# tsy935/eeg-gnn-ssl

Measured on AMD Instinct MI355X. Metric: EEG clips/sec (60s, 19ch, K=2, 2-layer x64) fwd+bwd, higher is better.
Workload: dtype f32

## Files before the change

eeg_gnn_ssl_amd/_lib.py:

```python
from __future__ import annotations

import ctypes
import os
from ctypes import POINTER, c_char_p, c_float, c_int, c_int32, c_int64, c_size_t, c_void_p

_HERE = os.path.dirname(os.path.abspath(__file__))
HIP_LIB_PATH = os.path.join(_HERE, "libeeg_dcrnn_hip.so")
DEV_LIB_PATH = os.path.join(_HERE, "libeeg_dcrnn_hip_dev.so")
ABI_VERSION = 5


class LayerDims(ctypes.Structure):
    _fields_ = [("T", c_int32), ("B", c_int32), ("N", c_int32), ("H", c_int32), ("Fin", c_int32),
                ("M", c_int32), ("act", c_int32), ("p_batched", c_int32), ("x_planes_ready", c_int32),
                ("x_batch_major", c_int32), ("x_plane_stride", c_int64), ("pack3", c_void_p), ("spectral", c_void_p),
                ("spack", c_void_p)]


class DecoderDims(ctypes.Structure):
    _fields_ = [("T", c_int32), ("B", c_int32), ("N", c_int32), ("H", c_int32), ("Dout", c_int32),
                ("M", c_int32), ("L", c_int32), ("act", c_int32), ("p_batched", c_int32), ("dropout_p", c_float),
                ("teacher_on_device", c_int32)]


_FP = c_void_p

_SIGNATURES = {
    "eeg_dcrnn_last_error": (c_char_p, []),
    "eeg_dcrnn_abi_version": (c_int, []),
    "eeg_dcrnn_is_device_build": (c_int, []),
    "eeg_dcrnn_supported": (c_int, [c_int, c_int, c_int, c_int]),
    "eeg_dcrnn_zero": (c_int, [_FP, c_size_t, c_void_p]),
    "eeg_dcrnn_prof_enable": (c_int, [c_int]),
    "eeg_dcrnn_prof_report": (c_int, [ctypes.c_char_p, c_size_t]),
    "eeg_dcrnn_prof_clock_probe": (c_int, [_FP, c_void_p]),
    "eeg_dcrnn_prof_clock_samples": (c_int, [_FP]),
    "eeg_dcrnn_hop_polys": (c_int, [POINTER(c_void_p), c_int, c_int, c_int, c_int, _FP, c_void_p]),
    "eeg_dcrnn_fft_features": (c_int, [_FP, c_int, c_int, c_int, c_int, _FP, _FP, c_float, c_float, _FP, _FP, c_void_p]),
    "eeg_dcrnn_corr_graph_ws_floats": (c_size_t, [c_int, c_int]),
    "eeg_dcrnn_corr_graph": (c_int, [_FP, c_int, c_int, c_int, c_int, c_int, _FP, _FP, _FP, _FP, c_void_p]),
    "eeg_dcrnn_pack_floats": (c_size_t, [c_int, c_int, c_int]),
    "eeg_dcrnn_pack_cell": (c_int, [_FP, _FP, _FP, _FP, c_int, c_int, c_int, _FP, c_void_p]),
    "eeg_dcrnn_pack3_halves": (c_size_t, [c_int, c_int, c_int]),
    "eeg_dcrnn_pack_cell_bf16x3": (c_int, [_FP, _FP, c_int, c_int, c_int, _FP, c_void_p]),
    "eeg_dcrnn_diffuse_fwd": (c_int, [_FP, _FP, c_int, c_int, c_int, c_int, c_int, c_int, _FP, c_void_p]),
    "eeg_dcrnn_diffuse_adj": (c_int, [_FP, _FP, c_int, c_int, c_int, c_int, c_int, c_int, _FP, c_void_p]),
    "eeg_dcrnn_dconv_fwd_ws_floats": (c_size_t, [c_int, c_int, c_int, c_int, c_int]),
    "eeg_dcrnn_dconv_fwd": (c_int, [_FP, _FP, c_int, c_int, c_int, c_int, c_int, _FP, _FP, c_int, _FP, _FP, c_void_p]),
    "eeg_dcrnn_dconv_bwd_ws_floats": (c_size_t, [c_int, c_int, c_int, c_int, c_int]),
    "eeg_dcrnn_dconv_bwd": (c_int, [_FP, _FP, c_int, c_int, c_int, c_int, c_int, _FP, c_int, _FP, _FP, _FP, _FP, _FP, c_void_p]),
    "eeg_dcrnn_spectral_basis_floats": (c_size_t, [c_int]),
    "eeg_dcrnn_spectral_basis": (c_int, [_FP, c_int, _FP, c_void_p]),
    "eeg_dcrnn_spectral_pack_floats": (c_size_t, [c_int, c_int, c_int, c_int]),
    "eeg_dcrnn_pack_cell_spectral": (c_int, [_FP, _FP, _FP, c_int, c_int, c_int, c_int, _FP, c_void_p]),
    "eeg_dcrnn_spectral_ok": (c_int, [POINTER(LayerDims), c_int]),
    "eeg_dcrnn_spectral_rows": (c_size_t, [c_size_t]),
    "eeg_dcrnn_layer_fwd_ws_floats": (c_size_t, [POINTER(LayerDims)]),
    "eeg_dcrnn_batch_major_ok": (c_int, [POINTER(LayerDims)]),
    "eeg_dcrnn_layer_fwd": (c_int, [POINTER(LayerDims)] + [_FP] * 14 + [c_void_p]),
    "eeg_dcrnn_layer_bwd_ws_floats": (c_size_t, [POINTER(LayerDims), c_int]),
    "eeg_dcrnn_layer_bwd": (c_int, [POINTER(LayerDims)] + [_FP] * 22 + [c_void_p]),
    "eeg_dcrnn_decoder_saved_floats": (c_size_t, [POINTER(DecoderDims)]),
    "eeg_dcrnn_decoder_fwd_ws_floats": (c_size_t, [POINTER(DecoderDims)]),
    "eeg_dcrnn_decoder_bwd_ws_floats": (c_size_t, [POINTER(DecoderDims)]),
    "eeg_dcrnn_decoder_is_persistent": (c_int, [POINTER(DecoderDims)]),
    "eeg_dcrnn_decoder_fwd": (c_int, [POINTER(DecoderDims), _FP, c_void_p, _FP, _FP, POINTER(c_void_p), _FP, _FP,
                                      _FP, _FP, _FP, _FP, c_void_p]),
    "eeg_dcrnn_decoder_bwd": (c_int, [POINTER(DecoderDims), c_void_p, _FP, POINTER(c_void_p), _FP, _FP, _FP, _FP, _FP,
                                      POINTER(c_void_p), POINTER(c_void_p), POINTER(c_void_p), POINTER(c_void_p),
                                      _FP, _FP, _FP, c_void_p]),
    "eeg_dcrnn_teacher_flags": (c_int, [_FP, _FP, c_int64, ctypes.c_double, c_int, _FP, c_void_p]),
    "eeg_dcrnn_fft_features_pair": (c_int, [_FP, _FP, c_int, c_int, c_int, c_int, c_int, _FP, _FP, c_float, c_float, _FP, _FP, _FP, c_void_p]),
    "eeg_dcrnn_augment_features": (c_int, [_FP, _FP, c_int, c_int, c_int, c_int, c_int, _FP, _FP, _FP, _FP, c_void_p]),
    "eeg_dcrnn_window_features": (c_int, [_FP, c_int, c_int, c_int, c_int, _FP, _FP, c_float, c_float, _FP, c_void_p]),
    "eeg_dcrnn_window_features_pair": (c_int, [_FP, _FP, c_int, c_int, c_int, c_int, c_int, _FP, _FP, c_float, c_float, _FP, _FP, c_void_p]),
    "eeg_dcrnn_augment_windows": (c_int, [_FP, _FP, c_int, c_int, c_int, c_int, c_int, _FP, _FP, _FP, _FP, _FP, c_void_p]),
    "eeg_dcrnn_corr_graph_rows_ws_floats": (c_size_t, [c_int, c_int, c_int]),
    "eeg_dcrnn_corr_graph_rows": (c_int, [_FP, c_int, c_int, c_int, c_int, ctypes.c_longlong, c_int, _FP, _FP, _FP, _FP, c_void_p]),
    "eeg_dcrnn_augment_draw": (c_int, [_FP, c_int, c_int, _FP, _FP, _FP, _FP, _FP, _FP, c_int, _FP, c_void_p]),
    "eeg_dcrnn_pack_cells": (c_int, [c_int, POINTER(c_void_p), POINTER(c_void_p), POINTER(c_void_p), POINTER(c_void_p), POINTER(ctypes.c_int32),
                             c_int, c_int, POINTER(c_void_p), _FP, c_int, POINTER(c_void_p), c_void_p]),
    "eeg_dcrnn_cls_head_loss_ws_floats": (c_size_t, [c_int, c_int, c_int]),
    "eeg_dcrnn_cls_head_loss": (c_int, [_FP, _FP, _FP, _FP, c_int, c_int, c_int, c_int, c_int, c_float, _FP, _FP, _FP, _FP, _FP, _FP, _FP, _FP, _FP,
                                c_void_p]),
    "eeg_dcrnn_gather_last": (c_int, [_FP, _FP, c_int, c_int, c_int, _FP, c_void_p]),
    "eeg_dcrnn_rng_take": (c_int, [_FP, ctypes.c_uint64, _FP, c_void_p]),
    "eeg_dcrnn_cls_head_fwd": (c_int, [_FP, _FP, _FP, c_int, c_int, c_int, c_int, c_float, _FP, _FP, _FP, c_void_p]),
    "eeg_dcrnn_cls_head_bwd": (c_int, [_FP, _FP, _FP, _FP, c_int, c_int, c_int, c_int, c_float, _FP, _FP, _FP, _FP, c_void_p]),
    "eeg_dcrnn_dropout_mask": (c_int, [_FP, c_size_t, c_float, _FP, c_void_p]),
    "eeg_dcrnn_bce_logits": (c_int, [_FP, _FP, c_int, _FP, _FP, c_void_p]),
    "eeg_dcrnn_ce_logits": (c_int, [_FP, _FP, c_int, c_int, _FP, _FP, c_void_p]),
    "eeg_dcrnn_masked_loss_ws_floats": (c_size_t, []),
    "eeg_dcrnn_masked_loss": (c_int, [_FP, _FP, c_size_t, c_int, c_float, c_float, c_float, c_int, _FP, _FP, _FP, c_void_p]),
    "eeg_dcrnn_clip_adam_ws_floats": (c_size_t, []),
    "eeg_dcrnn_clip_adam": (c_int, [_FP, _FP, _FP, _FP, c_size_t, c_float, c_float, c_float, c_float, c_float, c_float,
                                    c_int, c_float, _FP, _FP, c_void_p]),
    "eeg_dcrnn_clip_adam_dev": (c_int, [_FP, _FP, _FP, _FP, c_size_t, c_float, _FP, c_float, c_float, c_float, c_float,
                                        _FP, c_float, _FP, _FP, c_void_p]),
}


_SIGNATURES_DEV = {
    "eeg_dcrnn_set_seq_probe": (c_int, [_FP]),
    "eeg_dcrnn_set_tuning": (c_int, [c_int, c_int]),
}


class EegDcrnnError(RuntimeError):
    """Raised when a library call reports an error (shape/dtype/launch problems)."""


class EegDcrnnLib:
    def __init__(self, path: str = HIP_LIB_PATH, strict: bool = True):
        if not os.path.exists(path):
            raise ImportError(
                f"{path} not found: the MI355X HIP library is not built. Run `python -c 'import "
                f"__graft_entry__ as g; g.build()'` (or `make -C eeg_gnn_ssl_amd/csrc`). There is no CPU fallback.")
        self.path = path
        self._dll = ctypes.CDLL(path)
        for name, (res, args) in _SIGNATURES.items():
            try:
                fn = getattr(self._dll, name)
            except AttributeError as e:
                if not strict:
                    continue
                raise ImportError(f"{path} does not export {name} (declared in include/eeg_dcrnn.h)") from e
            fn.restype = res
            fn.argtypes = args
        self.is_dev_build = hasattr(self._dll, "eeg_dcrnn_set_tuning")
        if self.is_dev_build:
            for name, (res, args) in _SIGNATURES_DEV.items():
                fn = getattr(self._dll, name)
                fn.restype, fn.argtypes = res, args
        if self._dll.eeg_dcrnn_abi_version() != ABI_VERSION:
            raise ImportError(f"{path}: ABI version {self._dll.eeg_dcrnn_abi_version()} != {ABI_VERSION}; rebuild")
        self.is_device_build = bool(self._dll.eeg_dcrnn_is_device_build())

    def last_error(self) -> str:
        return self._dll.eeg_dcrnn_last_error().decode()

    def call(self, name: str, *args):
        rc = getattr(self._dll, name)(*args)
        if rc != 0:
            raise EegDcrnnError(f"{name}: {self.last_error()}")

    def query(self, name: str, *args):
        return getattr(self._dll, name)(*args)


_LIB = None


def get_lib() -> EegDcrnnLib:
    global _LIB
    if _LIB is None:
        lib = EegDcrnnLib(HIP_LIB_PATH)
        if not lib.is_device_build:
            raise ImportError(f"{HIP_LIB_PATH} is not a device build")
        _LIB = lib
    return _LIB
```

eeg_gnn_ssl_amd/csrc/api.cpp:

```cpp
#include <atomic>
#include <cmath>
#include <cstdarg>
#include <cstdio>
#include <cstring>

#include <string>
#include <vector>

#include "../../include/eeg_dcrnn.h"
#include "../../include/eeg_dcrnn_dev.h"
#include "../../include/eeg_dcrnn_prof.h"
#include "kernels_decoder.h"
#include "kernels_diffuse.h"
#include "kernels_feat.h"
#include "kernels_gemm.h"
#include "kernels_gemm_bf.h"
#include "kernels_graph.h"
#include "kernels_head.h"
#include "kernels_pack.h"
#include "spec_common.h"
#include "spec_launch.h"
#include "kernels_tail.h"
#include "prof.h"
#include "seq_launch.h"
// ... 515 lines not shown
    return 0;
}
namespace {
__global__ __launch_bounds__(256) void clock_probe_kernel(long long ticks, long long* __restrict__ out) {
    const float a = 0.001f * (threadIdx.x & 63), b = 1.f + (threadIdx.x & 63);
    f32x4 p = {0.f, 0.f, 0.f, 0.f}, q = p;
    const long long r0 = realtime_now();
    long long r1 = r0, rh = 0, ch = 0;
    for (int i = 0; i < (1 << 20) && r1 - r0 < ticks; ++i) {
#pragma unroll
        for (int k = 0; k < 16; ++k) { p = mfma16(a, b, p); q = mfma16(b, a, q); }
        r1 = realtime_now();
        if (rh == 0 && r1 - r0 >= ticks / 2) { rh = r1; ch = cycle_now(); }
    }
    const long long c1 = cycle_now();
    if (p[0] + q[0] == 12345.f) out[2] = 1;
    if (threadIdx.x == 0 && rh != 0) {
        atomic_add_u64(reinterpret_cast<unsigned long long*>(out), (unsigned long long)(c1 - ch));
        atomic_add_u64(reinterpret_cast<unsigned long long*>(out) + 1, (unsigned long long)(r1 - rh));
    }
}
}
int eeg_dcrnn_prof_clock_samples(int64_t* buf4) {
    g_clock_samples.store(reinterpret_cast<long long*>(buf4), std::memory_order_release);
    return 0;
}
int eeg_dcrnn_prof_clock_probe(int64_t* out2, void* stream) {
    if (out2 == nullptr) return fail("prof_clock_probe: null output");
    EEG_LAUNCH(clock_probe_kernel, dim3(platform_num_cus()), dim3(256), 0, S_(stream), (long long)20000, reinterpret_cast<long long*>(out2));
    return check_launch("clock_probe");
}
int eeg_dcrnn_supported(int N, int H, int Fin, int M) { return check_dims(N, H, Fin, M) == 0 ? 1 : 0; }
int eeg_dcrnn_zero(void* p, size_t bytes, void* stream) {
    if (bytes == 0) return 0;
    if (p == nullptr) return fail("zero: null pointer");
    if (reinterpret_cast<uintptr_t>(p) % 16 != 0)
        return hipMemsetAsync(p, 0, bytes, S_(stream)) == hipSuccess ? 0 : fail("zero: memset failed");
    const size_t n16 = bytes / 16;
    const int blocks = (int)(n16 / 256 < 1 ? 1 : (n16 / 256 > 1024 ? 1024 : n16 / 256));
    EEG_LAUNCH_P("zero", zero_kernel, dim3(blocks), dim3(256), 0, S_(stream), reinterpret_cast<float4*>(p), n16,
                 reinterpret_cast<unsigned char*>(p) + 16 * n16, (int)(bytes - 16 * n16));
    return check_launch("zero");
}

int eeg_dcrnn_hop_polys(const float* const* supports, int n_supports, int n_graphs, int N, int K, float* P_out,
                        void* stream) {
    if (n_supports < 1 || n_supports > 4) return fail("hop_polys: n_supports=%d unsupported (1..4)", n_supports);
    if (N < 1 || N > kMaxNodes) return fail("hop_polys: num_nodes=%d unsupported", N);
    if (K < 0) return fail("hop_polys: max_diffusion_step=%d unsupported (>= 0)", K);
    if (n_graphs < 1) return fail("hop_polys: no graphs (n_graphs=%d)", n_graphs);
    if (K == 0) return 0;
    if (n_supports * K + 1 > kMaxM) return fail("hop_polys: %d supports x K=%d exceeds %d hop matrices", n_supports, K, kMaxM);
    SupPtrs sp;
    for (int i = 0; i < 4; ++i) sp.p[i] = i < n_supports ? supports[i] : nullptr;
    const size_t lds = 4 * kMaxNodes * kMaxNodes * sizeof(float);
    EEG_LAUNCH_P("hop_polys", hop_polys_kernel, dim3(n_graphs), dim3(round_up(N * N, 64)), lds, S_(stream), sp, n_supports, N, K, P_out);
    return check_launch("hop_polys");
}

size_t eeg_dcrnn_pack_floats(int Fin, int H, int M) { return make_cell_pack(Fin, H, M).total; }

int eeg_dcrnn_pack_cell(const float* Wg, const float* bg, const float* Wc, const float* bc, int Fin, int H, int M,
                        float* pack, void* stream) {
    if (!seq_h_supported(H)) return fail("pack_cell: rnn_units=%d unsupported", H);
    if (Fin < 4 || Fin % 4 != 0) return fail("pack_cell: input dim %d must be a positive multiple of 4", Fin);
    if (!seq_m_supported(M)) return fail("pack_cell: num hop matrices M=%d unsupported (1,2,3,4,5,7)", M);
    CellPack p = make_cell_pack(Fin, H, M);
    EEG_LAUNCH_P("pack_cell", pack_cell_kernel, dim3(512), dim3(256), 0, S_(stream), Wg, bg, Wc, bc, pack, p);
    return check_launch("pack_cell");
}
size_t eeg_dcrnn_pack3_halves(int Fin, int H, int M) { return pack3_supported(Fin, H, M) ? make_pack3(Fin, H, M).total : 0; }
int eeg_dcrnn_pack_cell_bf16x3(const float* Wg, const float* Wc, int Fin, int H, int M, uint16_t* pack3, void* stream) {
    if (!pack3_supported(Fin, H, M)) return fail("pack_cell_bf16x3: rnn_units=%d, input_dim=%d, %d hop matrices: the bf16 split exists for 64 units", H, Fin, M);
    if (Wg == nullptr || Wc == nullptr || pack3 == nullptr) return fail("pack_cell_bf16x3: null pointer");
    EEG_LAUNCH_P("pack_cell", pack_cell_bf3_kernel, dim3(512), dim3(256), 0, S_(stream), Wg, Wc, Fin, H, M, pack3);
    return check_launch("pack_cell_bf3");
}

int eeg_dcrnn_diffuse_fwd(const float* X, const float* P, int p_batched, int S, int B, int N, int F, int M,
                          float* planes, void* stream) {
    if (N < 1 || N > kMaxNodes || F < 4 || F % 4 != 0 || M < 1 || M > kMaxM) return fail("diffuse_fwd: bad dims N=%d F=%d M=%d", N, F, M);
    if (S < 1 || B < 1) return fail("diffuse_fwd: empty input (S=%d, B=%d)", S, B);
    return diffuse_fwd(X, P, p_batched, S, B, N, F, M, planes, S_(stream));
}
int eeg_dcrnn_diffuse_adj(const float* Z, const float* P, int p_batched, int S, int B, int N, int F, int M,
                          float* dX, void* stream) {
    if (N < 1 || N > kMaxNodes || F < 4 || F % 4 != 0 || M < 1 || M > kMaxM) return fail("diffuse_adj: bad dims N=%d F=%d M=%d", N, F, M);
    if (S < 1 || B < 1) return fail("diffuse_adj: empty input (S=%d, B=%d)", S, B);
    return diffuse_adj(Z, P, p_batched, S, B, N, F, M, dX, S_(stream));
}

static bool layer_dims_positive(const eeg_layer_dims* d) {
    return d != nullptr && d->T >= 1 && d->B >= 1 && d->N >= 1 && d->H >= 1 && d->Fin >= 1 && d->M >= 1;
}
size_t eeg_dcrnn_layer_fwd_ws_floats(const eeg_layer_dims* d) {
    if (!layer_dims_positive(d)) return 0;
    const size_t xw = (size_t)d->T * d->B * d->N * 3 * d->H;
    return d->spectral != nullptr ? xw + (size_t)d->N * spec_rows(d->T * d->B) * 3 * d->H : xw;
}

size_t eeg_dcrnn_spectral_basis_floats(int N) { return (N >= 1 && N <= kMaxNodes) ? (size_t)spec_basis_floats(N) : 0; }
size_t eeg_dcrnn_spectral_rows(size_t S) { return (S + 15) / 16 * 16; }
int eeg_dcrnn_spectral_basis(const float* support, int N, float* basis, void* stream) {
    if (N < 2 || N > kMaxNodes) return fail("spectral_basis: num_nodes=%d unsupported (2..%d)", N, kMaxNodes);
    if (support == nullptr || basis == nullptr) return fail("spectral_basis: null pointer");
    if (launch_spec_basis(support, N, basis, S_(stream))) return fail("spectral_basis: launch failed");
    return check_launch("spectral_basis");
}
size_t eeg_dcrnn_spectral_pack_floats(int Fin, int H, int M, int N) {
    return (Fin >= 4 && Fin % 4 == 0 && H == 64 && M >= 1 && M <= kMaxM && N >= 1 && N <= kMaxNodes) ? spec_pack_floats(Fin, H, M, N) : 0;
}
int eeg_dcrnn_pack_cell_spectral(const float* Wg, const float* Wc, const float* basis, int Fin, int H, int M, int N, float* spack,
                                 void* stream) {
    if (eeg_dcrnn_spectral_pack_floats(Fin, H, M, N) == 0)
        return fail("pack_cell_spectral: input_dim=%d rnn_units=%d hop matrices=%d nodes=%d: the spectral form exists for 64 units", Fin, H, M, N);
    if (Wg == nullptr || Wc == nullptr || basis == nullptr || spack == nullptr) return fail("pack_cell_spectral: null pointer");
    if (launch_spec_pack(Wg, Wc, basis, Fin, H, M, N, spack, S_(stream))) return fail("pack_cell_spectral: launch failed");
    return check_launch("pack_cell_spectral");
}
int eeg_dcrnn_pack_cells(int n_cells, const float* const* Wg, const float* const* bg, const float* const* Wc, const float* const* bc,
                         const int32_t* Fin, int H, int M, float* const* packs, const float* basis, int N, float* const* spacks,
                         void* stream) {
    if (n_cells < 1 || n_cells > 4) return fail("pack_cells: %d cells (1..4 per launch)", n_cells);
    if (Wg == nullptr || bg == nullptr || Wc == nullptr || bc == nullptr || Fin == nullptr || packs == nullptr) return fail("pack_cells: null pointer table");
    if (!seq_h_supported(H)) return fail("pack_cells: rnn_units=%d unsupported", H);
    if (!seq_m_supported(M)) return fail("pack_cells: num hop matrices M=%d unsupported (1,2,3,4,5,7)", M);
    if ((basis == nullptr) != (spacks == nullptr)) return fail("pack_cells: the per-frequency packs need the basis block and their output table");
    int fin[4];
    for (int c = 0; c < n_cells; ++c) {
        fin[c] = Fin[c];
        if (fin[c] < 4 || fin[c] % 4 != 0) return fail("pack_cells: input dim %d of cell %d must be a positive multiple of 4", fin[c], c);
        if (Wg[c] == nullptr || bg[c] == nullptr || Wc[c] == nullptr || bc[c] == nullptr || packs[c] == nullptr || (spacks != nullptr && spacks[c] == nullptr))
            return fail("pack_cells: null pointer in the tables of cell %d", c);
        if (spacks != nullptr && eeg_dcrnn_spectral_pack_floats(fin[c], H, M, N) == 0)
            return fail("pack_cells: input_dim=%d rnn_units=%d hop matrices=%d nodes=%d: the spectral form exists for 64 units", fin[c], H, M, N);
    }
    if (launch_pack_cells(n_cells, Wg, bg, Wc, bc, fin, H, M, packs, basis, N, spacks, S_(stream))) return fail("pack_cells: launch failed");
    return check_launch("pack_cells");
}
int eeg_dcrnn_spectral_ok(const eeg_layer_dims* d, int need_dx) {
    if (!layer_dims_positive(d) || d->p_batched) return 0;
    if (d->x_planes_ready && d->Fin != d->H) return 0;
    if (check_dims(d->N, d->H, d->Fin, d->M)) return 0;
    return spec_supported(d->T, d->B, d->N, d->H, d->Fin, d->M, need_dx) ? 1 : 0;
}

int eeg_dcrnn_batch_major_ok(const eeg_layer_dims* d) {
    if (!diffuse_streams(d->p_batched, d->T * d->B, d->B, d->N, d->Fin)) return 0;
    const int R = d->T * d->B * d->N;
    const GemmKnobs k = gemm_knobs();
    return (nn_dma_applies(d->Fin, R, 3 * d->H, k) && tn_dma_applies(d->Fin, 3 * d->H, k)) ? 2 : 1;
}

int eeg_dcrnn_layer_fwd(const eeg_layer_dims* d, const float* X, float* Xtm, const float* h0, const float* P,
                        const float* pack, float* planes, float* Hext, float* Rs, float* Us, float* Cs, float* RHs,
                        float* Hplanes, float* RHplanes, float* ws, void* stream) {
    if (check_dims(d->N, d->H, d->Fin, d->M)) return 1;
    if (d->T < 1 || d->B < 1) return fail("layer_fwd: empty sequence/batch (T=%d, B=%d)", d->T, d->B);
    const bool save = Rs != nullptr;
    if (save != (Us != nullptr) || save != (Cs != nullptr) || save != (RHs != nullptr))
        return fail("layer_fwd: Rs/Us/Cs/RHs must be all NULL or all non-NULL");
    hipStream_t st = S_(stream);
    const int S = d->T * d->B, R = S * d->N, H = d->H, M = d->M, Fin = d->Fin;
    const size_t state = (size_t)d->B * d->N * H;
    CellPack p = make_cell_pack(Fin, H, M);
    if (h0 != nullptr && h0 != Hext && copy_floats(Hext, h0, state, st)) return 1;
    const size_t xs = d->x_plane_stride > 0 ? (size_t)d->x_plane_stride : (size_t)R * Fin;
    BtMap bt;
    if (d->x_batch_major) {
        if (Xtm != nullptr || d->x_planes_ready) return fail("layer_fwd: x_batch_major excludes Xtm and x_planes_ready");
        if (d->spectral == nullptr && eeg_dcrnn_batch_major_ok(d) != 2) return fail("layer_fwd: x_batch_major is not available for this shape (eeg_dcrnn_batch_major_ok)");
        bt.T = d->T; bt.B = d->B; bt.N = d->N;
    }
    float* XW = ws;
    if (d->spectral != nullptr) {
        if (!eeg_dcrnn_spectral_ok(d, 0)) return fail("layer_fwd: the spectral form does not cover this shape (eeg_dcrnn_spectral_ok)");
        if (Xtm != nullptr || d->spack == nullptr) return fail("layer_fwd: spectral excludes Xtm and needs spack");
        if ((Hplanes != nullptr) != (RHplanes != nullptr)) return fail("layer_fwd: Hplanes/RHplanes must be both NULL or both non-NULL");
        const SpecPack sp = make_spec_pack(Fin, H, M, d->N);
        const int N = d->N, Sp = spec_rows(S), SpE = d->B + Sp;
        const size_t xgs = d->x_plane_stride > 0 ? (size_t)d->x_plane_stride : (size_t)Sp * Fin;
        float* Yh = ws + (size_t)R * 3 * H;
        if (!d->x_planes_ready && launch_spec_mix(1, X, d->spectral, nullptr, N, d->T, d->B, Fin, d->x_batch_major ? 1 : 0, planes, st, "spec_mix_x"))
            return fail("spec_mix: launch failed");
        int nnf = g_tune[EEG_TUNE_SPEC_NN_GROUPED] == 0 ? launch_nnf(planes, xgs, Fin, Sp, N, d->spack + sp.sxr, sp.sxr_stride, Yh, num_cus(), st, "gemm_nn_xw", pack + p.bias,
                                               d->spectral + spec_csum_offset(N)) : -1;
        if (nnf > 0) return fail("gemm_nnf: launch failed");
        if (nnf < 0 && launch_nng(planes, Fin, Sp, N, d->spack + sp.sxq, sp.sxq_stride, sp.nct_x, Yh, num_cus(), st, "gemm_nn_xw", pack + p.bias,
                                  d->spectral + spec_csum_offset(N), xgs)) return fail("gemm_nng: launch failed");
        SeqFwdArgs a{XW, h0 != nullptr ? Hext : nullptr, P, d->p_batched, pack + p.bhg, pack + p.bhc, Hext + state, Rs, Us, Cs, RHs, nullptr, nullptr,
                     (size_t)0, d->T, d->B, N, d->act, seq_probe_arg(st)};
        SeqCall call = seq_fwd_call(H, M, N, d->T, d->B, 0, a.probe);
        call.spectral = true; call.Sp = Sp; call.SpE = SpE;
        const SeqPlan plan = seq_fwd_plan(call);
        if (plan.kind == SeqKind::TwoWaveSpec) {
            a.XW = Yh; a.Hpl = Hplanes; a.RHpl = RHplanes; a.spec_U = d->spectral; a.spec_Sp = Sp; a.spec_SpE = SpE;
            if (seq_fwd(H, M, plan, a, st)) return 1;
            if (Hplanes != nullptr) {
                if (launch_spec_zero_rows(Hplanes, N, (d->T + 1) * d->B, SpE, H, st)) return fail("spec_zero_rows: launch failed");
                if (launch_spec_zero_pad(RHplanes, N, S, H, st)) return fail("spec_zero_pad: launch failed");
            }
        } else {
            if (launch_spec_mix(0, Yh, d->spectral, nullptr, N, d->T, d->B, 3 * H, 0, XW, st, "spec_mix_y")) return fail("spec_mix: launch failed");
            if (seq_fwd(H, M, plan, a, st)) return 1;
            if (Hplanes != nullptr) {
                if (launch_spec_mix(1, Hext, d->spectral, nullptr, N, d->T + 1, d->B, H, 0, Hplanes, st, "spec_mix_h", SpE)) return fail("spec_mix: launch failed");
                if (launch_spec_mix(1, RHs, d->spectral, nullptr, N, d->T, d->B, H, 0, RHplanes, st, "spec_mix_h")) return fail("spec_mix: launch failed");
            }
        }
        return check_launch("layer_fwd (spectral)");
    } else if (d->x_planes_ready) {
        if (Xtm != nullptr) return fail("layer_fwd: x_planes_ready excludes a batch-major input");
    } else {
        if (diffuse_fwd(X, P, d->p_batched, S, d->B, d->N, Fin, M, planes, st, xs, d->x_batch_major ? 2 : (Xtm != nullptr ? 1 : 0), Xtm)) return 1;
        if (Xtm != nullptr) X = Xtm;
    }
    SegPtrs segs;
    for (int m = 0; m < kMaxM; ++m) segs.p[m] = m == 0 ? X : (m < M ? planes + (size_t)(m - 1) * xs : nullptr);
    const bool bf3 = d->pack3 != nullptr && pack3_supported(Fin, H, M);
    const Pack3 q = make_pack3(Fin, H, M);
    const NnCall cxw = nn_call(M, Fin, R, 3 * H / 16, 3 * H, 3 * H, bt, p.has_bxq, bf3 ? q.xw_nct : 0);
    if (gemm_nn(gemm_nn_plan(cxw), cxw, segs, NnRhs{pack + p.bx, pack + p.bxq, bf3 ? d->pack3 + q.xw : nullptr}, pack + p.bias, XW, st, "gemm_nn_xw", bt)) return 1;
    if ((Hplanes != nullptr) != (RHplanes != nullptr)) return fail("layer_fwd: Hplanes/RHplanes must be both NULL or both non-NULL");
    SeqFwdArgs a{XW, h0 != nullptr ? Hext : nullptr, P, d->p_batched, pack + p.bhg, pack + p.bhc, Hext + state, Rs, Us, Cs, RHs, Hplanes, RHplanes,
                 (size_t)(d->T + 1) * state, d->T, d->B, d->N, d->act, seq_probe_arg(st)};
    return seq_fwd(H, M, seq_fwd_plan(seq_fwd_call(H, M, d->N, d->T, d->B, a.plane_stride, a.probe)), a, st);
}

size_t eeg_dcrnn_layer_bwd_ws_floats(const eeg_layer_dims* d, int need_dx) { return layer_dims_positive(d) ? bwd_ws(d, need_dx).total : 0; }

int eeg_dcrnn_layer_bwd(const eeg_layer_dims* d, const float* X, const float* P, const float* pack,
                        const float* planes, const float* Hext, const float* Rs, const float* Us, const float* Cs,
                        const float* RHs, const float* Hplanes, const float* RHplanes, const float* dHseq,
                        const float* d_at_end, const float* d_at_len,
                        const int64_t* lengths, float* dX, float* dh0, float* dWg, float* dbg, float* dWc,
                        float* dbc, float* ws, void* stream) {
    if (check_dims(d->N, d->H, d->Fin, d->M)) return 1;
    if (d->T < 1 || d->B < 1) return fail("layer_bwd: empty sequence/batch (T=%d, B=%d)", d->T, d->B);
    hipStream_t st = S_(stream);
    const int S = d->T * d->B, R = S * d->N, H = d->H, M = d->M, Fin = d->Fin, N = d->N;
    const size_t state = (size_t)d->B * N * H;
    CellPack p = make_cell_pack(Fin, H, M);
    BwdWs w = bwd_ws(d, dX != nullptr);
    float* dXW = ws + w.dxw;
    float* dbias = ws + w.dbias;
    SeqBwdArgs a{Hext + state, Hext, Rs, Us, Cs, dHseq, d_at_end, d_at_len,
                 reinterpret_cast<const long long*>(lengths), P, d->p_batched, pack + p.b1, pack + p.b2,
                 dXW, dh0, dbias, d->T, d->B, N, d->act, seq_probe_arg(st)};
    SeqCall call = seq_bwd_call(H, M, N, d->T, d->B, a.probe);
    call.spectral = d->spectral != nullptr; call.Sp = spec_rows(S); call.SpE = d->B + spec_rows(S);
    const SeqPlan plan = seq_bwd_plan(call);
    const bool dyh_done = plan.kind == SeqKind::TwoWaveSpec;
    if (dyh_done) { a.spec_U = d->spectral; a.dYh = ws + w.dyh; a.spec_Sp = call.Sp; }
    if (seq_bwd(H, M, plan, a, st)) return 1;
    const size_t xs = d->x_plane_stride > 0 ? (size_t)d->x_plane_stride : (size_t)R * Fin;
    BtMap bt;
    if (d->x_batch_major) {
        if (d->spectral == nullptr && eeg_dcrnn_batch_major_ok(d) != 2) return fail("layer_bwd: x_batch_major is not available for this shape");
        bt.T = d->T; bt.B = d->B; bt.N = N;
    }
    if (d->spectral != nullptr) {
        if (!eeg_dcrnn_spectral_ok(d, dX != nullptr)) return fail("layer_bwd: the spectral form does not cover this shape (eeg_dcrnn_spectral_ok)");
        if (d->spack == nullptr) return fail("layer_bwd: spectral needs spack");
        if ((Hplanes != nullptr) != (RHplanes != nullptr)) return fail("layer_bwd: Hplanes/RHplanes must be both NULL or both non-NULL");
        const SpecPack sp = make_spec_pack(Fin, H, M, N);
        const int Sp = spec_rows(S), SpE = d->B + Sp;
        float* dYh = ws + w.dyh;
        if (dyh_done) {
            if (launch_spec_zero_pad(dYh, N, S, 3 * H, st)) return fail("spec_zero_pad: launch failed");
        } else if (launch_spec_mix(1, dXW, d->spectral, nullptr, N, d->T, d->B, 3 * H, 0, dYh, st, "spec_mix_dy")) return fail("spec_mix: launch failed");
        const float *hh = Hplanes, *rhh = RHplanes;
        size_t hh_gs = (size_t)SpE * H;
        if (hh == nullptr) {
            if (launch_spec_mix(1, Hext, d->spectral, nullptr, N, d->T, d->B, H, 0, ws + w.hplanes, st, "spec_mix_h")) return fail("spec_mix: launch failed");
            if (launch_spec_mix(1, RHs, d->spectral, nullptr, N, d->T, d->B, H, 0, ws + w.rhplanes, st, "spec_mix_h")) return fail("spec_mix: launch failed");
            hh = ws + w.hplanes; rhh = ws + w.rhplanes; hh_gs = 0;
        }
        if (cell_weight_grads_spectral(d, planes, xs_spec(d), hh, hh_gs, rhh, dYh, ws + w.partial, w, dWg, dWc, st, dbias, dbg, dbc)) return 1;
        if (dX != nullptr) {
            const int dxf = g_tune[EEG_TUNE_SPEC_DX_PASSES] == 0 ? launch_dxf(dYh, Sp, S, N, Fin, d->spack + sp.sxtq, sp.sxtq_stride, d->spectral, dX, st, "gemm_dx_f") : -1;
            if (dxf > 0) return fail("gemm_dxf: launch failed");
            if (dxf < 0) {
                float* dXh = ws + w.z;
                if (launch_nng(dYh, 3 * H, Sp, N, d->spack + sp.sxtq, sp.sxtq_stride, sp.nct_t, dXh, num_cus(), st, "gemm_nn_dx")) return fail("gemm_nng: launch failed");
                if (launch_spec_mix(0, dXh, d->spectral, nullptr, N, d->T, d->B, Fin, 0, dX, st, "spec_mix_dx")) return fail("spec_mix: launch failed");
            }
        }
        return check_launch("layer_bwd (spectral)");
    }
    if (cell_weight_grads(d, X, planes, xs, Hext, RHs, dXW, P, Hplanes, RHplanes, (size_t)(d->T + 1) * state,
                          ws + w.hplanes, ws + w.rhplanes, ws + w.partial, w, false, dWg, dWc, st, bt, dbias, dbg, dbc)) return 1;
    if (dX != nullptr) {
        float* Z = ws + w.z;
        SegPtrs sd;
        for (int m = 0; m < kMaxM; ++m) sd.p[m] = m == 0 ? dXW : nullptr;
        const bool bf3 = d->pack3 != nullptr && pack3_supported(Fin, H, M);
        const Pack3 q = make_pack3(Fin, H, M);
        const NnCall cdx = nn_call(1, 3 * H, R, round_up(M * Fin, 16) / 16, M * Fin, M * Fin, BtMap(), p.has_bxtq, bf3 ? q.dx_nct : 0);
        if (gemm_nn(gemm_nn_plan(cdx), cdx, sd, NnRhs{pack + p.bxt, pack + p.bxtq, bf3 ? d->pack3 + q.dx : nullptr}, nullptr, Z, st, "gemm_nn_dx")) return 1;
        if (diffuse_adj(Z, P, d->p_batched, S, d->B, N, Fin, M, dX, st)) return 1;
    }
    return 0;
}


int eeg_dcrnn_fft_features(const float* raw, int B, int N, int T, int W, const int32_t* perm, const float* log_scale,
                           float mean, float std_, float* feat_raw, float* feat_std, void* stream) {
    if (B < 1 || N < 1 || T < 1) return fail("fft_features: empty input (B=%d, N=%d, T=%d)", B, N, T);
    if (W < 4 || W % 4 != 0 || W / 4 + 1 > 64) return fail("fft_features: window=%d unsupported (multiple of 4, <= 252)", W);
    if (feat_raw == nullptr && feat_std == nullptr) return fail("fft_features: no output requested");
    if (feat_std != nullptr && !(std_ != 0.f)) return fail("fft_features: std must be non-zero");
    if (W == kFftWin) {
        const long long n_windows = (long long)B * N * T;
        const long long n_items = (n_windows + kFftPerWave - 1) / kFftPerWave;
        long long blocks = (n_items + 3) / 4;
        const long long cap = (long long)platform_num_cus() * kFftWgPerCu;
        if (blocks > cap) blocks = cap;
        const size_t lds = 4 * (size_t)kFftWaveDoubles * sizeof(double);
        EEG_SET_MAX_LDS(fft200_features_kernel, lds);
        EEG_LAUNCH_P("fft_features", fft200_features_kernel, dim3((unsigned)blocks), dim3(256), lds, S_(stream), raw, N, T, n_windows,
                     reinterpret_cast<const int*>(perm), log_scale, mean, 1.0f / std_, feat_raw, feat_std);
        return check_launch("fft_features");
    }
    int tchunk = T;
    while (tchunk > 1 && (long long)B * N * ceil_div(T, tchunk) < 8192) tchunk = ceil_div(tchunk, 2);
    EEG_LAUNCH_P("fft_features", fft_features_kernel, dim3(B * N, ceil_div(T, tchunk)), dim3(64), (size_t)W * sizeof(double), S_(stream),
                 raw, N, T, W, tchunk, reinterpret_cast<const int*>(perm), log_scale, mean, 1.0f / std_, feat_raw, feat_std);
    return check_launch("fft_features");
}

int eeg_dcrnn_fft_features_pair(const float* raw_x, const float* raw_y, int B, int N, int Tx, int Ty, int W, const int32_t* perm,
                                const float* log_scale, float mean, float std_, float* feat_raw_x, float* x_std, float* y_std,
                                void* stream) {
    if (raw_x == nullptr || raw_y == nullptr) return fail("fft_features_pair: null input (raw_x=%p, raw_y=%p)", (const void*)raw_x, (const void*)raw_y);
    if (B < 1 || N < 1 || Tx < 1 || Ty < 1) return fail("fft_features_pair: empty input (B=%d, N=%d, Tx=%d, Ty=%d)", B, N, Tx, Ty);
    if (W < 4 || W % 4 != 0 || W / 4 + 1 > 64) return fail("fft_features_pair: window=%d unsupported (multiple of 4, <= 252)", W);
    if (x_std == nullptr || y_std == nullptr)
        return fail("fft_features_pair: null output (x_std=%p, y_std=%p): the pair is the standardised input and target", (void*)x_std, (void*)y_std);
    if (!(std_ != 0.f)) return fail("fft_features_pair: std must be non-zero");
    if (W != kFftWin) {
        if (eeg_dcrnn_fft_features(raw_x, B, N, Tx, W, perm, log_scale, mean, std_, feat_raw_x, x_std, stream)) return 1;
        return eeg_dcrnn_fft_features(raw_y, B, N, Ty, W, perm, log_scale, mean, std_, nullptr, y_std, stream);
    }
    const FftHalf hx = {raw_x, Tx, (long long)B * N * Tx, feat_raw_x, x_std}, hy = {raw_y, Ty, (long long)B * N * Ty, nullptr, y_std};
    const long long n_items = (hx.n_windows + kFftPerWave - 1) / kFftPerWave + (hy.n_windows + kFftPerWave - 1) / kFftPerWave;
    long long blocks = (n_items + 3) / 4;
    const long long cap = (long long)platform_num_cus() * kFftWgPerCu;
    if (blocks > cap) blocks = cap;
    const size_t lds = 4 * (size_t)kFftWaveDoubles * sizeof(double);
    EEG_SET_MAX_LDS(fft200_features_pair_kernel, lds);
    EEG_LAUNCH_P("fft_features_pair", fft200_features_pair_kernel, dim3((unsigned)blocks), dim3(256), lds, S_(stream), hx, hy, N,
                 reinterpret_cast<const int*>(perm), log_scale, mean, 1.0f / std_);
    return check_launch("fft_features_pair");
}

int eeg_dcrnn_augment_features(const float* x, const float* y, int B, int Tx, int Ty, int N, int D, const int32_t* perm, const float* shift,
                               float* x_out, float* y_out, void* stream) {
    if (x == nullptr || y == nullptr || perm == nullptr || shift == nullptr) return fail("augment_features: null input / perm / shift");
    if (x_out == nullptr || y_out == nullptr) return fail("augment_features: null output (x_out=%p, y_out=%p)", (void*)x_out, (void*)y_out);
    if (x_out == x || y_out == y) return fail("augment_features: in-place call (rows move between nodes: outputs must not alias inputs)");
    if (B < 1 || N < 1 || Tx < 1 || Ty < 1) return fail("augment_features: empty input (B=%d, N=%d, Tx=%d, Ty=%d)", B, N, Tx, Ty);
    if (D < 4 || D % 4 != 0) return fail("augment_features: feature dim=%d unsupported (positive multiple of 4)", D);
    if ((((uintptr_t)x | (uintptr_t)y | (uintptr_t)x_out | (uintptr_t)y_out) & 15) != 0) return fail("augment_features: tensors must be 16-byte aligned");
    const long long pieces = (long long)(Tx + Ty) * N * (D / 4);
    const long long chunks = (pieces + kAugPerBlock - 1) / kAugPerBlock;
    if (chunks > 65535) return fail("augment_features: %lld values per clip exceed one launch (limit %lld)", 4 * pieces, 4LL * 65535 * kAugPerBlock);
    const dim3 grid((unsigned)B, (unsigned)chunks);
    if (D == 100)
        EEG_LAUNCH_P("augment_features", augment_features_kernel<25>, grid, dim3(kAugThreads), 0, S_(stream), x, y, N, Tx, Ty, D / 4,
                     reinterpret_cast<const int*>(perm), shift, x_out, y_out);
    else
        EEG_LAUNCH_P("augment_features", augment_features_kernel<0>, grid, dim3(kAugThreads), 0, S_(stream), x, y, N, Tx, Ty, D / 4,
                     reinterpret_cast<const int*>(perm), shift, x_out, y_out);
    return check_launch("augment_features");
}

static int window_stream(const char* what, bool raw, const float* x, const float* y, int B, int Tx, int Ty, int N, int W, const int32_t* perm,
                         const float* a, const float* c, float mean, float std_, float* x_out, float* y_out, void* stream) {
    if (B < 1 || N < 1 || Tx < 1 || Ty < 0) return fail("%s: empty input (B=%d, N=%d, Tx=%d, Ty=%d)", what, B, N, Tx, Ty);
    if (W < 4 || W % 4 != 0) return fail("%s: window=%d unsupported (positive multiple of 4)", what, W);
    if (x_out == x || (Ty > 0 && y_out == y)) return fail("%s: in-place call (rows move between nodes: outputs must not alias inputs)", what);
    if ((((uintptr_t)x | (uintptr_t)y | (uintptr_t)x_out | (uintptr_t)y_out) & 15) != 0) return fail("%s: tensors must be 16-byte aligned", what);
    const long long pieces = (long long)(Tx + Ty) * N * (W / 4);
    const long long chunks = (pieces + kAugPerBlock - 1) / kAugPerBlock;
    if (chunks > 65535) return fail("%s: %lld values per clip exceed one launch (limit %lld)", what, 4 * pieces, 4LL * 65535 * kAugPerBlock);
    const dim3 grid((unsigned)B, (unsigned)chunks);
    const int* pm = reinterpret_cast<const int*>(perm);
#define EEG_WSTREAM(RAW, D4C) \
    EEG_LAUNCH_P(what, (window_stream_kernel<RAW, D4C>), grid, dim3(kAugThreads), 0, S_(stream), x, y, N, Tx, Ty, W / 4, pm, a, c, mean, std_, x_out, y_out)
    if (raw) { if (W == 200) EEG_WSTREAM(true, 50); else EEG_WSTREAM(true, 0); }
    else { if (W == 200) EEG_WSTREAM(false, 50); else EEG_WSTREAM(false, 0); }
#undef EEG_WSTREAM
    return check_launch(what);
}

int eeg_dcrnn_window_features(const float* raw, int B, int N, int T, int W, const int32_t* perm, const float* scale, float mean, float std_,
                              float* x_std, void* stream) {
    if (raw == nullptr) return fail("window_features: null input");
    if (x_std == nullptr) return fail("window_features: null output");
    if (!(std_ != 0.f)) return fail("window_features: std must be non-zero");
    return window_stream("window_features", true, raw, nullptr, B, T, 0, N, W, perm, scale, nullptr, mean, std_, x_std, nullptr, stream);
}

int eeg_dcrnn_window_features_pair(const float* raw_x, const float* raw_y, int B, int N, int Tx, int Ty, int W, const int32_t* perm,
                                   const float* scale, float mean, float std_, float* x_std, float* y_std, void* stream) {
    if (raw_x == nullptr || raw_y == nullptr)
        return fail("window_features_pair: null input (raw_x=%p, raw_y=%p)", (const void*)raw_x, (const void*)raw_y);
    if (x_std == nullptr || y_std == nullptr)
        return fail("window_features_pair: null output (x_std=%p, y_std=%p): the pair is the standardised input and target", (void*)x_std, (void*)y_std);
    if (Ty < 1) return fail("window_features_pair: empty input (B=%d, N=%d, Tx=%d, Ty=%d)", B, N, Tx, Ty);
    if (!(std_ != 0.f)) return fail("window_features_pair: std must be non-zero");
    return window_stream("window_features_pair", true, raw_x, raw_y, B, Tx, Ty, N, W, perm, scale, nullptr, mean, std_, x_std, y_std, stream);
}

int eeg_dcrnn_augment_windows(const float* x, const float* y, int B, int Tx, int Ty, int N, int D, const int32_t* perm, const float* a,
                              const float* c, float* x_out, float* y_out, void* stream) {
    if (x == nullptr || perm == nullptr || a == nullptr || c == nullptr) return fail("augment_windows: null input / perm / factors");
    if ((y == nullptr) != (Ty == 0)) return fail("augment_windows: target and Ty=%d disagree (no target: y = NULL and Ty = 0)", Ty);
    if (x_out == nullptr || (y != nullptr && y_out == nullptr)) return fail("augment_windows: null output (x_out=%p, y_out=%p)", (void*)x_out, (void*)y_out);
    return window_stream("augment_windows", false, x, y, B, Tx, Ty, N, D, perm, a, c, 0.f, 1.f, x_out, y_out, stream);
}

static int corr_nsplit(int B, int T) {
    int ns = ceil_div(g_tune[EEG_TUNE_GRAM_WGS] > 0 ? g_tune[EEG_TUNE_GRAM_WGS] : 1024, B);
    const int cap = ceil_div(T, 4);
    if (ns > cap) ns = cap;
    return ns < 1 ? 1 : ns;
}
int eeg_dcrnn_augment_draw(const uint64_t* rng_used, int B, int N, const int32_t* swap_perm, int32_t* flags, int32_t* perm,
                           float* log_scale, const float* S_plain, const float* S_reflected, int n_supports, float* S_out, void* stream) {
    if (rng_used == nullptr || swap_perm == nullptr || flags == nullptr || perm == nullptr || log_scale == nullptr)
        return fail("augment_draw: null generator pair / swap table / output");
    if (B < 1 || N < 1 || N > kMaxNodes) return fail("augment_draw: B=%d clips, num_nodes=%d unsupported (B >= 1, 1 <= N <= %d)", B, N, kMaxNodes);
// ... 511 lines not shown
```

eeg_gnn_ssl_amd/csrc/kernels_gemm_f.h:

```cpp
#pragma once
#include "common.h"
#include "kernels_gemm_q.h"

namespace eeg {

#ifndef EEG_X_TNF_RC
#define EEG_X_TNF_RC 8
#endif
#ifndef EEG_X_TNF_NS
#define EEG_X_TNF_NS 5
#endif
#ifndef EEG_X_TNF_MINW
#define EEG_X_TNF_MINW 2
#endif
#ifndef EEG_X_TNF_NS2
#define EEG_X_TNF_NS2 3
#endif
#ifndef EEG_X_TNF_MINW2
#define EEG_X_TNF_MINW2 3
#endif
constexpr int kTnfRC = EEG_X_TNF_RC;
__host__ __device__ constexpr int tnf_ns(int FXT) { return FXT <= 2 ? EEG_X_TNF_NS2 : EEG_X_TNF_NS; }
__host__ __device__ constexpr int tnf_wgs_per_cu(int FXT) { return FXT <= 2 ? EEG_X_TNF_MINW2 : EEG_X_TNF_MINW; }
__host__ __device__ constexpr int tnf_stage_floats(int FXT) { return (kTnfRC / 8) * (FXT * 256 + 512 + 512 + 1536); }
// ... 229 lines not shown
            dsc[j] = rx; lofs[j] = d * 256; cstep[j] = (unsigned)(RC * Fin) * 4u;
            soff[j] = (unsigned)(rbeg * Fin) * 4u;
            vof[j] = d * 1024 + lane * 16 < RC * Fin * 4 ? (unsigned)(d * 1024 + lane * 16) : 0u;
        } else if (d < NX + NH) {
            dsc[j] = rh; lofs[j] = HI + (d - NX) * 256; cstep[j] = RC * 64 * 4u;
            soff[j] = (unsigned)(rbeg * 64) * 4u; vof[j] = (unsigned)((d - NX) * 1024 + lane * 16);
        } else if (d < NX + 2 * NH) {
            dsc[j] = rr; lofs[j] = RI + (d - NX - NH) * 256; cstep[j] = RC * 64 * 4u;
            soff[j] = (unsigned)(rbeg * 64) * 4u; vof[j] = (unsigned)((d - NX - NH) * 1024 + lane * 16);
        } else {
            dsc[j] = ry; lofs[j] = YI + (d - NX - 2 * NH) * 256; cstep[j] = RC * 192 * 4u;
            soff[j] = (unsigned)(rbeg * 192) * 4u; vof[j] = (unsigned)((d - NX - 2 * NH) * 1024 + lane * 16);
        }
    }
    float* px = part_x + (size_t)y * Fin * 192;
    float* pg = part_g + (size_t)y * 64 * 128;
    float* pc = part_c + (size_t)y * 64 * 64;
    const TnfRing<FXT> rg{dsc, lofs, vof, soff, cstep};
#ifndef EEG_X_TNF_NOR4
    if constexpr (FXT == 4) {
        if (Fin == 100) {
            if (s == 0) { if (e == 0) tnf_role_r4<0, 0>(sm, Q, lane, rg, px, pg, pc); else tnf_role_r4<0, 1>(sm, Q, lane, rg, px, pg, pc); }
            else { if (e == 0) tnf_role_r4<1, 0>(sm, Q, lane, rg, px, pg, pc); else tnf_role_r4<1, 1>(sm, Q, lane, rg, px, pg, pc); }
            return;
        }
    }
#endif
    if (s == 0) tnf_role<FXT, 0>(sm, Q, Fin, e, lane, rg, px, pg, pc);
    else tnf_role<FXT, 1>(sm, Q, Fin, e, lane, rg, px, pg, pc);
}

#ifndef EEG_X_NNF_NS
#define EEG_X_NNF_NS 3
#endif
constexpr int kNnfNS = EEG_X_NNF_NS;
__host__ __device__ constexpr int nnf_stage_floats(int K) { return 64 * K + 4; }
__host__ __device__ constexpr size_t nnf_lds_bytes(int K) { return (size_t)kNnfNS * nnf_stage_floats(K) * sizeof(float); }

template <int KQ, bool SWZ>
__global__ __launch_bounds__(256, 2) void gemm_nnf_kernel(const float* __restrict__ A, long long a_gstride, int K, int Sp, int G,
                                                         const float* __restrict__ Wr, unsigned w_gstride, float* __restrict__ C,
                                                         const float* __restrict__ bias, const float* __restrict__ gscale) {
    constexpr int NS = kNnfNS;
    EEG_DYN_SMEM(sm);
    const int tid = threadIdx.x, lane = tid & 63, w = wave_uniform(tid >> 6), rw = w & 1, cw = w >> 1, hh = lane >> 5, l32 = lane & 31;
    const int ST = nnf_stage_floats(K), CPG = ceil_div(Sp, 64), total = G * CPG;
    const int NPC = ceil_div(64 * K, 256), PER = ceil_div(NPC, 4);
    const int g0 = (int)(((long long)blockIdx.x * total) / gridDim.x), g1 = (int)(((long long)(blockIdx.x + 1) * total) / gridDim.x);
    const int Q = g1 - g0;
    if (tid < 4 * NS) sm[(tid >> 2) * ST + 64 * K + (tid & 3)] = 0.f;
    const unsigned lane_src = SWZ ? (unsigned)((lane >> 4) * 256 + (((lane & 15) ^ ((4 * w + (lane >> 4)) & 15)) << 4)) : (unsigned)lane * 16u;
    int d_g = g0, d_stage = 0, d_grp = -1;
    wbuf_t ra = make_wbuf_n(A, 0u);
    auto issue = [&]() __attribute__((always_inline)) {
        const int grp = d_g / CPG, lc = d_g - grp * CPG;
        if (grp != d_grp) { d_grp = grp; ra = make_wbuf_n(A + (size_t)grp * a_gstride, (unsigned)(Sp * K) * 4u); }
        float* base = sm + d_stage * ST;
        const unsigned cb = (unsigned)(lc * 64 * K) * 4u;
        for (int j = 0; j < PER; ++j) {
            int p = w + 4 * j;
            if (p >= NPC) p = NPC - 1;
            wbuf_dma16(ra, base + p * 256, cb + (unsigned)p * 1024u + lane_src, 0u);
        }
        d_stage = d_stage + 1 == NS ? 0 : d_stage + 1;
        ++d_g;
    };
    float wr[KQ][4][3];
    f32x16 acc[3];
    float binit[3] = {0.f, 0.f, 0.f};
    int c_grp = -1;
    wbuf_t rc = make_wbuf_n(C, 0u);
    const int row = 32 * rw + l32;
    const int a_row = row * K;
    const int ccol = 32 * 3 * cw + l32;
#pragma unroll 1
    for (int p = 0; p < NS - 1; ++p)
        if (p < Q) issue();
    int r_stage = 0;
#pragma unroll 1
    for (int q = 0; q < Q; ++q) {
        const int g = g0 + q, grp = g / CPG, lc = g - grp * CPG;
        if (grp != c_grp) {
            c_grp = grp;
            const wbuf_t rwt = make_wbuf(Wr + (size_t)grp * w_gstride);
#pragma unroll
            for (int kq = 0; kq < KQ; ++kq)
#pragma unroll
                for (int s = 0; s < 4; ++s)
#pragma unroll
                    for (int t = 0; t < 3; ++t) wr[kq][s][t] = wbuf_ld(rwt, (unsigned)(4 * hh * 192 + ccol), (unsigned)((8 * kq + s) * 192 + 32 * t));
            const float gs = bias != nullptr ? gscale[grp] : 0.f;
#pragma unroll
            for (int t = 0; t < 3; ++t) binit[t] = bias != nullptr ? gs * bias[ccol + 32 * t] : 0.f;
            rc = make_wbuf_n(C + (size_t)grp * Sp * 192, (unsigned)(Sp * 192) * 4u);
        }
        {
            int nd = Q - 1 - q;
            if (nd > NS - 2) nd = NS - 2;
            const int n = 48 * (q < NS - 1 ? q : NS - 1) + PER * nd;
            if (n >= 63) vm_wait_n<63>(); else if (n >= 55) vm_wait_n<55>(); else if (n >= 52) vm_wait_n<52>(); else if (n >= 48) vm_wait_n<48>();
            else if (n >= 14) vm_wait_n<14>(); else if (n >= 8) vm_wait_n<8>(); else if (n >= 7) vm_wait_n<7>(); else if (n >= 4) vm_wait_n<4>();
            else vm_wait_n<0>();
        }
#ifndef EEG_X_NNF_NOBAR
        EEG_LDS_BARRIER();
#endif
#ifndef EEG_X_NNF_NODMA
        if (q + NS - 1 < Q) issue();
#endif
        const float* st = sm + r_stage * ST;
#pragma unroll
        for (int t = 0; t < 3; ++t)
#pragma unroll
            for (int v = 0; v < 16; ++v) acc[t][v] = binit[t];
        f32x4 a4 = *reinterpret_cast<const f32x4*>(st + a_row + (SWZ ? ((hh ^ (row & 15)) << 2) : 4 * hh));
#pragma unroll
        for (int kq = 0; kq < KQ; ++kq) {
            f32x4 an = a4;
#ifndef EEG_X_NNF_NOLDS
            if (kq + 1 < KQ) an = *reinterpret_cast<const f32x4*>(st + a_row + (SWZ ? (((2 * (kq + 1) + hh) ^ (row & 15)) << 2) : 4 * (2 * (kq + 1) + hh)));
#endif
            EEG_SCHED_FENCE();
#pragma unroll
            for (int s = 0; s < 4; ++s)
#pragma unroll
                for (int t = 0; t < 3; ++t) acc[t] = mfma32(a4[s], wr[kq][s][t], acc[t]);
            EEG_SCHED_FENCE();
            a4 = an;
        }
        unsigned ob[4];
#pragma unroll
        for (int b = 0; b < 4; ++b) {
            ob[b] = (unsigned)((lc * 64 + 32 * rw + 4 * hh + 8 * b) * 192 + ccol);
            EEG_PIN(ob[b]);
        }
#pragma unroll
        for (int t = 0; t < 3; ++t)
#pragma unroll
#ifndef EEG_X_NNF_NOSTORE
            for (int v = 0; v < 16; ++v) wbuf_st1(rc, ob[v >> 2] + (unsigned)((v & 3) * 192 + 32 * t), 0u, acc[t][v]);
#else
            for (int v = 0; v < 16; ++v) { EEG_USE(acc[t][v]); (void)rc; }
#endif
        EEG_SCHED_FENCE();
        r_stage = r_stage + 1 == NS ? 0 : r_stage + 1;
    }
}

constexpr int kDxfMaxN = 20, kDxfNS = 3, kDxfRows = 32, kDxfStage = kDxfRows * 192;
__host__ __device__ constexpr size_t dxf_lds_bytes() { return (size_t)kDxfNS * kDxfStage * sizeof(float); }

template <int NT>
__global__ __launch_bounds__(256, 2) void gemm_dxf_kernel(const float* __restrict__ dYh, int Sp, int S, int Nrt, const float* __restrict__ Wtq,
                                                         unsigned w_gstride, const float* __restrict__ basis, float* __restrict__ dX) {
    const int N = NT > 0 ? NT : Nrt;
    constexpr int NS = kDxfNS, ST = kDxfStage, RB = kDxfRows, PER = 6;
    EEG_DYN_SMEM(sm);
    const int tid = threadIdx.x, lane = tid & 63, w = wave_uniform(tid >> 6), lr = lane & 15, lg = lane >> 4;
    const int r0 = (int)blockIdx.x * RB;
    unsigned src[PER];
#pragma unroll
    for (int j = 0; j < PER; ++j) {
        const int P = 64 * (w + 4 * j) + lane, row = P / 48, slot = P - row * 48;
        const int unit = (slot & ~15) | ((slot & 15) ^ (row & 15));
        src[j] = (unsigned)((r0 + row) * 768 + unit * 16);
    }
    int d_i = 0, d_stage = 0;
    auto issue = [&]() __attribute__((always_inline)) {
        const wbuf_t ra = make_wbuf_n(dYh + (size_t)d_i * Sp * 192, (unsigned)(Sp * 192) * 4u);
        float* base = sm + d_stage * ST;
#pragma unroll
        for (int j = 0; j < PER; ++j) wbuf_dma16(ra, base + (w + 4 * j) * 256, src[j], 0u);
        d_stage = d_stage + 1 == NS ? 0 : d_stage + 1;
        if (d_i + 1 < N) ++d_i;
    };
    f32x4 acc[kDxfMaxN][2];
#pragma unroll
    for (int j = 0; j < kDxfMaxN; ++j) acc[j][0] = acc[j][1] = (f32x4){0.f, 0.f, 0.f, 0.f};
    f32x4 wq[12];
    const unsigned wl = (unsigned)(w * 64 + lane) * 4u;
    static_assert(kDxfNS == 3, "the queue discipline below is written for two images in flight");
    issue();
    issue();
    EEG_SCHED_FENCE();
    {
        const wbuf_t rw0 = make_wbuf(Wtq);
#pragma unroll
        for (int c = 0; c < 12; ++c) wq[c] = wbuf_ld4(rw0, wl, (unsigned)(c * 4 * 256));
    }
    vm_wait_n<PER + 12>();
    int r_stage = 0;
    const int a_row = lr * 192;
#pragma unroll 1
    for (int i = 0; i < N; ++i) {
        EEG_LDS_BARRIER();
#ifndef EEG_X_DXF_NODMA
        issue();
#endif
        const wbuf_t rwn = make_wbuf(Wtq + (size_t)(i + 1 < N ? i + 1 : i) * w_gstride);
        const float* st = sm + r_stage * ST;
        float uu[kDxfMaxN];
#pragma unroll
        for (int j = 0; j < kDxfMaxN; ++j) uu[j] = (NT > 0 ? j < NT : j < N) ? basis[j * N + i] : 0.f;
        f32x4 t0 = {0.f, 0.f, 0.f, 0.f}, t1 = {0.f, 0.f, 0.f, 0.f};
        auto frag_off = [&](int c) __attribute__((always_inline)) {
            const int u = 4 * c + lg;
            return a_row + (((u & ~15) | ((u & 15) ^ lr)) << 2);
        };
        f32x4 fa[2][2];
        fa[0][0] = *reinterpret_cast<const f32x4*>(st + frag_off(0));
        fa[0][1] = *reinterpret_cast<const f32x4*>(st + 16 * 192 + frag_off(0));
#pragma unroll
        for (int c = 0; c < 12; ++c) {
            if (c + 1 < 12) {
                fa[(c + 1) & 1][0] = *reinterpret_cast<const f32x4*>(st + frag_off(c + 1));
                fa[(c + 1) & 1][1] = *reinterpret_cast<const f32x4*>(st + 16 * 192 + frag_off(c + 1));
            }
            EEG_SCHED_FENCE();
#pragma unroll
            for (int e = 0; e < 4; ++e) {
                t0 = mfma16(wq[c][e], fa[c & 1][0][e], t0);
                t1 = mfma16(wq[c][e], fa[c & 1][1][e], t1);
            }
            EEG_SCHED_FENCE();
#ifndef EEG_X_DXF_NOW
            wq[c] = wbuf_ld4(rwn, wl, (unsigned)(c * 4 * 256));
#endif
            EEG_SCHED_FENCE();
        }
#pragma unroll
        for (int j = 0; j < kDxfMaxN; ++j)
            if (NT > 0 ? j < NT : j < N) {
                acc[j][0] += t0 * uu[j];
                acc[j][1] += t1 * uu[j];
            }
        r_stage = r_stage + 1 == NS ? 0 : r_stage + 1;
    }
    const wbuf_t rx = make_wbuf_n(dX, (unsigned)(S * N * 64) * 4u);
#pragma unroll
    for (int t = 0; t < 2; ++t) {
        const unsigned rb = (unsigned)((r0 + 16 * t + lr) * N * 64 + 16 * w + 4 * lg);
#pragma unroll
        for (int j = 0; j < kDxfMaxN; ++j)
            if (j < N) wbuf_st4(rx, rb + (unsigned)(j * 64), 0u, acc[j][t]);
    }
}

}
```

eeg_gnn_ssl_amd/csrc/kernels_seq.h:

```cpp
#pragma once
#include "common.h"
#include "lds_diffuse.h"

namespace eeg {

constexpr int seq_nks(int N) { return N <= 20 ? 5 : 8; }
constexpr bool seq_has_two_wave(int H, int M, int nks) { return H == 64 && nks == 5 && M <= 3; }
constexpr bool seq_has_spec(int H, int M, int nks) { return seq_has_two_wave(H, M, nks) && M >= 2; }
constexpr bool seq_has_probe(int H, int M, int nks) { return kDevBuild && H == 64 && M == 3 && nks == 5; }
constexpr bool seq_has_stream(int H, int M) { return H == 64 && M <= 5; }

template <int H, int M>
struct SeqGeom {
    static constexpr int KA = M * H, KAP = lds_stride_x(KA), KS = KA / 4;
    static constexpr int KG = M * 2 * H, KGP = lds_stride_x(KG), KSG = KG / 4;
    static constexpr int NGT = 2 * H / 16, NCT = H / 16;
    static constexpr int GT = ceil_div(NGT, 4), CT = ceil_div(NCT, 4);
};
constexpr size_t seq_fwd_lds_floats(int H, int M) { return (size_t)(M - 1) * kPFloats + 2 * 32 * lds_stride_x(M * H); }
constexpr size_t seq_fwd2_lds_floats(int H, int M, bool spec) {
    return seq_fwd_lds_floats(H, M) + 16 * 64 + (spec ? 3 * 16 * 64 + 4 * 64 + 4 * (M * H / 4 / 4) * 256 : 0);
}
constexpr size_t seq_bwd_lds_floats(int H, int M, int rows) {
    return (size_t)(M - 1) * kPFloats + (size_t)rows * (lds_stride_x(M * H) + lds_stride_x(M * 2 * H));
// ... 143 lines not shown
    if constexpr (Q0 >= Q1) return;
    float4 a0 = frag(p0, s0, Q0), a1 = frag(p1, s1, Q0);
#pragma unroll
    for (int q = Q0; q < Q1; ++q) {
        float4 n0 = a0, n1 = a1;
        if (q + 1 < Q1) { n0 = frag(p0, s0, q + 1); n1 = frag(p1, s1, q + 1); }
        EEG_SCHED_FENCE();
        const float x0[4] = {a0.x, a0.y, a0.z, a0.w}, x1[4] = {a1.x, a1.y, a1.z, a1.w};
#pragma unroll
        for (int j = 0; j < 4; ++j) {
            if (j & 1) alt = mfma16(w[4 * q + j], x0[j], alt);
            else acc = mfma16(w[4 * q + j], x0[j], acc);
        }
#pragma unroll
        for (int j = 0; j < 4; ++j) rem[j] = mfma4(x1[j], w[4 * q + j], rem[j]);
        EEG_SCHED_FENCE();
        a0 = n0;
        a1 = n1;
    }
}

template <int NKS>
__device__ __forceinline__ void load_spec_frags(const float* __restrict__ U, int N, int lane, float (&uf)[NKS], float (&u4)[NKS]) {
    const int lr = lane & 15, lg = lane >> 4;
#pragma unroll
    for (int ks = 0; ks < NKS; ++ks) {
        const int n = 4 * ks + lg, i4 = 16 + (lane & 3);
        uf[ks] = (n < N && lr < N) ? U[n * N + lr] : 0.f;
        u4[ks] = (n < N && i4 < N) ? U[n * N + i4] : 0.f;
    }
}
template <int NKS, int NG>
__device__ __forceinline__ void spec_mix_tiles_out(const float* const (&tile)[NG], const int (&stride)[NG], const int (&src_col)[NG],
                                                   const int (&gcol)[NG], const float (&uf)[NKS], const float (&u4)[NKS], int lr, int lg,
                                                   wbuf_t out, unsigned voff0, unsigned voff1, unsigned soff, bool valid0, bool valid1) {
    float a[NG][NKS];
#pragma unroll
    for (int g = 0; g < NG; ++g)
#pragma unroll
        for (int ks = 0; ks < NKS; ++ks) a[g][ks] = tile[g][lds_sw(4 * ks + lg, src_col[g] + lr, stride[g])];
    f32x4 acc[NG], alt[NG], rem[NG], rem2[NG];
#pragma unroll
    for (int g = 0; g < NG; ++g) acc[g] = alt[g] = rem[g] = rem2[g] = (f32x4){0.f, 0.f, 0.f, 0.f};
#pragma unroll
    for (int ks = 0; ks < NKS; ++ks)
#pragma unroll
        for (int g = 0; g < NG; ++g) {
            if (NG == 1 && (ks & 1)) alt[g] = mfma16(a[g][ks], uf[ks], alt[g]);
            else acc[g] = mfma16(a[g][ks], uf[ks], acc[g]);
        }
#pragma unroll
    for (int ks = 0; ks < NKS; ++ks)
#pragma unroll
        for (int g = 0; g < NG; ++g) {
            if (ks & 1) rem2[g] = mfma4(u4[ks], a[g][ks], rem2[g]);
            else rem[g] = mfma4(u4[ks], a[g][ks], rem[g]);
        }
    if (NG == 1) acc[0] += alt[0];
#pragma unroll
    for (int g = 0; g < NG; ++g) {
        f32x4 tr = rem[g] + rem2[g];
        EEG_PIN(tr);
        const float r1 = rem4_reduce(tr);
        if (valid0) wbuf_st4(out, voff0 + (unsigned)gcol[g], soff, acc[g]);
        if (valid1) wbuf_st1(out, voff1 + (unsigned)gcol[g], soff, r1);
    }
}

template <int NKS>
__device__ __forceinline__ float mfma_rem4_ldsw(const float* __restrict__ X, int stride, int lane, int lg, const float* __restrict__ wl) {
    const int s1 = lg ^ sigma4(lane & 3);
    const float* p1 = X + (16 + (lane & 3)) * stride;
    auto frag = [&](int q) { return *reinterpret_cast<const float4*>(p1 + 64 * (q >> 2) + 4 * ((4 * (q & 3)) ^ s1)); };
    f32x4 rem[4];
#pragma unroll
    for (int j = 0; j < 4; ++j) rem[j] = (f32x4){0.f, 0.f, 0.f, 0.f};
    constexpr int NQ = NKS / 4, D = 2;
    float4 xa[D], wa[D];
#pragma unroll
    for (int d = 0; d < D; ++d) {
        xa[d] = frag(d < NQ ? d : NQ - 1);
        wa[d] = *reinterpret_cast<const float4*>(wl + (d < NQ ? d : NQ - 1) * 256 + 4 * lane);
    }
#pragma unroll
    for (int q = 0; q < NQ; ++q) {
        const float4 a1 = xa[q % D], w4 = wa[q % D];
        if (q + D < NQ) {
            xa[q % D] = frag(q + D);
            wa[q % D] = *reinterpret_cast<const float4*>(wl + (q + D) * 256 + 4 * lane);
        }
        EEG_SCHED_FENCE();
        const float x1[4] = {a1.x, a1.y, a1.z, a1.w}, ww[4] = {w4.x, w4.y, w4.z, w4.w};
#pragma unroll
        for (int j = 0; j < 4; ++j) rem[j] = mfma4(x1[j], ww[j], rem[j]);
        EEG_SCHED_FENCE();
    }
    f32x4 t = (rem[0] + rem[1]) + (rem[2] + rem[3]);
    EEG_PIN(t);
    return rem4_reduce(t);
}

struct ClockSample {
    long long c0, r0;
    __device__ __forceinline__ void begin(const long long* clk, bool me) {
        if (clk != nullptr && me) { c0 = cycle_now(); r0 = realtime_now(); }
    }
    __device__ __forceinline__ void end(long long* clk, bool me) {
        if (clk != nullptr && me) {
            atomic_add_u64(reinterpret_cast<unsigned long long*>(clk), (unsigned long long)(cycle_now() - c0));
            atomic_add_u64(reinterpret_cast<unsigned long long*>(clk) + 1, (unsigned long long)(realtime_now() - r0));
        }
    }
};

template <bool ON>
struct PhaseProbe {
    long long acc[8];
    long long last;
    long long rt[4];
    __device__ __forceinline__ void start() {
        if (ON) {
#pragma unroll
            for (int i = 0; i < 8; ++i) acc[i] = 0;
            rt[0] = realtime_now();
            rt[1] = rt[2] = rt[3] = 0;
            last = cycle_now();
        }
    }
    __device__ __forceinline__ void mark(int k) {
        if (ON) {
            const long long t = cycle_now();
            acc[k] += t - last;
            last = t;
        }
    }
    __device__ __forceinline__ void stamp(int k) {
        if (ON) rt[k] = realtime_now();
    }
    __device__ __forceinline__ void dump(long long* p, int slot0) {
        if (ON) {
            rt[3] = realtime_now();
            if (p != nullptr && (threadIdx.x & 63) == 0) {
                long long* d = p + ((size_t)blockIdx.x * 4 + ((threadIdx.x >> 6) & 3)) * 32 + slot0;
#pragma unroll
                for (int i = 0; i < 8; ++i) d[i] = acc[i];
                long long* e = p + ((size_t)blockIdx.x * 4 + ((threadIdx.x >> 6) & 3)) * 32 + 16 + slot0 / 2;
#pragma unroll
                for (int i = 0; i < 4; ++i) e[i] = rt[i];
            }
        }
    }
};

template <int H, int M, int NKS, bool PROBE = false>
__global__ __launch_bounds__(256, 1) void seq_fwd_kernel(
    const float* __restrict__ XW, const float* __restrict__ h0, const float* __restrict__ P, int p_batched,
    const float* __restrict__ bhg, const float* __restrict__ bhc,
    float* __restrict__ Hseq, float* __restrict__ Rs, float* __restrict__ Us, float* __restrict__ Cs,
    float* __restrict__ RHs, float* __restrict__ Hpl, float* __restrict__ RHpl, size_t plane_stride,
    int T, int B, int N, int act, long long* probe) {
    using G = SeqGeom<H, M>;
    constexpr int KAP = G::KAP, KS = G::KS, CT = G::CT, NGT = G::NGT, NCT = G::NCT;
    PhaseProbe<PROBE> pp;
    pp.start();
    EEG_DYN_SMEM(sm);
    float* Pl = sm;
    float* A = Pl + (M - 1) * kPFloats;
    float* A2 = A + 32 * KAP;
    constexpr bool REM4 = NKS == 5;
    const int tid = threadIdx.x, lane = tid & 63, wave = tid >> 6, lr = lane & 15, lg = lane >> 4;
    const bool save = Rs != nullptr;

    float wg[2 * CT][KS], wc[CT][KS];
#pragma unroll
    for (int i = 0; i < CT; ++i) {
        const int ct = wave + 4 * i < NCT ? wave + 4 * i : 0;
#pragma unroll
        for (int ks = 0; ks < KS; ++ks) {
            wg[i][ks] = bhg[((size_t)ks * NGT + ct) * 64 + lane];
            wg[CT + i][ks] = bhg[((size_t)ks * NGT + NCT + ct) * 64 + lane];
            wc[i][ks] = bhc[((size_t)ks * NCT + ct) * 64 + lane];
        }
    }

    for (int b = blockIdx.x; b < B; b += gridDim.x) {
    __syncthreads();
    for (int e = tid; e < 2 * 32 * KAP; e += 256) A[e] = 0.f;
    lds_load_polys(Pl, P, p_batched ? b : 0, M, N);
    __syncthreads();
    float pf[poly_slots<M, NKS>()][NKS];
    load_poly_frags<M, NKS, false>(Pl, pf, lr, lg);
    if (h0 != nullptr) {
        for (int e = tid; e < N * H; e += 256) A[lds_sw(e / H, e % H, KAP)] = h0[(size_t)b * N * H + e];
    } else {
        for (int e = tid; e < N * H; e += 256) (Hseq - (size_t)B * N * H)[(size_t)b * N * H + e] = 0.f;
    }
    __syncthreads();

    const int node[2] = {lr, 16 + lr};
    const bool valid[2] = {lr < N, 16 + lr < N};
    const int nodec[2] = {valid[0] ? lr : N - 1, valid[1] ? 16 + lr : N - 1};
    const f32x4 zero4 = {0.f, 0.f, 0.f, 0.f};
    int oxw[CT][2], oh[CT][2];
    const int node1 = 16 + lg;
    const bool valid1 = node1 < N;
    int l1[CT];
#pragma unroll
    for (int i = 0; i < CT; ++i)
#pragma unroll
        for (int nt = 0; nt < 2; ++nt) {
            const int ct = wave + 4 * i < NCT ? wave + 4 * i : 0;
            oxw[i][nt] = nodec[nt] * (3 * H) + ct * 16 + 4 * lg;
            oh[i][nt] = nodec[nt] * H + ct * 16 + 4 * lg;
            if (REM4 && nt == 1) {
                oxw[i][1] = (valid1 ? node1 : N - 1) * (3 * H) + ct * 16 + lr;
                oh[i][1] = (valid1 ? node1 : N - 1) * H + ct * 16 + lr;
                l1[i] = lds_sw(node1, ct * 16 + lr, KAP);
            }
        }

    const bool plane_buf = (double)(M - 1) * plane_stride * sizeof(float) < 2147483648.0;
    auto diffuse_own = [&](float* buf, float* planes, int t) {
        EEG_WAVE_SYNC();
        float* g = planes != nullptr ? planes + ((size_t)t * B + b) * N * H : nullptr;
#pragma unroll
        for (int i = 0; i < CT; ++i)
            if (wave + 4 * i < NCT) lds_diffuse_tile<M, NKS>(buf, KAP, (wave + 4 * i) * 16, H, pf, lr, lg, g, plane_stride, N, plane_buf);
    };
    diffuse_own(A, Hpl, 0);
    f32x4 nxr[CT][2], nxu[CT][2], nxc[CT][2];
    auto fetch_xw = [&](int t) {
        const wbuf_t bx = make_wbuf(XW + ((size_t)t * B + b) * N * (3 * H));
#pragma unroll
        for (int i = 0; i < CT; ++i)
#pragma unroll
            for (int nt = 0; nt < 2; ++nt) {
                if (REM4 && nt == 1) {
                    nxr[i][1] = (f32x4){wbuf_ld(bx, oxw[i][1], 0u), 0.f, 0.f, 0.f};
                    nxu[i][1] = (f32x4){wbuf_ld(bx, oxw[i][1] + H, 0u), 0.f, 0.f, 0.f};
                    nxc[i][1] = (f32x4){wbuf_ld(bx, oxw[i][1] + 2 * H, 0u), 0.f, 0.f, 0.f};
                    continue;
                }
                nxr[i][nt] = wbuf_ld4(bx, oxw[i][nt], 0u);
                nxu[i][nt] = wbuf_ld4(bx, oxw[i][nt] + H, 0u);
                nxc[i][nt] = wbuf_ld4(bx, oxw[i][nt] + 2 * H, 0u);
            }
    };
    fetch_xw(0);
    for (int t = 0; t < T; ++t) {
        const size_t s = (size_t)t * B + b;
        f32x4 ag[2 * CT][2], ac[CT][2], ug[CT][2];
#pragma unroll
        for (int i = 0; i < CT; ++i)
#pragma unroll
            for (int nt = 0; nt < 2; ++nt) {
                ag[i][nt] = nxr[i][nt]; ag[CT + i][nt] = nxu[i][nt]; ac[i][nt] = nxc[i][nt];
            }
        EEG_LDS_BARRIER();
        pp.mark(0);

        mfma_nodes32<2 * CT, KS, REM4, 0, 0, false, false, REM4>(A, KAP, lane, lr, lg, wg, ag);
        pp.mark(1);
        const wbuf_t bR = make_wbuf((save ? Rs : Hseq) + s * N * H), bRH = make_wbuf((save ? RHs : Hseq) + s * N * H),
                     bU = make_wbuf((save ? Us : Hseq) + s * N * H);
#pragma unroll
        for (int i = 0; i < CT; ++i) {
            const int ct = wave + 4 * i;
            if (ct < NCT) {
                const int col = ct * 16 + 4 * lg;
#pragma unroll
                for (int nt = 0; nt < 2; ++nt) {
                    if (REM4 && nt == 1) {
                        const float rg1 = sigmoidf_(ag[i][1][0]), u1 = sigmoidf_(ag[CT + i][1][0]);
                        ug[i][1] = (f32x4){u1, 0.f, 0.f, 0.f};
                        const float rh1 = valid1 ? rg1 * A[l1[i]] : 0.f;
                        A2[l1[i]] = rh1;
                        if (save && valid1) {
                            wbuf_st1(bR, oh[i][1], 0u, rg1);
                            wbuf_st1(bRH, oh[i][1], 0u, rh1);
                            wbuf_st1(bU, oh[i][1], 0u, u1);
                        }
                        continue;
                    }
                    const f32x4 rg = sigmoid4_(ag[i][nt]), u = sigmoid4_(ag[CT + i][nt]);
                    ug[i][nt] = u;
                    f32x4 rh = rg * ld4(A + lds_sw(node[nt], col, KAP));
                    rh = valid[nt] ? rh : zero4;
                    st4(A2 + lds_sw(node[nt], col, KAP), rh);
                    if (save && valid[nt]) {
                        wbuf_st4(bR, oh[i][nt], 0u, rg);
                        wbuf_st4(bRH, oh[i][nt], 0u, rh);
                        wbuf_st4(bU, oh[i][nt], 0u, u);
                    }
                }
            }
        }
        pp.mark(2);
        diffuse_own(A2, RHpl, t);
        pp.mark(7);
        EEG_LDS_BARRIER();
        pp.mark(3);
        if (t + 1 < T) fetch_xw(t + 1);

        mfma_nodes32<CT, KS, REM4, 0, 0, false, false, REM4>(A2, KAP, lane, lr, lg, wc, ac);
        pp.mark(4);
        const wbuf_t bH = make_wbuf(Hseq + s * N * H), bC = make_wbuf((save ? Cs : Hseq) + s * N * H);
#pragma unroll
        for (int i = 0; i < CT; ++i) {
            const int ct = wave + 4 * i;
            if (ct < NCT) {
                const int col = ct * 16 + 4 * lg;
#pragma unroll
                for (int nt = 0; nt < 2; ++nt) {
                    if (REM4 && nt == 1) {
                        const float u1 = ug[i][1][0], h1 = A[l1[i]];
                        const float c1 = act == 0 ? tanhf_(ac[i][1][0]) : fmaxf(ac[i][1][0], 0.f);
                        const float hn1 = valid1 ? u1 * h1 + (1.f - u1) * c1 : 0.f;
                        A[l1[i]] = hn1;
                        if (valid1) {
                            wbuf_st1(bH, oh[i][1], 0u, hn1);
                            if (save) wbuf_st1(bC, oh[i][1], 0u, c1);
                        }
                        continue;
                    }
                    const f32x4 u = ug[i][nt], h = ld4(A + lds_sw(node[nt], col, KAP));
                    const f32x4 c = act == 0 ? tanh4_(ac[i][nt]) : relu4_(ac[i][nt]);
                    f32x4 hn = u * h + (1.f - u) * c;
                    hn = valid[nt] ? hn : zero4;
                    st4(A + lds_sw(node[nt], col, KAP), hn);
                    if (valid[nt]) {
                        wbuf_st4(bH, oh[i][nt], 0u, hn);
                        if (save) wbuf_st4(bC, oh[i][nt], 0u, c);
                    }
                }
            }
        }
        pp.mark(5);
        if (t + 1 < T || Hpl != nullptr) diffuse_own(A, Hpl, t + 1);
        pp.mark(6);
    }
    }
    pp.dump(probe, 0);
}

template <int H, int M, int NKS, bool PROBE = false, bool SPEC = false>
__global__ __launch_bounds__(512, 1) void seq_fwd2_kernel(
    const float* __restrict__ XW, const float* __restrict__ h0, const float* __restrict__ P, int p_batched,
    const float* __restrict__ bhg, const float* __restrict__ bhc,
    float* __restrict__ Hseq, float* __restrict__ Rs, float* __restrict__ Us, float* __restrict__ Cs,
    float* __restrict__ RHs, float* __restrict__ Hpl, float* __restrict__ RHpl, size_t plane_stride,
    int T, int B, int N, int act, long long* probe, const float* __restrict__ spec_U = nullptr, int spec_Sp = 0, int spec_SpE = 0) {
    using G = SeqGeom<H, M>;
    PhaseProbe<PROBE> pp;
    pp.start();
    static_assert(G::CT == 1 && NKS == 5, "one column tile per wave, second node tile on the 4x4x1 MFMA");
    constexpr int KAP = G::KAP, KS = G::KS, NGT = G::NGT, NCT = G::NCT, UST = 64;
    EEG_DYN_SMEM(sm);
    float* Pl = sm;
    float* A = Pl + (M - 1) * kPFloats;
    float* A2 = A + 32 * KAP;
    const int tid = threadIdx.x, lane = tid & 63, wave8 = SPEC ? wave_uniform(tid >> 6) : (tid >> 6), role = wave8 >> 2, wave = wave8 & 3;
    const int lr = lane & 15, lg = lane >> 4;
    float* U = A2 + 32 * KAP;
    float* XR = U + 16 * UST;
    float* XC = XR + 16 * UST;
    float* XRr = XC + 2 * 16 * UST;
    float* W1L = XRr + 4 * 64;
    const bool save = Rs != nullptr;
    const int ct = wave;
    const wbuf_t bH = make_wbuf(Hseq), bR = make_wbuf(save ? Rs : Hseq), bU = make_wbuf(save ? Us : Hseq),
                 bC = make_wbuf(save ? Cs : Hseq), bRH = make_wbuf(save ? RHs : Hseq);

    float w0[1][KS], w1[1][KS];
#pragma unroll
    for (int ks = 0; ks < KS; ++ks) w0[0][ks] = bhg[((size_t)ks * NGT + (role == 0 ? ct : NCT + ct)) * 64 + lane];
    if (!SPEC || role == 0) {
#pragma unroll
        for (int ks = 0; ks < KS; ++ks) w1[0][ks] = bhc[((size_t)ks * NCT + ct) * 64 + lane];
    } else {
#pragma unroll
        for (int q = 0; q < KS / 4; ++q) {
            f32x4 v;
#pragma unroll
            for (int j = 0; j < 4; ++j) v[j] = bhc[((size_t)(4 * q + j) * NCT + ct) * 64 + lane];
            st4(W1L + (ct * (KS / 4) + q) * 256 + 4 * lane, v);
        }
    }
    auto clip = [&](const int b, auto ROLE_T) __attribute__((always_inline)) {
    constexpr int ROLE_C = decltype(ROLE_T)::value;
    __syncthreads();
    for (int e = tid; e < 2 * 32 * KAP; e += 512) A[e] = 0.f;
    lds_load_polys(Pl, P, p_batched ? b : 0, M, N);
    __syncthreads();
    if (h0 != nullptr) {
        for (int e = tid; e < N * H; e += 512) A[lds_sw(e / H, e % H, KAP)] = h0[(size_t)b * N * H + e];
    } else {
        for (int e = tid; e < N * H; e += 512) (Hseq - (size_t)B * N * H)[(size_t)b * N * H + e] = 0.f;
    }
    __syncthreads();

    const bool valid[2] = {lr < N, 16 + lr < N};
    const int nodec[2] = {valid[0] ? lr : N - 1, valid[1] ? 16 + lr : N - 1};
    const f32x4 zero4 = {0.f, 0.f, 0.f, 0.f};
    const int col = ct * 16 + 4 * lg;
    const int oxw0 = nodec[0] * (3 * H) + col, oh0 = nodec[0] * H + col;
    const int node1 = 16 + lg, col1 = ct * 16 + lr;
    const bool valid1 = node1 < N;
    const int oxw1 = (valid1 ? node1 : N - 1) * (3 * H) + col1, oh1 = (valid1 ? node1 : N - 1) * H + col1;
    const int l1 = lds_sw(node1, col1, KAP);
    if (ROLE_C < 0 ? role == 0 : ROLE_C == 0) {
        EEG_SETPRIO(3);
        float pf[poly_slots<M, NKS>()][NKS];
        load_poly_frags<M, NKS, false>(Pl, pf, lr, lg);
        auto diffuse_own = [&](float* buf, float* planes, int t) {
            EEG_WAVE_SYNC();
            float* g = (!SPEC && planes != nullptr) ? planes + ((size_t)t * B + b) * N * H : nullptr;
            lds_diffuse_tile<M, NKS>(buf, KAP, ct * 16, H, pf, lr, lg, g, plane_stride, N, true);
        };
        diffuse_own(A, Hpl, 0);
        f32x4 nxr0 = zero4, nxc = zero4;
        float nxr1 = 0.f;
        auto fetch_xw = [&](int t) {
            if constexpr (SPEC) return;
            const wbuf_t bx = make_wbuf(XW + ((size_t)t * B + b) * N * (3 * H));
            nxr0 = wbuf_ld4(bx, oxw0, 0u);
            nxr1 = wbuf_ld(bx, oxw1, 0u);
            nxc = wbuf_ld4(bx, oxw0 + 2 * H, 0u);
        };
        fetch_xw(0);
        pp.stamp(1);
        pp.last = PROBE ? cycle_now() : 0;
        ClockSample cs;
        const bool cs_me = !PROBE && b == 0 && tid == 0;
        cs.begin(probe, cs_me);
        constexpr int QSA = KS / 4 / M;
        f32x4 rc[5] = {zero4, zero4, zero4, zero4, zero4};
        f32x4 ra = zero4;
        bool pre_r = false;
        for (int t = 0; t < T; ++t) {
            const size_t s = (size_t)t * B + b;
            f32x4 ar[1][2] = {{nxr0, (f32x4){nxr1, 0.f, 0.f, 0.f}}}, ac[1][2] = {{nxc, zero4}};
            const unsigned so = (unsigned)(s * N * H);
            EEG_LDS_BARRIER();
            pp.mark(0);
            if constexpr (SPEC) {
                ar[0][0] = ld4(XR + lds_sw(lr, col, UST));
                ar[0][1][0] = XRr[ct * 64 + lane];
                if (M > 1 && pre_r) ra += ar[0][0];
            }

            if (M > 1 && pre_r) {
                ar[0][0] = ra;
                mfma_nodes32<1, KS, true, 0, 0, false, true, true, (M > 1 ? QSA : 0)>(A, KAP, lane, lr, lg, w0, ar, rc);
            } else
                mfma_nodes32<1, KS, true, 0, 0, false, true, true>(A, KAP, lane, lr, lg, w0, ar);
            pp.mark(1);
            {
                const f32x4 rg = sigmoid4_(ar[0][0]);
                f32x4 rh = rg * ld4(A + lds_sw(lr, col, KAP));
                rh = valid[0] ? rh : zero4;
                st4(A2 + lds_sw(lr, col, KAP), rh);
                const float rg1 = sigmoidf_(ar[0][1][0]);
                const float rh1 = valid1 ? rg1 * A[l1] : 0.f;
                A2[l1] = rh1;
                if (save && valid[0]) {
                    wbuf_st4(bR, oh0, so, rg);
                    wbuf_st4(bRH, oh0, so, rh);
                }
                if (save && valid1) {
                    wbuf_st1(bR, oh1, so, rg1);
                    wbuf_st1(bRH, oh1, so, rh1);
                }
            }
            pp.mark(2);
            diffuse_own(A2, RHpl, t);
            pp.mark(7);
            EEG_LDS_BARRIER();
            pp.mark(3);
            if (t + 1 < T) fetch_xw(t + 1);
            if constexpr (SPEC) ac[0][0] = ld4(XC + (t & 1) * (16 * UST) + lds_sw(lr, col, UST));
            mfma_nodes32<1, KS, true, 1>(A2, KAP, lane, lr, lg, w1, ac);
            pp.mark(4);
            {
                const f32x4 u = ld4(U + lds_sw(lr, col, UST)), h = ld4(A + lds_sw(lr, col, KAP));
                const f32x4 c = act == 0 ? tanh4_(ac[0][0]) : relu4_(ac[0][0]);
                f32x4 hn = u * h + (1.f - u) * c;
                hn = valid[0] ? hn : zero4;
                st4(A + lds_sw(lr, col, KAP), hn);
                if (valid[0]) {
                    wbuf_st4(bH, oh0, so, hn);
                    if (save) wbuf_st4(bC, oh0, so, c);
                }
            }
            pp.mark(5);
            EEG_LDS_BARRIER();
            if (t + 1 < T || (!SPEC && Hpl != nullptr)) diffuse_own(A, Hpl, t + 1);
            pre_r = M > 1 && t + 1 < T;
            if (pre_r) {
                ra = SPEC ? zero4 : nxr0;
                rc[0] = rc[1] = rc[2] = rc[3] = rc[4] = zero4;
                f32x4 rr4[4] = {zero4, zero4, zero4, zero4};
                mfma_tile_quads<KS, 0, QSA>(A, KAP, lane, lr, lg, w0[0], ra, rc[4], rr4);
                rc[0] = rr4[0]; rc[1] = rr4[1]; rc[2] = rr4[2]; rc[3] = rr4[3];
            }
            pp.mark(6);
        }
        cs.end(probe, cs_me);
        pp.stamp(2);
    } else {
        f32x4 nxu0 = zero4;
        float nxu1 = 0.f, nxc1 = 0.f;
        float ux[NKS], ux4[NKS], ut[NKS], ut4[NKS], yv[3][NKS];
        const unsigned vyb = (unsigned)lg * (unsigned)spec_Sp * (3 * H) + ct * 16 + lr;
        const unsigned vy4 = (unsigned)(16 + lg < N ? 16 + lg : N - 1) * (unsigned)spec_Sp * (3 * H) + ct * 16 + lr;
        const wbuf_t bY = make_wbuf(XW), bHh = make_wbuf(Hpl != nullptr ? Hpl : Hseq), bRHh = make_wbuf(RHpl != nullptr ? RHpl : Hseq);
        const unsigned oe0 = (unsigned)lr * (unsigned)spec_SpE * H + col, oe1 = (unsigned)node1 * (unsigned)spec_SpE * H + col1;
        const unsigned or0 = (unsigned)lr * (unsigned)spec_Sp * H + col, or1 = (unsigned)node1 * (unsigned)spec_Sp * H + col1;
        if constexpr (SPEC) {
            load_spec_frags<NKS>(spec_U, N, lane, ut, ut4);
#pragma unroll
            for (int ks = 0; ks < NKS; ++ks) {
                const int i = 4 * ks + lg, j4 = 16 + (lane & 3);
                ux[ks] = (i < N && lr < N) ? spec_U[lr * N + i] : 0.f;
                ux4[ks] = (i < N && j4 < N) ? spec_U[j4 * N + i] : 0.f;
            }
        }
        auto fetch_y = [&](int t) {
            const unsigned so = (unsigned)(((size_t)t * B + b) * (3 * H));
#pragma unroll
            for (int g = 0; g < 3; ++g)
#pragma unroll
                for (int ks = 0; ks < NKS; ++ks)
                    yv[g][ks] = ks < 4 ? wbuf_ld(bY, vyb + g * H, so + (unsigned)(4 * ks) * (unsigned)spec_Sp * (3 * H)) : wbuf_ld(bY, vy4 + g * H, so);
        };
        auto xw_mix = [&](int tn) {
            f32x4 acc[3] = {zero4, zero4, zero4}, rem[3] = {zero4, zero4, zero4}, rem2[3] = {zero4, zero4, zero4};
#pragma unroll
            for (int ks = 0; ks < NKS; ++ks)
#pragma unroll
                for (int g = 0; g < 3; ++g) acc[g] = mfma16(yv[g][ks], ux[ks], acc[g]);
#pragma unroll
            for (int ks = 0; ks < NKS; ++ks)
#pragma unroll
                for (int g = 0; g < 3; ++g) {
                    if (ks & 1) rem2[g] = mfma4(ux4[ks], yv[g][ks], rem2[g]);
                    else rem[g] = mfma4(ux4[ks], yv[g][ks], rem[g]);
                }
            f32x4 t0 = rem[0] + rem2[0], t1 = rem[1] + rem2[1], t2 = rem[2] + rem2[2];
            EEG_PIN(t0); EEG_PIN(t1); EEG_PIN(t2);
            st4(XR + lds_sw(lr, col, UST), acc[0]);
            st4(XC + (tn & 1) * (16 * UST) + lds_sw(lr, col, UST), acc[2]);
            XRr[ct * 64 + lane] = rem4_reduce(t0);
            nxu0 = acc[1];
            nxu1 = rem4_reduce(t1);
            nxc1 = rem4_reduce(t2);
        };
        auto export_tile = [&](const float* tile, wbuf_t out, unsigned o0, unsigned o1, unsigned row) {
            const float* const tl[1] = {tile};
            const int strd[1] = {KAP}, scol[1] = {ct * 16}, gcol[1] = {0};
            spec_mix_tiles_out<NKS, 1>(tl, strd, scol, gcol, ut, ut4, lr, lg, out, o0, o1, row * H, valid[0], valid1);
        };
        auto fetch_x = [&](int t) {
            if constexpr (SPEC) { fetch_y(t); return; }
            const wbuf_t bx = make_wbuf(XW + ((size_t)t * B + b) * N * (3 * H));
            nxu0 = wbuf_ld4(bx, oxw0 + H, 0u);
            nxu1 = wbuf_ld(bx, oxw1 + H, 0u);
            nxc1 = wbuf_ld(bx, oxw1 + 2 * H, 0u);
        };
        fetch_x(0);
        if constexpr (SPEC) {
            xw_mix(0);
        }
        constexpr int QS = KS / 4 / M;
        f32x4 ua = zero4, ub = zero4, urem[4] = {zero4, zero4, zero4, zero4};
        float ux1 = 0.f;
        bool pre = false;
        for (int t = 0; t < T; ++t) {
            const size_t s = (size_t)t * B + b;
            f32x4 au[1][2] = {{nxu0, (f32x4){nxu1, 0.f, 0.f, 0.f}}}, ac[1][2] = {{zero4, (f32x4){nxc1, 0.f, 0.f, 0.f}}};
            const unsigned so = (unsigned)(s * N * H);
            EEG_LDS_BARRIER();
            if (!pre) {
                ua = nxu0; ub = zero4; ux1 = nxu1;
                urem[0] = urem[1] = urem[2] = urem[3] = zero4;
            }
            if (t + 1 < T) fetch_x(t + 1);
            if (!pre) mfma_tile_quads<KS, 0, QS>(A, KAP, lane, lr, lg, w0[0], ua, ub, urem);
            mfma_tile_quads<KS, QS, KS / 4>(A, KAP, lane, lr, lg, w0[0], ua, ub, urem);
            {
                f32x4 tt = (urem[0] + urem[1]) + (urem[2] + urem[3]);
                EEG_PIN(tt);
                au[0][0] = ua + ub;
                au[0][1][0] = ux1 + rem4_reduce(tt);
            }
            float u1;
            {
                const f32x4 u0 = sigmoid4_(au[0][0]);
                u1 = sigmoidf_(au[0][1][0]);
                st4(U + lds_sw(lr, col, UST), u0);
                if (save && valid[0]) wbuf_st4(bU, oh0, so, u0);
            }
            if constexpr (SPEC) {
                if (Hpl != nullptr) export_tile(A, bHh, oe0, oe1, (unsigned)s);
            }
            EEG_LDS_BARRIER();
            if constexpr (SPEC) ac[0][1][0] += mfma_rem4_ldsw<KS>(A2, KAP, lane, lg, W1L + ct * (KS / 4) * 256);
            else mfma_nodes32<1, KS, true, 2, 0, false, false, true>(A2, KAP, lane, lr, lg, w1, ac);
            {
                const float h1 = A[l1];
                const float c1 = act == 0 ? tanhf_(ac[0][1][0]) : fmaxf(ac[0][1][0], 0.f);
                const float hn1 = valid1 ? u1 * h1 + (1.f - u1) * c1 : 0.f;
                A[l1] = hn1;
                if (valid1) {
                    wbuf_st1(bH, oh1, so, hn1);
                    if (save) {
                        wbuf_st1(bC, oh1, so, c1);
                        wbuf_st1(bU, oh1, so, u1);
                    }
                }
            }
            if constexpr (SPEC) {
                if (RHpl != nullptr) export_tile(A2, bRHh, or0, or1, (unsigned)s);
            }
            EEG_LDS_BARRIER();
#ifdef EEG_X_BPRE
            pre = t + 1 < T;
#else
            pre = !SPEC && t + 1 < T;
#endif
            if constexpr (SPEC) {
                if (!pre && t + 1 < T) xw_mix(t + 1);
            }
            if (pre) {
                ua = SPEC ? zero4 : nxu0; ub = zero4; ux1 = SPEC ? 0.f : nxu1;
                urem[0] = urem[1] = urem[2] = urem[3] = zero4;
                mfma_tile_quads<KS, 0, QS>(A, KAP, lane, lr, lg, w0[0], ua, ub, urem);
                if constexpr (SPEC) {
                    xw_mix(t + 1);
                    ua += nxu0;
                    ux1 = nxu1;
                }
            }
        }
        if constexpr (SPEC) {
            if (Hpl != nullptr) export_tile(A, bHh, oe0, oe1, (unsigned)((size_t)T * B + b));
        }
    }
    };
    if constexpr (SPEC) {
        if (role == 0) { for (int b = blockIdx.x; b < B; b += gridDim.x) clip(b, SeqIdx<0>()); }
        else { for (int b = blockIdx.x; b < B; b += gridDim.x) clip(b, SeqIdx<1>()); }
    } else {
        for (int b = blockIdx.x; b < B; b += gridDim.x) clip(b, SeqIdx<-1>());
    }
    if (role == 0) pp.dump(probe, 0);
}

template <int H, int M, int NKS, bool PROBE = false>
__global__ __launch_bounds__(256, 1) void seq_bwd_kernel(
    const float* __restrict__ Hseq, const float* __restrict__ h0, const float* __restrict__ Rs,
    const float* __restrict__ Us, const float* __restrict__ Cs, const float* __restrict__ dHseq,
    const float* __restrict__ d_at_end, const float* __restrict__ d_at_len, const long long* __restrict__ lengths,
    const float* __restrict__ P, int p_batched, const float* __restrict__ b1p, const float* __restrict__ b2p,
    float* __restrict__ dXW, float* __restrict__ dh0, float* __restrict__ dbias_part, int T, int B, int N, int act,
    long long* probe) {
    using G = SeqGeom<H, M>;
    constexpr int KAP = G::KAP, KS = G::KS, KGP = G::KGP, KSG = G::KSG, CT = G::CT, NCT = G::NCT;
    PhaseProbe<PROBE> pp;
    pp.start();
    EEG_DYN_SMEM(sm);
    float* Pl = sm;
    constexpr int ROWS = seq_bwd_rows(H, M, NKS);
    float* EC = Pl + (M - 1) * kPFloats;
    float* EG = EC + ROWS * KAP;
    constexpr bool REM4 = NKS == 5;
    const int tid = threadIdx.x, lane = tid & 63, wave = tid >> 6, lr = lane & 15, lg = lane >> 4;

    float w1[CT][KS], w2[CT][KSG];
#pragma unroll
    for (int i = 0; i < CT; ++i) {
        const int ct = wave + 4 * i < NCT ? wave + 4 * i : 0;
#pragma unroll
        for (int ks = 0; ks < KS; ++ks) w1[i][ks] = b1p[((size_t)ks * NCT + ct) * 64 + lane];
#pragma unroll
        for (int ks = 0; ks < KSG; ++ks) w2[i][ks] = b2p[((size_t)ks * NCT + ct) * 64 + lane];
    }
    for (int b = blockIdx.x; b < B; b += gridDim.x) {
    __syncthreads();
    for (int e = tid; e < ROWS * (KAP + KGP); e += 256) EC[e] = 0.f;
    lds_load_polys(Pl, P, p_batched ? b : 0, M, N);
    int t_len = -1;
    if (d_at_len != nullptr) {
        t_len = lengths != nullptr ? (int)lengths[b] - 1 : T - 1;
        t_len = t_len < 0 ? 0 : (t_len >= T ? T - 1 : t_len);
    }
    __syncthreads();
    float pf[poly_slots<M, NKS>()][NKS];
    load_poly_frags<M, NKS, true>(Pl, pf, lr, lg);

    const int node[2] = {lr, 16 + lr};
    const bool valid[2] = {lr < N, 16 + lr < N};
    const int nodec[2] = {valid[0] ? lr : N - 1, valid[1] ? 16 + lr : N - 1};
    const f32x4 zero4 = {0.f, 0.f, 0.f, 0.f};
    int oh[CT][2], oxw[CT][2];
    bool own[CT];
    const int node1 = 16 + lg;
    const bool valid1 = node1 < N;
    int lc1[CT], lg1[CT], lu1[CT];
#pragma unroll
    for (int i = 0; i < CT; ++i) {
        own[i] = wave + 4 * i < NCT;
        const int ct = own[i] ? wave + 4 * i : 0;
#pragma unroll
        for (int nt = 0; nt < 2; ++nt) {
            oh[i][nt] = nodec[nt] * H + ct * 16 + 4 * lg;
            oxw[i][nt] = node[nt] * (3 * H) + ct * 16 + 4 * lg;
        }
        if (REM4) {
            oh[i][1] = (valid1 ? node1 : N - 1) * H + ct * 16 + lr;
            oxw[i][1] = node1 * (3 * H) + ct * 16 + lr;
            lc1[i] = lds_sw(node1, ct * 16 + lr, KAP);
            lg1[i] = lds_sw(node1, ct * 16 + lr, KGP);
            lu1[i] = lds_sw(node1, H + ct * 16 + lr, KGP);
        }
    }

    f32x4 dh[CT][2], sb_r[CT], sb_u[CT], sb_c[CT];
    float sb1_r[CT], sb1_u[CT], sb1_c[CT];
#pragma unroll
    for (int i = 0; i < CT; ++i) {
        dh[i][0] = zero4;
        dh[i][1] = zero4;
        sb_r[i] = sb_u[i] = sb_c[i] = zero4;
        sb1_r[i] = sb1_u[i] = sb1_c[i] = 0.f;
    }

    const size_t tstride = (size_t)B * N * H;
    const size_t boff = (size_t)b * N * H;
    f32x4 nh[CT][2], nr[CT][2], nu[CT][2], nc[CT][2], ng[CT][2];
    auto fetch = [&](int t) {
        const size_t so = (size_t)t * tstride + boff;
        const float* hs = t > 0 ? Hseq + (so - tstride) : (h0 != nullptr ? h0 + boff : nullptr);
#pragma unroll
        for (int i = 0; i < CT; ++i)
#pragma unroll
            for (int nt = 0; nt < 2; ++nt) {
                const int o = oh[i][nt];
                if (REM4 && nt == 1) {
                    nh[i][1] = (f32x4){hs != nullptr ? hs[o] : 0.f, 0.f, 0.f, 0.f};
                    nr[i][1] = (f32x4){Rs[so + o], 0.f, 0.f, 0.f};
                    nu[i][1] = (f32x4){Us[so + o], 0.f, 0.f, 0.f};
                    nc[i][1] = (f32x4){Cs[so + o], 0.f, 0.f, 0.f};
                    float g1 = dHseq != nullptr ? dHseq[so + o] : 0.f;
                    if (d_at_end != nullptr && t == T - 1) g1 += d_at_end[boff + o];
                    if (t == t_len) g1 += d_at_len[boff + o];
                    ng[i][1] = (f32x4){g1, 0.f, 0.f, 0.f};
                    continue;
                }
                nh[i][nt] = hs != nullptr ? ld4(hs + o) : zero4;
                nr[i][nt] = ld4(Rs + so + o);
                nu[i][nt] = ld4(Us + so + o);
                nc[i][nt] = ld4(Cs + so + o);
                f32x4 g = dHseq != nullptr ? ld4(dHseq + so + o) : zero4;
                if (d_at_end != nullptr && t == T - 1) g += ld4(d_at_end + boff + o);
                if (t == t_len) g += ld4(d_at_len + boff + o);
                ng[i][nt] = g;
            }
    };
    fetch(T - 1);
    for (int t = T - 1; t >= 0; --t) {
        float* dxw = dXW + ((size_t)t * B + b) * N * (3 * H);
// ... 423 lines not shown
```

eeg_gnn_ssl_amd/csrc/seq_inst.cpp:

```cpp
#include "kernels_seq.h"
#include "prof.h"
#include "seq_launch.h"

#ifndef EEG_SEQ_H
#error "compile with -DEEG_SEQ_H=<hidden units>"
#endif
#define EEG_CAT2(a, b) a##b
#define EEG_CAT(a, b) EEG_CAT2(a, b)

namespace eeg {
namespace {

template <int H, int M, int NKS, bool PROBE>
int run_fwd1(const SeqPlan& p, const SeqFwdArgs& a, hipStream_t st) {
    EEG_SET_MAX_LDS((seq_fwd_kernel<H, M, NKS, PROBE>), p.lds);
    EEG_LAUNCH_P("seq_fwd", (seq_fwd_kernel<H, M, NKS, PROBE>), dim3(p.grid), dim3(p.block), p.lds, st, a.XW, a.h0, a.P, a.p_batched, a.bhg, a.bhc,
                 a.Hseq, a.Rs, a.Us, a.Cs, a.RHs, a.Hpl, a.RHpl, a.plane_stride, a.T, a.B, a.N, a.act, a.probe);
    return hipGetLastError() == hipSuccess ? 0 : 1;
}
template <int H, int M, int NKS, bool PROBE, bool SPEC>
int run_fwd2(const SeqPlan& p, const SeqFwdArgs& a, hipStream_t st) {
    EEG_SET_MAX_LDS((seq_fwd2_kernel<H, M, NKS, PROBE, SPEC>), p.lds);
    EEG_LAUNCH_P("seq_fwd", (seq_fwd2_kernel<H, M, NKS, PROBE, SPEC>), dim3(p.grid), dim3(p.block), p.lds, st, a.XW, a.h0, a.P, a.p_batched, a.bhg,
                 a.bhc, a.Hseq, a.Rs, a.Us, a.Cs, a.RHs, a.Hpl, a.RHpl, a.plane_stride, a.T, a.B, a.N, a.act, a.probe, a.spec_U, a.spec_Sp, a.spec_SpE);
    return hipGetLastError() == hipSuccess ? 0 : 1;
}
template <int H, int M, int NKS, bool PROBE>
int run_bwd1(const SeqPlan& p, const SeqBwdArgs& a, hipStream_t st) {
    EEG_SET_MAX_LDS((seq_bwd_kernel<H, M, NKS, PROBE>), p.lds);
    EEG_LAUNCH_P("seq_bwd", (seq_bwd_kernel<H, M, NKS, PROBE>), dim3(p.grid), dim3(p.block), p.lds, st, a.Hseq, a.h0, a.Rs, a.Us, a.Cs, a.dHseq,
                 a.d_at_end, a.d_at_len, a.lengths, a.P, a.p_batched, a.b1, a.b2, a.dXW, a.dh0, a.dbias_part, a.T, a.B, a.N, a.act, a.probe);
    return hipGetLastError() == hipSuccess ? 0 : 1;
}
template <int H, int M, int NKS, bool PROBE, bool SPEC>
int run_bwd2(const SeqPlan& p, const SeqBwdArgs& a, hipStream_t st) {
    EEG_SET_MAX_LDS((seq_bwd2_kernel<H, M, NKS, PROBE, SPEC>), p.lds);
    EEG_LAUNCH_P("seq_bwd", (seq_bwd2_kernel<H, M, NKS, PROBE, SPEC>), dim3(p.grid), dim3(p.block), p.lds, st, a.Hseq, a.h0, a.Rs, a.Us, a.Cs, a.dHseq,
                 a.d_at_end, a.d_at_len, a.lengths, a.P, a.p_batched, a.b1, a.b2, a.dXW, a.dh0, a.dbias_part, a.T, a.B, a.N, a.act, a.probe,
                 a.spec_U, a.dYh, a.spec_Sp);
    return hipGetLastError() == hipSuccess ? 0 : 1;
}

template <int H, int M, int NKS>
int fwd_nks(const SeqPlan& p, const SeqFwdArgs& a, hipStream_t st) {
    if constexpr (seq_has_probe(H, M, NKS)) {
        if (p.probe && p.kind == SeqKind::OneWave) return run_fwd1<H, M, NKS, true>(p, a, st);
        if (p.probe && p.kind == SeqKind::TwoWave) return run_fwd2<H, M, NKS, true, false>(p, a, st);
        if (p.probe) return run_fwd2<H, M, NKS, true, true>(p, a, st);
    }
    if constexpr (seq_has_spec(H, M, NKS)) {
        if (p.kind == SeqKind::TwoWaveSpec) return run_fwd2<H, M, NKS, false, true>(p, a, st);
    }
    if constexpr (seq_has_two_wave(H, M, NKS)) {
        if (p.kind == SeqKind::TwoWave) return run_fwd2<H, M, NKS, false, false>(p, a, st);
    }
    return run_fwd1<H, M, NKS, false>(p, a, st);
}
template <int H, int M>
int fwd_one(const SeqPlan& p, const SeqFwdArgs& a, hipStream_t st) {
    return p.nks == 5 ? fwd_nks<H, M, 5>(p, a, st) : fwd_nks<H, M, 8>(p, a, st);
}
template <int H, int M, int NKS>
int bwd_nks(const SeqPlan& p, const SeqBwdArgs& a, hipStream_t st) {
    if constexpr (seq_has_probe(H, M, NKS)) {
        if (p.probe && p.kind == SeqKind::OneWave) return run_bwd1<H, M, NKS, true>(p, a, st);
        if (p.probe && p.kind == SeqKind::TwoWave) return run_bwd2<H, M, NKS, true, false>(p, a, st);
        if (p.probe) return run_bwd2<H, M, NKS, true, true>(p, a, st);
    }
    if constexpr (seq_has_spec(H, M, NKS)) {
        if (p.kind == SeqKind::TwoWaveSpec) return run_bwd2<H, M, NKS, false, true>(p, a, st);
    }
    if constexpr (seq_has_two_wave(H, M, NKS)) {
        if (p.kind == SeqKind::TwoWave) return run_bwd2<H, M, NKS, false, false>(p, a, st);
    }
    return run_bwd1<H, M, NKS, false>(p, a, st);
}
template <int H, int M>
int bwd_one(const SeqPlan& p, const SeqBwdArgs& a, hipStream_t st) {
    return p.nks == 5 ? bwd_nks<H, M, 5>(p, a, st) : bwd_nks<H, M, 8>(p, a, st);
}

}

int EEG_CAT(launch_seq_fwd_h, EEG_SEQ_H)(int M, const SeqPlan& p, const SeqFwdArgs& a, hipStream_t st) {
    switch (M) {
        case 1: return fwd_one<EEG_SEQ_H, 1>(p, a, st);
        case 2: return fwd_one<EEG_SEQ_H, 2>(p, a, st);
        case 3: return fwd_one<EEG_SEQ_H, 3>(p, a, st);
        case 4: return fwd_one<EEG_SEQ_H, 4>(p, a, st);
        case 5: return fwd_one<EEG_SEQ_H, 5>(p, a, st);
        case 7: return fwd_one<EEG_SEQ_H, 7>(p, a, st);
        default: return 1;
    }
}
int EEG_CAT(launch_seq_bwd_h, EEG_SEQ_H)(int M, const SeqPlan& p, const SeqBwdArgs& a, hipStream_t st) {
    switch (M) {
        case 1: return bwd_one<EEG_SEQ_H, 1>(p, a, st);
        case 2: return bwd_one<EEG_SEQ_H, 2>(p, a, st);
        case 3: return bwd_one<EEG_SEQ_H, 3>(p, a, st);
        case 4: return bwd_one<EEG_SEQ_H, 4>(p, a, st);
        case 5: return bwd_one<EEG_SEQ_H, 5>(p, a, st);
        case 7: return bwd_one<EEG_SEQ_H, 7>(p, a, st);
        default: return 1;
    }
}

}
```

eeg_gnn_ssl_amd/csrc/seq_launch.h:

```cpp
#pragma once
#include "kernels_seq.h"

namespace eeg {

struct SeqFwdArgs {
    const float *XW, *h0, *P;
    int p_batched;
    const float *bhg, *bhc;
    float *Hseq, *Rs, *Us, *Cs, *RHs;
    float *Hpl, *RHpl;
    size_t plane_stride;
    int T, B, N, act;
    long long* probe;
    const float* spec_U = nullptr;
    int spec_Sp = 0, spec_SpE = 0;
};
struct SeqBwdArgs {
    const float *Hseq, *h0, *Rs, *Us, *Cs, *dHseq, *d_at_end, *d_at_len;
    const long long* lengths;
    const float* P;
    int p_batched;
    const float *b1, *b2;
    float *dXW, *dh0, *dbias_part;
    int T, B, N, act;
    long long* probe;
    const float* spec_U = nullptr;
    float* dYh = nullptr;
    int spec_Sp = 0;
};

enum class SeqKind { OneWave, TwoWave, TwoWaveSpec, Stream };
enum SeqPlanError { kSeqOk = 0, kSeqNoKernel, kSeqNoFit };
struct SeqPlan {
    SeqKind kind;
    bool probe;
    int nks, block, grid;
    size_t lds;
    int error;
};
struct SeqCall {
    int H, M, N, T, B;
    size_t plane_stride = 0;
    bool spectral = false;
    int Sp = 0, SpE = 0;
    int knob_one_wave = 0;
    int knob_no_spec = 0;
    int knob_stream = 0;
    bool probe = false;
};

constexpr bool seq_h_supported(int H) { return H == 16 || H == 32 || H == 64; }
constexpr bool seq_m_supported(int M) { return M == 1 || M == 2 || M == 3 || M == 4 || M == 5 || M == 7; }
inline bool seq_desc_reaches(double floats) { return floats * sizeof(float) < 2147483648.0; }
inline bool seq_spec_applies(const SeqCall& c, int nks) {
    return seq_has_spec(c.H, c.M, nks) && c.spectral && c.knob_no_spec == 0 && c.N >= 16 && seq_desc_reaches((double)c.T * c.B * c.N * 3 * c.H) &&
           seq_desc_reaches((double)c.N * c.Sp * 3 * c.H) && seq_desc_reaches((double)c.N * c.SpE * c.H) && (!c.probe || seq_has_probe(c.H, c.M, nks));
}
inline bool seq_probe_applies(const SeqCall& c, const SeqPlan& p) {
    return c.probe && seq_has_probe(c.H, c.M, p.nks) && (p.kind != SeqKind::OneWave || c.knob_one_wave != 0);
}
constexpr int kSeqMaxGrid = 256;
constexpr int kStreamGrid = 512;

inline SeqPlan seq_fwd_plan(const SeqCall& c) {
    SeqPlan p{SeqKind::OneWave, false, seq_nks(c.N), 256, c.B < kSeqMaxGrid ? c.B : kSeqMaxGrid, 0, kSeqOk};
    if (!seq_h_supported(c.H) || !seq_m_supported(c.M)) { p.error = kSeqNoKernel; return p; }
    p.lds = seq_fwd_lds_floats(c.H, c.M) * sizeof(float);
    if (p.lds > kMaxLdsBytes) { p.error = kSeqNoFit; return p; }
    if (seq_has_two_wave(c.H, c.M, p.nks) && c.knob_one_wave == 0 && seq_desc_reaches((double)c.T * c.B * c.N * c.H) &&
        seq_desc_reaches((double)(c.M - 1) * c.plane_stride)) {
        p.kind = seq_spec_applies(c, p.nks) ? SeqKind::TwoWaveSpec : SeqKind::TwoWave;
        p.block = 512;
        p.lds = seq_fwd2_lds_floats(c.H, c.M, p.kind == SeqKind::TwoWaveSpec) * sizeof(float);
    }
    p.probe = seq_probe_applies(c, p);
    return p;
}
inline SeqPlan seq_bwd_plan(const SeqCall& c) {
    SeqPlan p{SeqKind::OneWave, false, seq_nks(c.N), 256, c.B < kSeqMaxGrid ? c.B : kSeqMaxGrid, 0, kSeqOk};
    if (!seq_h_supported(c.H) || !seq_m_supported(c.M)) { p.error = kSeqNoKernel; return p; }
    const bool dxw_reached = seq_desc_reaches((double)c.T * c.B * c.N * 3 * c.H);
    const size_t lds_stream = seq_stream_bwd_lds_floats(c.M) * sizeof(float);
    if (c.knob_one_wave == 0 && !c.probe && seq_has_stream(c.H, c.M) && c.N <= kDecRows && c.knob_stream != 2 &&
        (c.knob_stream == 1 || (c.M >= 4 && c.B >= 384)) && 2 * lds_stream <= kMaxLdsBytes && dxw_reached) {
        p.kind = SeqKind::Stream;
        p.grid = c.B < kStreamGrid ? c.B : kStreamGrid;
        p.lds = lds_stream;
        return p;
    }
    if (seq_has_two_wave(c.H, c.M, p.nks) && c.knob_one_wave == 0 && dxw_reached) {
        p.kind = seq_spec_applies(c, p.nks) ? SeqKind::TwoWaveSpec : SeqKind::TwoWave;
        p.block = 512;
        p.lds = seq_bwd2_lds_floats(c.H, c.M) * sizeof(float);
    } else {
        p.lds = seq_bwd_lds_floats(c.H, c.M, seq_bwd_rows(c.H, c.M, p.nks)) * sizeof(float);
        if (p.lds > kMaxLdsBytes) p.error = kSeqNoFit;
    }
    p.probe = seq_probe_applies(c, p);
    return p;
}

int launch_seq_fwd_h16(int M, const SeqPlan& p, const SeqFwdArgs& a, hipStream_t st);
int launch_seq_fwd_h32(int M, const SeqPlan& p, const SeqFwdArgs& a, hipStream_t st);
int launch_seq_fwd_h64(int M, const SeqPlan& p, const SeqFwdArgs& a, hipStream_t st);
int launch_seq_bwd_h16(int M, const SeqPlan& p, const SeqBwdArgs& a, hipStream_t st);
int launch_seq_bwd_h32(int M, const SeqPlan& p, const SeqBwdArgs& a, hipStream_t st);
int launch_seq_bwd_h64(int M, const SeqPlan& p, const SeqBwdArgs& a, hipStream_t st);
int launch_seq_bwd_stream(int M, const SeqPlan& p, const SeqBwdArgs& a, hipStream_t st);
struct DecFwdArgs;
struct DecBwdArgs;
int launch_dec_fwd_persist(int M, const DecFwdArgs& a, size_t lds, hipStream_t st);
int launch_dec_bwd_persist(int M, int dt, const DecBwdArgs& a, size_t lds, hipStream_t st);


}
```

eeg_gnn_ssl_amd/csrc/spec_inst.cpp:

```cpp
#include "kernels_gemm_g.h"
#include "kernels_gemm_f.h"
#include "kernels_spectral.h"
#include "pack_cell.h"
#include "spec_launch.h"
#include "prof.h"

namespace eeg {

constexpr int kMaxPackJobs = 8;
struct PackJob {
    const float *Wg, *bg, *Wc, *bc, *basis;
    float* out;
    int spectral;
    CellPack cp;
    SpecPack sp;
};
struct PackJobs { PackJob j[kMaxPackJobs]; };
__global__ void pack_cells_kernel(PackJobs jobs) {
    const PackJob& jb = jobs.j[blockIdx.y];
    if (jb.spectral) pack_spectral_body(jb.Wg, jb.Wc, jb.basis, jb.out, jb.sp, (int)blockIdx.x, (int)gridDim.x);
    else pack_cell_body(jb.Wg, jb.bg, jb.Wc, jb.bc, jb.out, jb.cp, (int)blockIdx.x, (int)gridDim.x);
}


// ... 35 lines not shown
        }
    }
    EEG_LAUNCH_P("pack_cell", pack_cells_kernel, dim3(256, n), dim3(256), 0, st, jobs);
    return hipGetLastError() == hipSuccess ? 0 : 2;
}

int launch_spec_mix(int to_nodes, const float* in, const float* basis, const float* bias, int N, int T, int B, int F, int bm,
                    float* out, hipStream_t st, const char* tag, int node_rows) {
    const int S = T * B, Sp = node_rows > 0 ? node_rows : spec_rows(S), F4 = F / 4;
#ifndef EEG_X_MIX_VALU
    if (N <= 32 && F % 32 == 0 && (double)(to_nodes ? Sp : S) * (F / 32) < 2.0e9) {
        const int units = (to_nodes ? Sp : S) * ceil_div(F, 32);
        int nb = ceil_div(units, 4);
        if (nb > 2048) nb = 2048;
        if (N <= 20) {
            if (to_nodes) EEG_LAUNCH_P(tag, (spec_mix_mfma_kernel<0, 10>), dim3(nb), dim3(256), 0, st, in, basis, bias, N, S, Sp, F, bm, T, B, out);
            else EEG_LAUNCH_P(tag, (spec_mix_mfma_kernel<1, 10>), dim3(nb), dim3(256), 0, st, in, basis, bias, N, S, Sp, F, bm, T, B, out);
        } else {
            if (to_nodes) EEG_LAUNCH_P(tag, (spec_mix_mfma_kernel<0, 16>), dim3(nb), dim3(256), 0, st, in, basis, bias, N, S, Sp, F, bm, T, B, out);
            else EEG_LAUNCH_P(tag, (spec_mix_mfma_kernel<1, 16>), dim3(nb), dim3(256), 0, st, in, basis, bias, N, S, Sp, F, bm, T, B, out);
        }
        return hipGetLastError() == hipSuccess ? 0 : 2;
    }
#endif
    if (N == 19 && F4 <= 128) {
        int threads = 256;
        while (threads > 64 && (threads / 2) >= F4 && (threads / 2) / F4 >= Sp) threads /= 2;
        const int SPW = threads / F4;
        int nb = ceil_div(to_nodes ? Sp : S, SPW);
        if (nb > 1024) nb = 1024;
        if (to_nodes) EEG_LAUNCH_P(tag, spec_mix_in_kernel<19>, dim3(nb), dim3(threads), 0, st, in, basis, S, Sp, F, bm, T, B, out);
        else EEG_LAUNCH_P(tag, spec_mix_out_kernel<19>, dim3(nb), dim3(threads), 0, st, in, basis, bias, S, Sp, F, bm, T, B, out);
    } else {
        const size_t total = (size_t)(to_nodes ? Sp : S) * N * F4;
        int nb = (int)((total + 255) / 256 > 2048 ? 2048 : (total + 255) / 256);
        EEG_LAUNCH_P(tag, spec_mix_generic_kernel, dim3(nb), dim3(256), (size_t)N * N * sizeof(float), st, in, basis, bias, N, S, Sp, F, bm,
                     T, B, to_nodes, out);
    }
    return hipGetLastError() == hipSuccess ? 0 : 2;
}

int launch_spec_zero_rows(float* Xh, int N, int S, int Sp, int F, hipStream_t st) {
    if (Sp <= S) return 0;
    EEG_LAUNCH_P("zero", spec_zero_pad_kernel, dim3(ceil_div(N * (Sp - S) * F, 256)), dim3(256), 0, st, Xh, N, S, Sp, F);
    return hipGetLastError() == hipSuccess ? 0 : 2;
}
int launch_spec_zero_pad(float* Xh, int N, int S, int F, hipStream_t st) { return launch_spec_zero_rows(Xh, N, S, spec_rows(S), F, st); }

int launch_nng(const float* A, int F, int Sp, int G, const float* Wq, size_t wstride, int nct, float* C, int num_cus, hipStream_t st,
               const char* tag, const float* bias, const float* gscale, size_t a_gstride) {
    const unsigned ags = (unsigned)(a_gstride != 0 ? a_gstride : (size_t)Sp * F);
    const size_t lds = nng_lds_bytes(nct / 4);
    const int RT = (Sp / 16) * G;
    int Gw = 2 * (num_cus > 0 ? num_cus : 256);
    if (Gw > ceil_div(RT, 8)) Gw = ceil_div(RT, 8);
    if (Gw < 1) Gw = 1;
    if (nct == 12) {
        EEG_SET_MAX_LDS((gemm_nng_kernel<3, 2>), lds);
        EEG_LAUNCH_P(tag, (gemm_nng_kernel<3, 2>), dim3(Gw), dim3(256), lds, st, A, ags, F, Sp, G, Wq, (unsigned)wstride, C, 16 * nct, bias, gscale);
    } else if (nct == 4) {
        EEG_SET_MAX_LDS((gemm_nng_kernel<1, 2>), lds);
        EEG_LAUNCH_P(tag, (gemm_nng_kernel<1, 2>), dim3(Gw), dim3(256), lds, st, A, ags, F, Sp, G, Wq, (unsigned)wstride, C, 16 * nct, bias, gscale);
    } else {
        return 1;
    }
    return hipGetLastError() == hipSuccess ? 0 : 2;
}

TngPlan tng_plan(int F, int Sp, int G, int num_cus) {
    TngPlan p{};
    if (F < 4 || F % 4 != 0 || Sp < 16 || Sp % 16 != 0 || G < 1) return p;
    if (F == 64) {
        p.planar = 1; p.KT = 2; p.nkb = 1;
    } else {
        int best = 5, bcost = 1 << 30, bnkb = 1;
        for (int kt = 5; kt >= 4; --kt) {
            const int nkb = ceil_div(F, 32 * kt), cost = nkb * 32 * kt;
            if (cost < bcost) { best = kt; bcost = cost; bnkb = nkb; }
        }
        p.KT = best; p.nkb = bnkb;
    }
    const int target = 2 * (num_cus > 0 ? num_cus : 256);
    int spg = target / (G * p.nkb);
    if (spg < 1) spg = 1;
    int rps = round_up(ceil_div(Sp, spg), 16);
    if (rps < 64) rps = 64;
    if (rps > Sp) rps = Sp;
    p.rps = rps;
    p.spg = ceil_div(Sp, rps);
    p.ok = 1;
    return p;
}

namespace {
template <int KT, bool PLANAR>
int launch_tng_one(const TngPlan& p, const float* A, int F, int Sp, int G, const float* dY, float* partial, hipStream_t st, const char* tag,
                   long long skew) {
    constexpr int RC = 16, OT = 6;
    const size_t lds = 3 * (size_t)(RC * 32 * (KT + OT)) * sizeof(float);
    SegPtrs segs;
    for (int m = 0; m < kMaxM; ++m) segs.p[m] = m == 0 ? A : nullptr;
    EEG_SET_MAX_LDS((gemm_tnq_grouped_kernel<KT, OT, RC, PLANAR>), lds);
    EEG_LAUNCH_P(tag, (gemm_tnq_grouped_kernel<KT, OT, RC, PLANAR>), dim3(p.nkb, G * p.spg), dim3(256), lds, st, segs, F, Sp, G, p.spg, dY, 192,
                 0, 192, partial, p.rps, skew);
    return hipGetLastError() == hipSuccess ? 0 : 2;
}
}

int launch_tng_pair(const TngPlan& p, const float* Ah, const float* Arh, int Sp, int G, const float* dY, float* part_g, float* part_c,
                    hipStream_t st, const char* tag, size_t ah_gstride) {
    if (!p.ok || !p.planar || p.KT != 2 || p.nkb != 1) return 1;
    const long long skew = ah_gstride != 0 ? (long long)ah_gstride - (long long)Sp * 64 : 0;
    constexpr int RC = 16, KT = 2;
    const size_t lds = 3 * (size_t)(RC * 32 * (KT + 4)) * sizeof(float);
    TnqJob ja, jb;
    for (int m = 0; m < kMaxM; ++m) { ja.segs.p[m] = m == 0 ? Ah : nullptr; jb.segs.p[m] = m == 0 ? Arh : nullptr; }
    ja.ycol0 = 0; ja.Ov = 128; ja.partial = part_g;
    jb.ycol0 = 128; jb.Ov = 64; jb.partial = part_c;
    EEG_SET_MAX_LDS((gemm_tnq_grouped_pair_kernel<KT, RC, true>), lds);
    EEG_LAUNCH_P(tag, (gemm_tnq_grouped_pair_kernel<KT, RC, true>), dim3(1, 2 * G * p.spg), dim3(256), lds, st, ja, jb, 64, Sp, G, p.spg, dY, 192,
                 p.rps, skew, (long long)0);
    return hipGetLastError() == hipSuccess ? 0 : 2;
}

namespace {
template <int KQ, bool SWZ>
int launch_nnf_one(const float* A, size_t ags, int K, int Sp, int G, const float* Wr, size_t wstride, float* C, int num_cus, hipStream_t st,
                   const char* tag, const float* bias, const float* gscale) {
    const size_t lds = nnf_lds_bytes(K);
    const int total = G * ceil_div(Sp, 64);
    int nb = 2 * (num_cus > 0 ? num_cus : 256);
    if (nb > total) nb = total;
    EEG_SET_MAX_LDS((gemm_nnf_kernel<KQ, SWZ>), lds);
    EEG_LAUNCH_P(tag, (gemm_nnf_kernel<KQ, SWZ>), dim3(nb), dim3(256), lds, st, A, (long long)ags, K, Sp, G, Wr, (unsigned)wstride, C, bias, gscale);
    return hipGetLastError() == hipSuccess ? 0 : 2;
}
}
int launch_nnf(const float* A, size_t a_gstride, int K, int Sp, int G, const float* Wr, size_t wstride, float* C, int num_cus, hipStream_t st,
               const char* tag, const float* bias, const float* gscale) {
    if (K < 4 || K % 4 != 0 || Sp < 16 || G < 1 || (double)Sp * 192 * 4 >= 2.0e9) return -1;
    const size_t ags = a_gstride != 0 ? a_gstride : (size_t)Sp * K;
    const int kq = ceil_div(K, 8);
    const bool odd = ((K / 4) & 1) != 0;
#define EEG_NNF(KQ, SWZ) return launch_nnf_one<KQ, SWZ>(A, ags, K, Sp, G, Wr, wstride, C, num_cus, st, tag, bias, gscale)
    if (K == 64) EEG_NNF(8, true);
    if (odd && kq == 13) EEG_NNF(13, false);
    if (odd && kq == 9) EEG_NNF(9, false);
    if (odd && kq == 5) EEG_NNF(5, false);
    if (odd && kq == 2) EEG_NNF(2, false);
#undef EEG_NNF
    return -1;
}

int launch_dxf(const float* dYh, int Sp, int S, int N, int Fin, const float* Wtq, size_t wstride, const float* basis, float* dX,
               hipStream_t st, const char* tag) {
    if (Fin != 64 || N < 1 || N > kDxfMaxN || Sp < 16 || S < 1 || S > Sp) return -1;
    if ((double)Sp * 192 * 4 >= 2147483648.0 || (double)S * N * 64 * 4 >= 2147483648.0) return -1;
    const size_t lds = dxf_lds_bytes();
    if (N == 19) {
        EEG_SET_MAX_LDS(gemm_dxf_kernel<19>, lds);
        EEG_LAUNCH_P(tag, gemm_dxf_kernel<19>, dim3(ceil_div(Sp, kDxfRows)), dim3(256), lds, st, dYh, Sp, S, N, Wtq, (unsigned)wstride, basis, dX);
    } else {
        EEG_SET_MAX_LDS(gemm_dxf_kernel<0>, lds);
        EEG_LAUNCH_P(tag, gemm_dxf_kernel<0>, dim3(ceil_div(Sp, kDxfRows)), dim3(256), lds, st, dYh, Sp, S, N, Wtq, (unsigned)wstride, basis, dX);
    }
    return hipGetLastError() == hipSuccess ? 0 : 2;
}

TnfPlan tnf_plan(int Fin, int H, int Sp, int G, int num_cus) {
    TnfPlan p{};
    if (H != 64 || Fin < 4 || Fin % 4 != 0 || Fin > 128 || Sp < 16 || Sp % 16 != 0 || G < 1) return p;
    if ((double)Sp * 192 * 4 >= 2147483648.0) return p;
    p.fxt = ceil_div(Fin, 32);
#ifdef EEG_X_TNF_TARGET1
    const int target = 1 * (num_cus > 0 ? num_cus : 256);
#else
    const int target = tnf_wgs_per_cu(p.fxt) * (num_cus > 0 ? num_cus : 256);
#endif
    int spg = target / G;
    if (spg < 1) spg = 1;
    int rps = round_up(ceil_div(Sp, spg), 16);
    if (rps < 64) rps = 64;
    if (rps > Sp) rps = Sp;
    p.rps = rps;
    p.spg = ceil_div(Sp, rps);
    p.ok = 1;
    return p;
}
namespace {
template <int FXT>
int launch_tnf_one(const TnfPlan& p, const float* Xh, size_t xgs, int Fin, const float* Hh, size_t hgs, const float* RHh, const float* dY,
                   int Sp, int G, float* part_x, float* part_g, float* part_c, hipStream_t st, const char* tag) {
    const size_t lds = tnf_lds_bytes(FXT);
    EEG_SET_MAX_LDS((gemm_tnf_kernel<FXT>), lds);
    EEG_LAUNCH_P(tag, (gemm_tnf_kernel<FXT>), dim3(G * p.spg), dim3(256), lds, st, Xh, (long long)xgs, Fin, Hh, (long long)hgs, RHh, dY, Sp,
                 p.spg, p.rps, part_x, part_g, part_c);
    return hipGetLastError() == hipSuccess ? 0 : 2;
}
}
int launch_tnf(const TnfPlan& p, const float* Xh, size_t x_gstride, int Fin, const float* Hh, size_t h_gstride, const float* RHh,
               const float* dY, int Sp, int G, float* part_x, float* part_g, float* part_c, hipStream_t st, const char* tag) {
    if (!p.ok) return 1;
    const size_t xgs = x_gstride != 0 ? x_gstride : (size_t)Sp * Fin, hgs = h_gstride != 0 ? h_gstride : (size_t)Sp * 64;
    switch (p.fxt) {
        case 1: return launch_tnf_one<1>(p, Xh, xgs, Fin, Hh, hgs, RHh, dY, Sp, G, part_x, part_g, part_c, st, tag);
        case 2: return launch_tnf_one<2>(p, Xh, xgs, Fin, Hh, hgs, RHh, dY, Sp, G, part_x, part_g, part_c, st, tag);
        case 3: return launch_tnf_one<3>(p, Xh, xgs, Fin, Hh, hgs, RHh, dY, Sp, G, part_x, part_g, part_c, st, tag);
        case 4: return launch_tnf_one<4>(p, Xh, xgs, Fin, Hh, hgs, RHh, dY, Sp, G, part_x, part_g, part_c, st, tag);
    }
    return 1;
}

int launch_tng(const TngPlan& p, const float* A, int F, int Sp, int G, const float* dY, float* partial, hipStream_t st, const char* tag,
               size_t a_gstride) {
    if (!p.ok) return 1;
    const long long skew = a_gstride != 0 ? (long long)a_gstride - (long long)Sp * F : 0;
    if (p.planar) return launch_tng_one<2, true>(p, A, F, Sp, G, dY, partial, st, tag, skew);
    if (p.KT == 4) return launch_tng_one<4, false>(p, A, F, Sp, G, dY, partial, st, tag, skew);
    return launch_tng_one<5, false>(p, A, F, Sp, G, dY, partial, st, tag, skew);
}

}
```

eeg_gnn_ssl_amd/csrc/spec_launch.h:

```cpp
#pragma once
#include "kernels_gemm.h"

namespace eeg {

bool spec_supported(int T, int B, int N, int H, int Fin, int M, int need_dx);

size_t spec_pack_floats(int Fin, int H, int M, int N);
int launch_spec_basis(const float* S, int N, float* basis, hipStream_t st);
int launch_spec_pack(const float* Wg, const float* Wc, const float* basis, int Fin, int H, int M, int N, float* spack, hipStream_t st);

int launch_pack_cells(int n_cells, const float* const* Wg, const float* const* bg, const float* const* Wc, const float* const* bc,
                      const int* Fin, int H, int M, float* const* packs, const float* basis, int N, float* const* spacks, hipStream_t st);

int launch_spec_mix(int to_nodes, const float* in, const float* basis, const float* bias, int N, int T, int B, int F, int bm,
                    float* out, hipStream_t st, const char* tag, int node_rows = 0);

int launch_spec_zero_pad(float* Xh, int N, int S, int F, hipStream_t st);

int launch_nng(const float* A, int F, int Sp, int G, const float* Wq, size_t wstride, int nct, float* C, int num_cus,
               hipStream_t st, const char* tag, const float* bias = nullptr, const float* gscale = nullptr, size_t a_gstride = 0);

struct TngPlan { int ok, KT, planar, nkb, spg, rps; };
TngPlan tng_plan(int F, int Sp, int G, int num_cus);
int launch_tng(const TngPlan& p, const float* A, int F, int Sp, int G, const float* dY, float* partial, hipStream_t st, const char* tag,
               size_t a_gstride = 0);
int launch_tng_pair(const TngPlan& p, const float* Ah, const float* Arh, int Sp, int G, const float* dY, float* part_g, float* part_c,
                    hipStream_t st, const char* tag, size_t ah_gstride = 0);
int launch_nnf(const float* A, size_t a_gstride, int K, int Sp, int G, const float* Wr, size_t wstride, float* C, int num_cus, hipStream_t st,
               const char* tag, const float* bias, const float* gscale);
int launch_dxf(const float* dYh, int Sp, int S, int N, int Fin, const float* Wtq, size_t wstride, const float* basis, float* dX,
               hipStream_t st, const char* tag);
struct TnfPlan { int ok, fxt, spg, rps; };
TnfPlan tnf_plan(int Fin, int H, int Sp, int G, int num_cus);
int launch_tnf(const TnfPlan& p, const float* Xh, size_t x_gstride, int Fin, const float* Hh, size_t h_gstride, const float* RHh,
               const float* dY, int Sp, int G, float* part_x, float* part_g, float* part_c, hipStream_t st, const char* tag);
int launch_spec_zero_rows(float* Xh, int N, int S, int Sp, int F, hipStream_t st);

}
```

eeg_gnn_ssl_amd/ops.py:

```python
from __future__ import annotations

import ctypes
from typing import List, Optional, Sequence, Tuple

import torch

from . import _lib
from ._lib import DecoderDims, LayerDims

ACT_CODES = {"tanh": 0, "relu": 1, None: 1}
NS = "eeg_dcrnn"
_libdef = torch.library.Library(NS, "DEF")


import os as _os

GEMM_MODE = 1 if _os.environ.get("EEG_DCRNN_SPLIT_BF16", "0") not in ("", "0") else 0


def set_gemm_mode(mode: int) -> int:
    global GEMM_MODE
    if mode not in (0, 1):
        raise ValueError("gemm mode must be 0 (fp32 MFMA) or 1 (three-term bf16 split)")
    prev, GEMM_MODE = GEMM_MODE, int(mode)
# ... 330 lines not shown


_define("dconv", "(Tensor x, Tensor P, int p_batched, Tensor weight, Tensor biases) -> Tensor", _dconv_impl,
        lambda x, p, p_batched, weight, biases: x.new_empty((x.shape[0], x.shape[1], weight.shape[1])))
_define("dconv_bwd", "(Tensor dout, Tensor x, Tensor P, int p_batched, Tensor weight, bool need_dx) -> (Tensor, Tensor, Tensor)",
        _dconv_bwd_impl,
        lambda dout, x, p, p_batched, weight, need_dx: (x.new_empty(x.shape if need_dx else (0,)), torch.empty_like(weight),
                                                        x.new_empty((weight.shape[1],))))


def _dconv_setup(ctx, inputs, output):
    x, p, p_batched, weight, _ = inputs
    ctx.save_for_backward(x, p, weight)
    ctx.p_batched = p_batched


def _dconv_backward(ctx, dout):
    x, p, weight = ctx.saved_tensors
    dx, dw, db = torch.ops.eeg_dcrnn.dconv_bwd(dout, x, p, ctx.p_batched, weight, ctx.needs_input_grad[0])
    return (dx if ctx.needs_input_grad[0] else None), None, None, dw, db


torch.library.register_autograd(f"{NS}::dconv", _dconv_backward, setup_context=_dconv_setup, lib=_libdef)


class GradSink:

    def __init__(self, params: Sequence[torch.Tensor]):
        self.params = list(params)
        self.armed = False
        self.written = [False] * len(self.params)
        for i, p in enumerate(self.params):
            p._eeg_grad_sink = (self, i)

    def __enter__(self):
        self.armed = True
        self.written = [False] * len(self.params)
        return self

    def __exit__(self, *exc):
        self.armed = False
        return False

    @staticmethod
    def take(param: torch.Tensor) -> Optional[torch.Tensor]:
        ref = getattr(param, "_eeg_grad_sink", None)
        if ref is None:
            return None
        sink, i = ref
        tgt = param.grad
        if (not sink.armed or sink.written[i] or sink.params[i] is not param or tgt is None or not tgt.is_contiguous()
                or tgt.shape != param.shape):
            return None
        sink.written[i] = True
        return tgt


def _layer_dims(t_len, b, n, h, fin, m, act, p_batched, planes_ready):
    dims = LayerDims(t_len, b, n, h, fin, m, act, p_batched)
    if planes_ready:
        dims.x_planes_ready = 1
        dims.x_plane_stride = (t_len + 1) * b * n * fin
    return dims


def _dcgru_layer_impl(x, x_off: int, h0, p, p_batched: int, wg, bg, wc, bc, lengths, x_planes, n: int, h: int, m: int,
                      act: int, save: bool, want_hsel: bool, basis=None, pack=None, spack=None):
    lib = _lib.get_lib()
    if x.dim() != 4 or x.shape[2] != n:
        raise RuntimeError(f"inputs have shape {tuple(x.shape)}, expected (T, B, num_nodes={n}, input_dim)")
    t_len, b, fin = x.shape[0] - x_off, x.shape[1], x.shape[3]
    if not lib.query("eeg_dcrnn_supported", n, h, fin, m):
        raise RuntimeError("eeg_gnn_ssl_amd: " + lib.last_error())
    _check_polys(p, p_batched, b, n, m)
    if lengths is not None:
        _check_lengths(lengths, b)
    if h0 is not None and h0.numel() != b * n * h:
        raise RuntimeError(f"initial_hidden_state has shape {tuple(h0.shape)}, expected ({b}, {n * h})")
    ready = x_planes is not None
    spec = basis is not None
    dims = _layer_dims(t_len, b, n, h, fin, m, act, p_batched, ready)
    if spec:
        _check(lib, basis, "basis")
        sp_rows = int(lib.query("eeg_dcrnn_spectral_rows", t_len * b))
        if ready:
            dims.x_plane_stride = (b + sp_rows) * fin
        if p_batched or basis.numel() != _spectral_basis_floats(n) or not lib.query("eeg_dcrnn_spectral_ok", ctypes.byref(dims), 0):
            raise RuntimeError("dcgru_layer: the spectral form needs one shared support (p_batched = 0) and a shape "
                               "eeg_dcrnn_spectral_ok accepts")
        if ready and tuple(x_planes.shape) != (n, b + sp_rows, fin):
            raise RuntimeError(f"x_planes has shape {tuple(x_planes.shape)}, expected {(n, b + sp_rows, fin)} (the layer below's U^T h)")
    empty = _new((0,), p)
    xsrc, xtm = None, None
    bm = 0
    if not x.is_contiguous() and x_off == 0 and not ready and x.transpose(0, 1).is_contiguous():
        bm = 2 if spec else lib.query("eeg_dcrnn_batch_major_ok", ctypes.byref(dims))
    if bm:
        xsrc = x.transpose(0, 1)
        _check(lib, xsrc, "inputs")
        if bm == 2:
            dims.x_batch_major = 1
            xk = xsrc
        else:
            xtm = _new((t_len, b, n, fin), x)
            xk = xtm
    else:
        if not x.is_contiguous():
            xtm = x.contiguous()
            x = xtm
        _check(lib, x, "inputs")
        xk = x[x_off:] if x_off else x
    if h0 is not None:
        h0 = h0.contiguous()
        _check(lib, h0, "initial_hidden_state")
    _check(lib, p, "P")
    pack_given, spack_given = pack is not None, spack is not None
    if pack is None:
        pack = torch.ops.eeg_dcrnn.pack_cell(wg, bg, wc, bc, fin, h, m)
    elif pack.numel() < _pack_base_floats(fin, h, m):
        raise RuntimeError(f"dcgru_layer: pack has {pack.numel()} floats, a cell of input_dim={fin}, num_units={h}, num_matrices={m} needs "
                           f"{_pack_base_floats(fin, h, m)}")
    _set_pack3(dims, pack, fin, h, m)
    s = t_len * b
    if spec:
        if spack is None:
            spack = torch.ops.eeg_dcrnn.pack_cell_spectral(wg, wc, basis, fin, h, m, n)
        elif spack.numel() != lib.query("eeg_dcrnn_spectral_pack_floats", fin, h, m, n):
            raise RuntimeError(f"dcgru_layer: spack has {spack.numel()} floats, expected {lib.query('eeg_dcrnn_spectral_pack_floats', fin, h, m, n)}")
        dims.spectral, dims.spack = basis.data_ptr(), spack.data_ptr()
        if ready:
            _check(lib, x_planes, "x_planes")
            planes, planes_ptr = _new((0,), p), x_planes.data_ptr() + 4 * b * fin
        else:
            planes = _new((n, sp_rows, fin), x)
            planes_ptr = planes.data_ptr()
    elif ready:
        _check(lib, x_planes, "x_planes")
        if tuple(x_planes.shape) != (m - 1, t_len + 1, b, n, fin):
            raise RuntimeError(f"x_planes has shape {tuple(x_planes.shape)}, expected {(m - 1, t_len + 1, b, n, fin)}")
        planes, planes_ptr = _new((0,), p), x_planes.data_ptr() + 4 * b * n * fin
    else:
        planes = _new((m - 1, s, n, fin), x)
        planes_ptr = planes.data_ptr()
    hext = _new((t_len + 1, b, n * h), x)
    if save:
        rs, us, cs, rhs = (_new((t_len, b, n * h), x) for _ in range(4))
        if spec:
            hpl, rhpl = _new((n, b + sp_rows, h), x), _new((n, sp_rows, h), x)
        else:
            hpl, rhpl = (_new((m - 1, t_len + 1, b, n, h), x) for _ in range(2))
    else:
        rs = us = cs = rhs = hpl = rhpl = None
    ws = _new((lib.query("eeg_dcrnn_layer_fwd_ws_floats", ctypes.byref(dims)),), x)
    lib.call("eeg_dcrnn_layer_fwd", ctypes.byref(dims), _p(xsrc if xsrc is not None else xk), _p(xtm) if (xsrc is not None and bm != 2) else None,
             _p(h0), _p(p), _p(pack), planes_ptr, _p(hext), _p(rs), _p(us), _p(cs), _p(rhs), _p(hpl), _p(rhpl), _p(ws), _stream(x))
    if lengths is not None:
        lengths = lengths.to(device=x.device, dtype=torch.int64).contiguous()
        hsel = _new((b, n * h), x)
        lib.call("eeg_dcrnn_gather_last", _p(hext[1:]), _p(lengths), t_len, b, n * h, _p(hsel), _stream(x))
    elif want_hsel:
        hsel = hext[t_len].clone()
    else:
        hsel = _new((0,), x)
    if not save:
        return hext, hsel, []
    return hext, hsel, [xtm if xtm is not None else empty, _new((0,), p) if pack_given else pack, planes, rs, us, cs, rhs, hpl, rhpl,
                        _new((0,), p) if (spack_given or not spec) else spack]


def _dcgru_layer_fake(x, x_off, h0, p, p_batched, wg, bg, wc, bc, lengths, x_planes, n, h, m, act, save, want_hsel, basis=None,
                      pack=None, spack=None):
    t_len, b, fin = x.shape[0] - x_off, x.shape[1], x.shape[3]
    ne = lambda *shape: x.new_empty(shape)
    hext, hsel = ne(t_len + 1, b, n * h), (ne(b, n * h) if (want_hsel or lengths is not None) else ne(0))
    if not save:
        return hext, hsel, []
    zero_copy = False
    spec = basis is not None
    if not x.is_contiguous() and x_off == 0 and x_planes is None and x.transpose(0, 1).is_contiguous():
        dims = _layer_dims(t_len, b, n, h, fin, m, act, p_batched, False)
        zero_copy = spec or _lib.get_lib().query("eeg_dcrnn_batch_major_ok", ctypes.byref(dims)) == 2
    xtm = ne(t_len, b, n, fin) if (not x.is_contiguous() and not zero_copy) else ne(0)
    planes = ne(0) if x_planes is not None else ne(m - 1, t_len * b, n, fin)
    spack_in, spack = spack, ne(0)
    byp = [ne(m - 1, t_len + 1, b, n, h) for _ in range(2)]
    if spec:
        lib = _lib.get_lib()
        sp_rows = int(lib.query("eeg_dcrnn_spectral_rows", t_len * b))
        if x_planes is None:
            planes = ne(n, sp_rows, fin)
        if spack_in is None:
            spack = ne(int(lib.query("eeg_dcrnn_spectral_pack_floats", fin, h, m, n)))
        byp = [ne(n, b + sp_rows, h), ne(n, sp_rows, h)]
    return hext, hsel, [xtm, ne(0) if pack is not None else ne(_pack_floats(fin, h, m)), planes] + [ne(t_len, b, n * h) for _ in range(4)] + byp + [spack]


def _dcgru_layer_bwd_impl(d_hext, d_hsel, x, x_off: int, p, p_batched: int, pack, planes, x_planes, hext, rs, us, cs, rhs,
                          hpl, rhpl, lengths, has_h0: bool, n: int, h: int, m: int, act: int, need_dx: bool, need_dh0: bool,
                          dwg, dbg, dwc, dbc, basis=None, spack=None):
    lib = _lib.get_lib()
    t_len, b, fin = hext.shape[0] - 1, hext.shape[1], x.shape[3]
    ready = x_planes is not None
    dims = _layer_dims(t_len, b, n, h, fin, m, act, p_batched, ready)
    if not x.is_contiguous():
        if not x.transpose(0, 1).is_contiguous():
            raise RuntimeError("dcgru_layer_bwd: x must be contiguous or the transposed view of a batch-major tensor")
        dims.x_batch_major = 1
    planes_ptr = x_planes.data_ptr() + 4 * b * n * fin if ready else planes.data_ptr()
    _set_pack3(dims, pack, fin, h, m)
    if basis is not None:
        if ready:
            dims.x_plane_stride = x_planes.shape[1] * fin
            planes_ptr = x_planes.data_ptr() + 4 * b * fin
        if spack is None or not lib.query("eeg_dcrnn_spectral_ok", ctypes.byref(dims), 1 if need_dx else 0):
            raise RuntimeError("dcgru_layer_bwd: the spectral form does not cover this call (input gradient of a layer whose "
                               "input width is not 64?)")
        dims.spectral, dims.spack = basis.data_ptr(), spack.data_ptr()
    state = b * n * h
    if d_hext is not None:
        d_hext = d_hext.contiguous()
        _check(lib, d_hext, "grad of hext")
    if d_hsel is not None:
        d_hsel = d_hsel.contiguous()
    d_hseq_ptr = ctypes.c_void_p(d_hext.data_ptr() + 4 * state) if d_hext is not None else None
    d_at_end = d_hsel if lengths is None else None
    d_at_len = d_hsel if lengths is not None else None
    xk_ptr = ctypes.c_void_p(x.data_ptr() + 4 * x_off * b * n * fin)
    dx = _new((t_len + x_off, b, n, fin), hext) if need_dx else _new((0,), hext)
    if need_dx and x_off:
        lib.call("eeg_dcrnn_zero", _p(dx), 4 * x_off * b * n * fin, _stream(dx))
    dx_ptr = ctypes.c_void_p(dx.data_ptr() + 4 * x_off * b * n * fin) if need_dx else None
    dh0 = _new((b, n * h), hext) if (need_dh0 and has_h0) else _new((0,), hext)
    ws = _new((lib.query("eeg_dcrnn_layer_bwd_ws_floats", ctypes.byref(dims), 1 if need_dx else 0),), hext)
    lib.call("eeg_dcrnn_layer_bwd", ctypes.byref(dims), xk_ptr, _p(p), _p(pack), planes_ptr, _p(hext), _p(rs),
             _p(us), _p(cs), _p(rhs), _p(_none_if_empty(hpl)), _p(_none_if_empty(rhpl)), d_hseq_ptr, _p(d_at_end), _p(d_at_len), _p(lengths), dx_ptr,
             _p(dh0) if dh0.numel() else None, _p(dwg), _p(dbg), _p(dwc), _p(dbc), _p(ws), _stream(hext))
    return dx, dh0


def _dcgru_layer_bwd_fake(d_hext, d_hsel, x, x_off, p, p_batched, pack, planes, x_planes, hext, rs, us, cs, rhs, hpl, rhpl,
                          lengths, has_h0, n, h, m, act, need_dx, need_dh0, dwg, dbg, dwc, dbc, basis=None, spack=None):
    t_len, b, fin = hext.shape[0] - 1, hext.shape[1], x.shape[3]
    return (hext.new_empty((t_len + x_off, b, n, fin) if need_dx else (0,)),
            hext.new_empty((b, n * h) if (need_dh0 and has_h0) else (0,)))


_define("dcgru_layer",
        "(Tensor x, int x_off, Tensor? h0, Tensor P, int p_batched, Tensor wg, Tensor bg, Tensor wc, Tensor bc, Tensor? lengths, "
        "Tensor? x_planes, int n, int h, int m, int act, bool save, bool want_hsel, Tensor? basis, Tensor? pack=None, Tensor? spack=None) -> "
        "(Tensor hext, Tensor hsel, Tensor[] saved)",
        _dcgru_layer_impl, _dcgru_layer_fake)
_define("dcgru_layer_bwd",
        "(Tensor? d_hext, Tensor? d_hsel, Tensor x, int x_off, Tensor P, int p_batched, Tensor pack, Tensor planes, Tensor? x_planes, "
        "Tensor hext, Tensor rs, Tensor us, Tensor cs, Tensor rhs, Tensor hpl, Tensor rhpl, Tensor? lengths, bool has_h0, int n, int h, "
        "int m, int act, bool need_dx, bool need_dh0, Tensor(a!) dwg, Tensor(b!) dbg, Tensor(c!) dwc, Tensor(d!) dbc, "
        "Tensor? basis, Tensor? spack) -> (Tensor, Tensor)",
        _dcgru_layer_bwd_impl, _dcgru_layer_bwd_fake)


def _dcgru_layer_setup(ctx, inputs, output):
    (x, x_off, h0, p, p_batched, wg, bg, wc, bc, lengths, x_planes, n, h, m, act, save, want_hsel, basis, _pack, _spack) = inputs
    hext, _, saved = output
    ctx.set_materialize_grads(False)
    ctx.saved_ok = bool(save) and len(saved) == 10
    ctx.meta = (x_off, p_batched, n, h, m, act, h0 is not None)
    ctx.params = (wg, bg, wc, bc)
    if ctx.saved_ok:
        xtm = saved[0]
        lens = None if lengths is None else lengths.to(device=x.device, dtype=torch.int64).contiguous()
        kept = list(saved[1:])
        if _pack is not None:
            kept[0] = _pack
        if _spack is not None and basis is not None:
            kept[8] = _spack
        ctx.save_for_backward(xtm if xtm.numel() else x, p, x_planes, lens, basis, hext, *kept)


def _dcgru_layer_backward(ctx, d_hext, d_hsel, d_saved):
    if not ctx.saved_ok:
        raise RuntimeError("eeg_dcrnn::dcgru_layer was run with save=False: nothing was kept for the backward pass")
    xk, p, x_planes, lens, basis, hext, pack, planes, rs, us, cs, rhs, hpl, rhpl, spack = ctx.saved_tensors
    x_off, p_batched, n, h, m, act, has_h0 = ctx.meta
    need_dx, need_dh0 = ctx.needs_input_grad[0], has_h0 and ctx.needs_input_grad[2]
    fin = xk.shape[3]
    rows = (fin + h) * m
    shapes = ((rows, 2 * h), (2 * h,), (rows, h), (h,))
    sunk = [GradSink.take(q) for q in ctx.params]
    bufs = [t if t is not None else _new(sh, hext) for t, sh in zip(sunk, shapes)]
    dx, dh0 = torch.ops.eeg_dcrnn.dcgru_layer_bwd(d_hext, d_hsel, xk, x_off, p, p_batched, pack, planes, x_planes, hext,
                                                  rs, us, cs, rhs, hpl, rhpl, lens, has_h0, n, h, m, act, need_dx, need_dh0, *bufs,
                                                  basis, spack if basis is not None else None)
    ret = [None if t is not None else g for t, g in zip(sunk, bufs)]
    grads = (dx if need_dx else None, None, dh0 if need_dh0 else None, None, None, *ret, None, None, None, None, None, None, None, None,
             None, None, None)
    return grads[:len(ctx.needs_input_grad)]


torch.library.register_autograd(f"{NS}::dcgru_layer", _dcgru_layer_backward, setup_context=_dcgru_layer_setup, lib=_libdef)


def _dec_dims(meta, dropout_p=0.0, teacher_on_device=False):
    t_len, b, n, h, dout, m, n_layers, act, p_batched = meta
    return DecoderDims(t_len, b, n, h, dout, m, n_layers, act, p_batched, float(dropout_p), 1 if teacher_on_device else 0)


def _teacher_arg(lib, teacher, teacher_dev, t_len):
    if teacher_dev is not None:
        _check(lib, teacher_dev, "teacher_dev", torch.int32)
        if teacher_dev.numel() != t_len:
            raise RuntimeError(f"teacher_dev: expected int32[{t_len}], got {tuple(teacher_dev.shape)}")
        return _p(teacher_dev), teacher_dev, True
    if len(teacher) > 0 and any(teacher):
        arr = (ctypes.c_int32 * t_len)(*[1 if teacher[i] else 0 for i in range(t_len)])
        return ctypes.cast(arr, ctypes.c_void_p), arr, False
    return None, None, False


def make_rng_state(device, stream_id: int = 0) -> torch.Tensor:
    rank = 0
    if torch.distributed.is_available() and torch.distributed.is_initialized():
        rank = torch.distributed.get_rank()
    g = torch.Generator().manual_seed((torch.initial_seed() + 0x9E3779B97F4A7C15 * int(stream_id) + 0xD1B54A32D192ED03 * rank) % (1 << 63))
    seed = int(torch.randint(0, 2 ** 62, (1,), generator=g).item())
    return torch.tensor([seed, 0], dtype=torch.int64, device=device)


def _check_rng(lib, t, name):
    _check(lib, t, name, torch.int64)
    if t.numel() != 2:
        raise RuntimeError(f"{name}: expected int64[2] {{seed, offset}}, got {tuple(t.shape)}")


def _dcgru_decoder_impl(targets, h0, p, p_batched: int, wg0, bg0, wc0, bc0, wg1, bg1, wc1, bc1, wp, bp, teacher: List[int],
                        t_len: int, n: int, h: int, dout: int, m: int, n_layers: int, act: int, dropout_p: float, rng_used,
                        teacher_dev=None):
    lib = _lib.get_lib()
    if dropout_p > 0:
        if rng_used is None:
            raise RuntimeError("dcgru_decoder: dropout_p > 0 needs rng_used (ops.rng_take)")
        _check_rng(lib, rng_used, "rng_used")
    for fin in (dout, h):
        if not lib.query("eeg_dcrnn_supported", n, h, fin, m):
            raise RuntimeError("eeg_gnn_ssl_amd: " + lib.last_error())
    h0 = h0.contiguous()
    b = h0.shape[1]
    wp, bp = wp.detach().contiguous(), bp.detach().contiguous()
    for t, nm in ((h0, "initial_hidden_state"), (p, "P"), (wp, "projection_layer.weight"), (bp, "projection_layer.bias")):
        _check(lib, t, nm)
    if tuple(wp.shape) != (dout, h) or tuple(bp.shape) != (dout,):
        raise RuntimeError(f"projection_layer shapes {tuple(wp.shape)}, {tuple(bp.shape)} do not match ({dout}, {h})")
    if tuple(h0.shape) != (n_layers, b, n * h):
        raise RuntimeError(f"initial_hidden_state has shape {tuple(h0.shape)}, expected ({n_layers}, {b}, {n * h})")
    _check_polys(p, p_batched, b, n, m)
    if targets is not None and targets.numel() != t_len * b * n * dout:
        raise RuntimeError(f"decoder inputs have shape {tuple(targets.shape)}, expected ({t_len}, {b}, {n}*{dout}) "
                           f"(T, B, num_nodes * output_dim)")
    tf_ptr, tf_keep, tf_dev = _teacher_arg(lib, teacher, teacher_dev, t_len)
    use_tf = tf_ptr is not None
    if use_tf:
        if targets is None:
            raise RuntimeError("teacher forcing needs the target sequence")
        targets = targets.contiguous()
        _check(lib, targets, "inputs (teacher-forcing targets)")
    pack0 = torch.ops.eeg_dcrnn.pack_cell(wg0, bg0, wc0, bc0, dout, h, m)
    pack1 = torch.ops.eeg_dcrnn.pack_cell(wg1, bg1, wc1, bc1, h, h, m) if n_layers > 1 else _new((0,), h0)
    packs = [pack0] + [pack1] * (n_layers - 1)
    dims = _dec_dims((t_len, b, n, h, dout, m, n_layers, act, p_batched), dropout_p, tf_dev)
    out = _new((t_len, b, n * dout), h0)
    saved = _new((lib.query("eeg_dcrnn_decoder_saved_floats", ctypes.byref(dims)),), h0)
    ws = _new((lib.query("eeg_dcrnn_decoder_fwd_ws_floats", ctypes.byref(dims)),), h0)
    pk_arr = (ctypes.c_void_p * n_layers)(*[q.data_ptr() for q in packs])
    lib.call("eeg_dcrnn_decoder_fwd", ctypes.byref(dims), _p(targets) if use_tf else None, tf_ptr, _p(h0), _p(p), pk_arr,
             _p(wp), _p(bp), _p(rng_used) if dropout_p > 0 else None, _p(out), _p(saved), _p(ws), _stream(h0))
    return out, [saved, pack0, pack1]


def _dcgru_decoder_bwd_impl(d_out, p, p_batched: int, saved, pack0, pack1, wp, teacher: List[int], t_len: int, n: int, h: int,
                            dout: int, m: int, n_layers: int, act: int, dropout_p: float, rng_used,
                            dwg0, dbg0, dwc0, dbc0, dwg1, dbg1, dwc1, dbc1, dwp, dbp, teacher_dev=None):
    lib = _lib.get_lib()
    d_out = d_out.contiguous()
    _check(lib, d_out, "grad of the decoder output")
    b = d_out.shape[1]
# ... 885 lines not shown
```

include/eeg_dcrnn.h:

```cpp
#ifndef EEG_DCRNN_H
#define EEG_DCRNN_H
#include <stddef.h>
#include <stdint.h>

#ifdef __cplusplus
extern "C" {
#endif

typedef struct eeg_layer_dims {
    int32_t T, B, N, H, Fin, M;
    int32_t act;
    int32_t p_batched;
    int32_t x_planes_ready;
    int32_t x_batch_major;
    int64_t x_plane_stride;
    const uint16_t* pack3;
    const float* spectral;
    const float* spack;
} eeg_layer_dims;

typedef struct eeg_decoder_dims {
    int32_t T, B, N, H;
    int32_t Dout;
    int32_t M, L;
    int32_t act, p_batched;
    float dropout_p;
    int32_t teacher_on_device;
} eeg_decoder_dims;

const char* eeg_dcrnn_last_error(void);
int eeg_dcrnn_abi_version(void);
int eeg_dcrnn_is_device_build(void);
int eeg_dcrnn_supported(int N, int H, int Fin, int M);

int eeg_dcrnn_zero(void* p, size_t bytes, void* stream);

int eeg_dcrnn_hop_polys(const float* const* supports, int n_supports, int n_graphs, int N, int K,
                        float* P_out, void* stream);

int eeg_dcrnn_fft_features(const float* raw, int B, int N, int T, int W, const int32_t* perm,
                           const float* log_scale, float mean, float std_, float* feat_raw,
                           float* feat_std, void* stream);

int eeg_dcrnn_fft_features_pair(const float* raw_x, const float* raw_y, int B, int N, int Tx, int Ty, int W, const int32_t* perm,
                                const float* log_scale, float mean, float std_, float* feat_raw_x, float* x_std, float* y_std,
                                void* stream);

int eeg_dcrnn_augment_features(const float* x, const float* y, int B, int Tx, int Ty, int N, int D, const int32_t* perm,
                               const float* shift, float* x_out, float* y_out, void* stream);

int eeg_dcrnn_window_features(const float* raw, int B, int N, int T, int W, const int32_t* perm, const float* scale, float mean,
                              float std_, float* x_std, void* stream);

int eeg_dcrnn_window_features_pair(const float* raw_x, const float* raw_y, int B, int N, int Tx, int Ty, int W, const int32_t* perm,
                                   const float* scale, float mean, float std_, float* x_std, float* y_std, void* stream);

int eeg_dcrnn_augment_windows(const float* x, const float* y, int B, int Tx, int Ty, int N, int D, const int32_t* perm, const float* a,
                              const float* c, float* x_out, float* y_out, void* stream);

size_t eeg_dcrnn_corr_graph_ws_floats(int B, int T);
int eeg_dcrnn_corr_graph(const float* X, int B, int T, int N, int D, int top_k, float* adj, float* S1,
                         float* S2, float* ws, void* stream);

size_t eeg_dcrnn_corr_graph_rows_ws_floats(int B, int P, int Q);
int eeg_dcrnn_corr_graph_rows(const float* X, int B, int N, int P, int Q, long long piece_stride, int top_k, float* adj, float* S1,
                              float* S2, float* ws, void* stream);

size_t eeg_dcrnn_pack_floats(int Fin, int H, int M);
int eeg_dcrnn_pack_cell(const float* Wg, const float* bg, const float* Wc, const float* bc,
                        int Fin, int H, int M, float* pack, void* stream);

size_t eeg_dcrnn_pack3_halves(int Fin, int H, int M);
int eeg_dcrnn_pack_cell_bf16x3(const float* Wg, const float* Wc, int Fin, int H, int M, uint16_t* pack3, void* stream);

size_t eeg_dcrnn_spectral_basis_floats(int N);
int eeg_dcrnn_spectral_basis(const float* support, int N, float* basis, void* stream);
size_t eeg_dcrnn_spectral_pack_floats(int Fin, int H, int M, int N);
int eeg_dcrnn_pack_cell_spectral(const float* Wg, const float* Wc, const float* basis, int Fin, int H, int M, int N,
                                 float* spack, void* stream);
int eeg_dcrnn_pack_cells(int n_cells, const float* const* Wg, const float* const* bg, const float* const* Wc,
                         const float* const* bc, const int32_t* Fin, int H, int M, float* const* packs, const float* basis,
                         int N, float* const* spacks, void* stream);
int eeg_dcrnn_spectral_ok(const eeg_layer_dims* d, int need_dx);
size_t eeg_dcrnn_spectral_rows(size_t S);

int eeg_dcrnn_diffuse_fwd(const float* X, const float* P, int p_batched, int S, int B, int N, int F,
                          int M, float* planes, void* stream);
int eeg_dcrnn_diffuse_adj(const float* Z, const float* P, int p_batched, int S, int B, int N, int F,
                          int M, float* dX, void* stream);

size_t eeg_dcrnn_dconv_fwd_ws_floats(int B, int N, int F, int M, int O);
int eeg_dcrnn_dconv_fwd(const float* X, const float* P, int p_batched, int B, int N, int F, int M,
                        const float* W, const float* bias, int O, float* out, float* ws, void* stream);

size_t eeg_dcrnn_dconv_bwd_ws_floats(int B, int N, int F, int M, int O);
int eeg_dcrnn_dconv_bwd(const float* X, const float* P, int p_batched, int B, int N, int F, int M,
                        const float* W, int O, const float* dOut, float* dX, float* dW, float* dbias,
                        float* ws, void* stream);

size_t eeg_dcrnn_layer_fwd_ws_floats(const eeg_layer_dims* d);
int eeg_dcrnn_batch_major_ok(const eeg_layer_dims* d);
int eeg_dcrnn_layer_fwd(const eeg_layer_dims* d, const float* X, float* Xtm, const float* h0, const float* P,
                        const float* pack, float* planes, float* Hext, float* Rs, float* Us,
                        float* Cs, float* RHs, float* Hplanes, float* RHplanes, float* ws, void* stream);

size_t eeg_dcrnn_layer_bwd_ws_floats(const eeg_layer_dims* d, int need_dx);
int eeg_dcrnn_layer_bwd(const eeg_layer_dims* d, const float* X, const float* P, const float* pack,
                        const float* planes, const float* Hext, const float* Rs, const float* Us,
                        const float* Cs, const float* RHs, const float* Hplanes, const float* RHplanes,
                        const float* dHseq, const float* d_at_end,
                        const float* d_at_len, const int64_t* lengths, float* dX, float* dh0,
                        float* dWg, float* dbg, float* dWc, float* dbc, float* ws, void* stream);

size_t eeg_dcrnn_decoder_saved_floats(const eeg_decoder_dims* d);
size_t eeg_dcrnn_decoder_fwd_ws_floats(const eeg_decoder_dims* d);
size_t eeg_dcrnn_decoder_bwd_ws_floats(const eeg_decoder_dims* d);
int eeg_dcrnn_decoder_is_persistent(const eeg_decoder_dims* d);
int eeg_dcrnn_decoder_fwd(const eeg_decoder_dims* d, const float* targets, const int32_t* teacher,
                          const float* h0, const float* P, const float* const* packs, const float* Wp,
                          const float* bp, const uint64_t* rng_used, float* out, float* saved,
                          float* ws, void* stream);
int eeg_dcrnn_decoder_bwd(const eeg_decoder_dims* d, const int32_t* teacher, const float* P,
                          const float* const* packs, const float* Wp, const float* saved, const float* dOut,
                          const uint64_t* rng_used, float* dh0, float* const* dWg, float* const* dbg,
                          float* const* dWc, float* const* dbc, float* dWp, float* dbp, float* ws, void* stream);

int eeg_dcrnn_teacher_flags(uint64_t* rng_state, int64_t* samples_seen, int64_t increment, double cl_decay_steps, int T,
                            int32_t* flags, void* stream);

int eeg_dcrnn_augment_draw(const uint64_t* rng_used, int B, int N, const int32_t* swap_perm, int32_t* flags, int32_t* perm,
                           float* log_scale, const float* S_plain, const float* S_reflected, int n_supports, float* S_out,
                           void* stream);

int eeg_dcrnn_gather_last(const float* Htop, const int64_t* lengths, int T, int B, int NH,
                          float* last, void* stream);
int eeg_dcrnn_rng_take(uint64_t* rng_state, uint64_t groups, uint64_t* rng_used, void* stream);
int eeg_dcrnn_cls_head_fwd(const float* z, const float* W, const float* bias, int B, int N, int H,
                           int C, float dropout_p, const uint64_t* rng_used,
                           float* logits, int32_t* arg, void* stream);
int eeg_dcrnn_cls_head_bwd(const float* z, const float* W, const float* dlogits, const int32_t* arg,
                           int B, int N, int H, int C, float dropout_p, const uint64_t* rng_used,
                           float* dz, float* dW, float* dbias, void* stream);

size_t eeg_dcrnn_cls_head_loss_ws_floats(int B, int H, int C);
int eeg_dcrnn_cls_head_loss(const float* z, const float* W, const float* bias, const void* targets, int kind, int B, int N,
                            int H, int C, float dropout_p, const uint64_t* rng_used, float* logits, int32_t* arg,
                            float* dlogits, float* dz, float* dW, float* dbias, float* loss, float* ws, void* stream);
int eeg_dcrnn_dropout_mask(const uint64_t* rng_used, size_t n, float dropout_p, float* mask, void* stream);

int eeg_dcrnn_bce_logits(const float* logits, const float* y, int B, float* loss, float* dlogits, void* stream);
int eeg_dcrnn_ce_logits(const float* logits, const int64_t* y, int B, int C, float* loss, float* dlogits,
                        void* stream);
size_t eeg_dcrnn_masked_loss_ws_floats(void);
int eeg_dcrnn_masked_loss(const float* pred, const float* y, size_t n, int use_scaler, float mean, float std_,
                          float mask_val, int kind, float* loss, float* dpred, float* ws, void* stream);
size_t eeg_dcrnn_clip_adam_ws_floats(void);
int eeg_dcrnn_clip_adam(float* params, float* grads, float* exp_avg, float* exp_avg_sq, size_t n,
                        float max_norm, float lr, float beta1, float beta2, float eps, float weight_decay,
                        int step, float grad_scale, float* ws, float* norm_out, void* stream);

int eeg_dcrnn_clip_adam_dev(float* params, float* grads, float* exp_avg, float* exp_avg_sq, size_t n,
                            float max_norm, const float* lr_dev, float beta1, float beta2, float eps,
                            float weight_decay, int32_t* step_dev, float grad_scale, float* ws, float* norm_out,
                            void* stream);

#ifdef __cplusplus
}
#endif
#endif
```

Baseline: 136,500.

## Fuse last-state selection into seq forward and dX front zeroing into dxf kernel

The recurrent forward kernels now write the selected hidden state (at each sequence's last valid step) straight into the hsel buffer, which removes a separate gather launch or clone. The spectral dX GEMM kernel also zeroes the leading dX rows that the host previously cleared with a separate memset. In the spectral two-wave path the RH save store is skipped when RH planes are produced instead. Each change removes a small kernel launch and its memory pass, in exchange for more ABI fields and extra conditional stores in hot loops.

```diff
diff --git a/eeg_gnn_ssl_amd/_lib.py b/eeg_gnn_ssl_amd/_lib.py
--- a/eeg_gnn_ssl_amd/_lib.py
+++ b/eeg_gnn_ssl_amd/_lib.py
@@ -14,7 +14,8 @@
     _fields_ = [("T", c_int32), ("B", c_int32), ("N", c_int32), ("H", c_int32), ("Fin", c_int32),
                 ("M", c_int32), ("act", c_int32), ("p_batched", c_int32), ("x_planes_ready", c_int32),
                 ("x_batch_major", c_int32), ("x_plane_stride", c_int64), ("pack3", c_void_p), ("spectral", c_void_p),
-                ("spack", c_void_p)]
+                ("spack", c_void_p), ("dx_front_rows", c_int64), ("sel_lengths", c_void_p),
+                ("hsel", c_void_p)]
 
 
 class DecoderDims(ctypes.Structure):
@@ -59,6 +60,7 @@
     "eeg_dcrnn_batch_major_ok": (c_int, [POINTER(LayerDims)]),
     "eeg_dcrnn_layer_fwd": (c_int, [POINTER(LayerDims)] + [_FP] * 14 + [c_void_p]),
     "eeg_dcrnn_layer_bwd_ws_floats": (c_size_t, [POINTER(LayerDims), c_int]),
+    "eeg_dcrnn_layer_bwd_clears_dx_front": (c_int, [POINTER(LayerDims)]),
     "eeg_dcrnn_layer_bwd": (c_int, [POINTER(LayerDims)] + [_FP] * 22 + [c_void_p]),
     "eeg_dcrnn_decoder_saved_floats": (c_size_t, [POINTER(DecoderDims)]),
     "eeg_dcrnn_decoder_fwd_ws_floats": (c_size_t, [POINTER(DecoderDims)]),
diff --git a/eeg_gnn_ssl_amd/csrc/api.cpp b/eeg_gnn_ssl_amd/csrc/api.cpp
--- a/eeg_gnn_ssl_amd/csrc/api.cpp
+++ b/eeg_gnn_ssl_amd/csrc/api.cpp
@@ -691,6 +691,16 @@
     return (nn_dma_applies(d->Fin, R, 3 * d->H, k) && tn_dma_applies(d->Fin, 3 * d->H, k)) ? 2 : 1;
 }
 
+static void seq_sel_args(const eeg_layer_dims* d, const SeqPlan& plan, SeqFwdArgs& a) {
+    if (d->hsel != nullptr && seq_fwd_selects(plan.kind)) { a.lengths = reinterpret_cast<const long long*>(d->sel_lengths); a.hsel = d->hsel; }
+}
+static int seq_sel_finish(const eeg_layer_dims* d, const SeqPlan& plan, const float* Hext, hipStream_t st) {
+    if (d->hsel == nullptr || seq_fwd_selects(plan.kind)) return 0;
+    const size_t state = (size_t)d->B * d->N * d->H;
+    if (d->sel_lengths == nullptr) return copy_floats(d->hsel, Hext + (size_t)d->T * state, state, st);
+    return eeg_dcrnn_gather_last(Hext + state, d->sel_lengths, d->T, d->B, d->N * d->H, d->hsel, st);
+}
+
 int eeg_dcrnn_layer_fwd(const eeg_layer_dims* d, const float* X, float* Xtm, const float* h0, const float* P,
                         const float* pack, float* planes, float* Hext, float* Rs, float* Us, float* Cs, float* RHs,
                         float* Hplanes, float* RHplanes, float* ws, void* stream) {
@@ -732,6 +742,7 @@
         SeqCall call = seq_fwd_call(H, M, N, d->T, d->B, 0, a.probe);
         call.spectral = true; call.Sp = Sp; call.SpE = SpE;
         const SeqPlan plan = seq_fwd_plan(call);
+        seq_sel_args(d, plan, a);
         if (plan.kind == SeqKind::TwoWaveSpec) {
             a.XW = Yh; a.Hpl = Hplanes; a.RHpl = RHplanes; a.spec_U = d->spectral; a.spec_Sp = Sp; a.spec_SpE = SpE;
             if (seq_fwd(H, M, plan, a, st)) return 1;
@@ -747,6 +758,7 @@
                 if (launch_spec_mix(1, RHs, d->spectral, nullptr, N, d->T, d->B, H, 0, RHplanes, st, "spec_mix_h")) return fail("spec_mix: launch failed");
             }
         }
+        if (seq_sel_finish(d, plan, Hext, st)) return 1;
         return check_launch("layer_fwd (spectral)");
     } else if (d->x_planes_ready) {
         if (Xtm != nullptr) return fail("layer_fwd: x_planes_ready excludes a batch-major input");
@@ -763,10 +775,22 @@
     if ((Hplanes != nullptr) != (RHplanes != nullptr)) return fail("layer_fwd: Hplanes/RHplanes must be both NULL or both non-NULL");
     SeqFwdArgs a{XW, h0 != nullptr ? Hext : nullptr, P, d->p_batched, pack + p.bhg, pack + p.bhc, Hext + state, Rs, Us, Cs, RHs, Hplanes, RHplanes,
                  (size_t)(d->T + 1) * state, d->T, d->B, d->N, d->act, seq_probe_arg(st)};
-    return seq_fwd(H, M, seq_fwd_plan(seq_fwd_call(H, M, d->N, d->T, d->B, a.plane_stride, a.probe)), a, st);
+    const SeqPlan plan = seq_fwd_plan(seq_fwd_call(H, M, d->N, d->T, d->B, a.plane_stride, a.probe));
+    seq_sel_args(d, plan, a);
+    if (seq_fwd(H, M, plan, a, st)) return 1;
+    return seq_sel_finish(d, plan, Hext, st);
 }
 
 size_t eeg_dcrnn_layer_bwd_ws_floats(const eeg_layer_dims* d, int need_dx) { return layer_dims_positive(d) ? bwd_ws(d, need_dx).total : 0; }
+
+static bool bwd_dx_fused(const eeg_layer_dims* d) {
+    const int S = d->T * d->B;
+    return d->spectral != nullptr && g_tune[EEG_TUNE_SPEC_DX_PASSES] == 0 && dxf_applies(spec_rows(S), S, d->N, d->Fin, d->dx_front_rows);
+}
+int eeg_dcrnn_layer_bwd_clears_dx_front(const eeg_layer_dims* d) {
+    if (!layer_dims_positive(d) || d->spectral == nullptr || !eeg_dcrnn_spectral_ok(d, 1)) return 0;
+    return bwd_dx_fused(d) ? 1 : 0;
+}
 
 int eeg_dcrnn_layer_bwd(const eeg_layer_dims* d, const float* X, const float* P, const float* pack,
                         const float* planes, const float* Hext, const float* Rs, const float* Us, const float* Cs,
@@ -776,6 +800,8 @@
                         float* dbc, float* ws, void* stream) {
     if (check_dims(d->N, d->H, d->Fin, d->M)) return 1;
     if (d->T < 1 || d->B < 1) return fail("layer_bwd: empty sequence/batch (T=%d, B=%d)", d->T, d->B);
+    if (d->dx_front_rows != 0 && (dX == nullptr || !eeg_dcrnn_layer_bwd_clears_dx_front(d)))
+        return fail("layer_bwd: dx_front_rows=%lld where no kernel of this call clears them (eeg_dcrnn_layer_bwd_clears_dx_front)", (long long)d->dx_front_rows);
     hipStream_t st = S_(stream);
     const int S = d->T * d->B, R = S * d->N, H = d->H, M = d->M, Fin = d->Fin, N = d->N;
     const size_t state = (size_t)d->B * N * H;
@@ -817,7 +843,7 @@
         }
         if (cell_weight_grads_spectral(d, planes, xs_spec(d), hh, hh_gs, rhh, dYh, ws + w.partial, w, dWg, dWc, st, dbias, dbg, dbc)) return 1;
         if (dX != nullptr) {
-            const int dxf = g_tune[EEG_TUNE_SPEC_DX_PASSES] == 0 ? launch_dxf(dYh, Sp, S, N, Fin, d->spack + sp.sxtq, sp.sxtq_stride, d->spectral, dX, st, "gemm_dx_f") : -1;
+            const int dxf = g_tune[EEG_TUNE_SPEC_DX_PASSES] == 0 ? launch_dxf(dYh, Sp, S, N, Fin, d->spack + sp.sxtq, sp.sxtq_stride, d->spectral, dX, st, "gemm_dx_f", d->dx_front_rows) : -1;
             if (dxf > 0) return fail("gemm_dxf: launch failed");
             if (dxf < 0) {
                 float* dXh = ws + w.z;
diff --git a/eeg_gnn_ssl_amd/csrc/kernels_gemm_f.h b/eeg_gnn_ssl_amd/csrc/kernels_gemm_f.h
--- a/eeg_gnn_ssl_amd/csrc/kernels_gemm_f.h
+++ b/eeg_gnn_ssl_amd/csrc/kernels_gemm_f.h
@@ -405,7 +405,8 @@
 
 template <int NT>
 __global__ __launch_bounds__(256, 2) void gemm_dxf_kernel(const float* __restrict__ dYh, int Sp, int S, int Nrt, const float* __restrict__ Wtq,
-                                                         unsigned w_gstride, const float* __restrict__ basis, float* __restrict__ dX) {
+                                                         unsigned w_gstride, const float* __restrict__ basis, float* __restrict__ dX,
+                                                         unsigned zero_floats) {
     const int N = NT > 0 ? NT : Nrt;
     constexpr int NS = kDxfNS, ST = kDxfStage, RB = kDxfRows, PER = 6;
     EEG_DYN_SMEM(sm);
@@ -497,6 +498,11 @@
         for (int j = 0; j < kDxfMaxN; ++j)
             if (j < N) wbuf_st4(rx, rb + (unsigned)(j * 64), 0u, acc[j][t]);
     }
-}
-
-}
+    if (zero_floats != 0u) {
+        const wbuf_t rz = make_wbuf_n(dX - zero_floats, zero_floats * 4u);
+        const f32x4 z4 = {0.f, 0.f, 0.f, 0.f};
+        for (unsigned e = ((unsigned)blockIdx.x * 256u + (unsigned)tid) * 4u; e < zero_floats; e += (unsigned)gridDim.x * 1024u) wbuf_st4(rz, e, 0u, z4);
+    }
+}
+
+}
diff --git a/eeg_gnn_ssl_amd/csrc/kernels_seq.h b/eeg_gnn_ssl_amd/csrc/kernels_seq.h
--- a/eeg_gnn_ssl_amd/csrc/kernels_seq.h
+++ b/eeg_gnn_ssl_amd/csrc/kernels_seq.h
@@ -319,13 +319,19 @@
     }
 };
 
+__device__ __forceinline__ int seq_sel_step(const float* hsel, const long long* lengths, int b, int T) {
+    if (hsel == nullptr) return -1;
+    const int t = lengths != nullptr ? (int)lengths[b] - 1 : T - 1;
+    return t < 0 ? 0 : (t >= T ? T - 1 : t);
+}
+
 template <int H, int M, int NKS, bool PROBE = false>
 __global__ __launch_bounds__(256, 1) void seq_fwd_kernel(
     const float* __restrict__ XW, const float* __restrict__ h0, const float* __restrict__ P, int p_batched,
     const float* __restrict__ bhg, const float* __restrict__ bhc,
     float* __restrict__ Hseq, float* __restrict__ Rs, float* __restrict__ Us, float* __restrict__ Cs,
     float* __restrict__ RHs, float* __restrict__ Hpl, float* __restrict__ RHpl, size_t plane_stride,
-    int T, int B, int N, int act, long long* probe) {
+    int T, int B, int N, int act, long long* probe, const long long* __restrict__ lengths = nullptr, float* __restrict__ hsel = nullptr) {
     using G = SeqGeom<H, M>;
     constexpr int KAP = G::KAP, KS = G::KS, CT = G::CT, NGT = G::NGT, NCT = G::NCT;
     PhaseProbe<PROBE> pp;
@@ -351,6 +357,8 @@
     }
 
     for (int b = blockIdx.x; b < B; b += gridDim.x) {
+    const int t_sel = seq_sel_step(hsel, lengths, b, T);
+    const wbuf_t bS = make_wbuf((hsel != nullptr ? hsel : Hseq) + (size_t)b * N * H);
     __syncthreads();
     for (int e = tid; e < 2 * 32 * KAP; e += 256) A[e] = 0.f;
     lds_load_polys(Pl, P, p_batched ? b : 0, M, N);
@@ -487,6 +495,7 @@
                         if (valid1) {
                             wbuf_st1(bH, oh[i][1], 0u, hn1);
                             if (save) wbuf_st1(bC, oh[i][1], 0u, c1);
+                            if (t == t_sel) wbuf_st1(bS, oh[i][1], 0u, hn1);
                         }
                         continue;
                     }
@@ -498,6 +507,7 @@
                     if (valid[nt]) {
                         wbuf_st4(bH, oh[i][nt], 0u, hn);
                         if (save) wbuf_st4(bC, oh[i][nt], 0u, c);
+                        if (t == t_sel) wbuf_st4(bS, oh[i][nt], 0u, hn);
                     }
                 }
             }
@@ -516,7 +526,8 @@
     const float* __restrict__ bhg, const float* __restrict__ bhc,
     float* __restrict__ Hseq, float* __restrict__ Rs, float* __restrict__ Us, float* __restrict__ Cs,
     float* __restrict__ RHs, float* __restrict__ Hpl, float* __restrict__ RHpl, size_t plane_stride,
-    int T, int B, int N, int act, long long* probe, const float* __restrict__ spec_U = nullptr, int spec_Sp = 0, int spec_SpE = 0) {
+    int T, int B, int N, int act, long long* probe, const float* __restrict__ spec_U = nullptr, int spec_Sp = 0, int spec_SpE = 0,
+    const long long* __restrict__ lengths = nullptr, float* __restrict__ hsel = nullptr) {
     using G = SeqGeom<H, M>;
     PhaseProbe<PROBE> pp;
     pp.start();
@@ -534,6 +545,7 @@
     float* XRr = XC + 2 * 16 * UST;
     float* W1L = XRr + 4 * 64;
     const bool save = Rs != nullptr;
+    const bool keep_rh = !(SPEC && RHpl != nullptr);
     const int ct = wave;
     const wbuf_t bH = make_wbuf(Hseq), bR = make_wbuf(save ? Rs : Hseq), bU = make_wbuf(save ? Us : Hseq),
                  bC = make_wbuf(save ? Cs : Hseq), bRH = make_wbuf(save ? RHs : Hseq);
@@ -575,6 +587,9 @@
     const bool valid1 = node1 < N;
     const int oxw1 = (valid1 ? node1 : N - 1) * (3 * H) + col1, oh1 = (valid1 ? node1 : N - 1) * H + col1;
     const int l1 = lds_sw(node1, col1, KAP);
+    const int t_sel = seq_sel_step(hsel, lengths, b, T);
+    const wbuf_t bS = make_wbuf(hsel != nullptr ? hsel : Hseq);
+    const unsigned sel_o = (unsigned)((size_t)b * N * H);
     if (ROLE_C < 0 ? role == 0 : ROLE_C == 0) {
         EEG_SETPRIO(3);
         float pf[poly_slots<M, NKS>()][NKS];
@@ -632,11 +647,11 @@
                 A2[l1] = rh1;
                 if (save && valid[0]) {
                     wbuf_st4(bR, oh0, so, rg);
-                    wbuf_st4(bRH, oh0, so, rh);
+                    if (keep_rh) wbuf_st4(bRH, oh0, so, rh);
                 }
                 if (save && valid1) {
                     wbuf_st1(bR, oh1, so, rg1);
-                    wbuf_st1(bRH, oh1, so, rh1);
+                    if (keep_rh) wbuf_st1(bRH, oh1, so, rh1);
                 }
             }
             pp.mark(2);
@@ -657,6 +672,7 @@
                 if (valid[0]) {
                     wbuf_st4(bH, oh0, so, hn);
                     if (save) wbuf_st4(bC, oh0, so, c);
+                    if (t == t_sel) wbuf_st4(bS, oh0, sel_o, hn);
                 }
             }
             pp.mark(5);
@@ -784,6 +800,7 @@
                         wbuf_st1(bC, oh1, so, c1);
                         wbuf_st1(bU, oh1, so, u1);
                     }
+                    if (t == t_sel) wbuf_st1(bS, oh1, sel_o, hn1);
                 }
             }
             if constexpr (SPEC) {
diff --git a/eeg_gnn_ssl_amd/csrc/seq_inst.cpp b/eeg_gnn_ssl_amd/csrc/seq_inst.cpp
--- a/eeg_gnn_ssl_amd/csrc/seq_inst.cpp
+++ b/eeg_gnn_ssl_amd/csrc/seq_inst.cpp
@@ -15,14 +15,14 @@
 int run_fwd1(const SeqPlan& p, const SeqFwdArgs& a, hipStream_t st) {
     EEG_SET_MAX_LDS((seq_fwd_kernel<H, M, NKS, PROBE>), p.lds);
     EEG_LAUNCH_P("seq_fwd", (seq_fwd_kernel<H, M, NKS, PROBE>), dim3(p.grid), dim3(p.block), p.lds, st, a.XW, a.h0, a.P, a.p_batched, a.bhg, a.bhc,
-                 a.Hseq, a.Rs, a.Us, a.Cs, a.RHs, a.Hpl, a.RHpl, a.plane_stride, a.T, a.B, a.N, a.act, a.probe);
+                 a.Hseq, a.Rs, a.Us, a.Cs, a.RHs, a.Hpl, a.RHpl, a.plane_stride, a.T, a.B, a.N, a.act, a.probe, a.lengths, a.hsel);
     return hipGetLastError() == hipSuccess ? 0 : 1;
 }
 template <int H, int M, int NKS, bool PROBE, bool SPEC>
 int run_fwd2(const SeqPlan& p, const SeqFwdArgs& a, hipStream_t st) {
     EEG_SET_MAX_LDS((seq_fwd2_kernel<H, M, NKS, PROBE, SPEC>), p.lds);
     EEG_LAUNCH_P("seq_fwd", (seq_fwd2_kernel<H, M, NKS, PROBE, SPEC>), dim3(p.grid), dim3(p.block), p.lds, st, a.XW, a.h0, a.P, a.p_batched, a.bhg,
-                 a.bhc, a.Hseq, a.Rs, a.Us, a.Cs, a.RHs, a.Hpl, a.RHpl, a.plane_stride, a.T, a.B, a.N, a.act, a.probe, a.spec_U, a.spec_Sp, a.spec_SpE);
+                 a.bhc, a.Hseq, a.Rs, a.Us, a.Cs, a.RHs, a.Hpl, a.RHpl, a.plane_stride, a.T, a.B, a.N, a.act, a.probe, a.spec_U, a.spec_Sp, a.spec_SpE, a.lengths, a.hsel);
     return hipGetLastError() == hipSuccess ? 0 : 1;
 }
 template <int H, int M, int NKS, bool PROBE>
diff --git a/eeg_gnn_ssl_amd/csrc/seq_launch.h b/eeg_gnn_ssl_amd/csrc/seq_launch.h
--- a/eeg_gnn_ssl_amd/csrc/seq_launch.h
+++ b/eeg_gnn_ssl_amd/csrc/seq_launch.h
@@ -14,6 +14,8 @@
     long long* probe;
     const float* spec_U = nullptr;
     int spec_Sp = 0, spec_SpE = 0;
+    const long long* lengths = nullptr;
+    float* hsel = nullptr;
 };
 struct SeqBwdArgs {
     const float *Hseq, *h0, *Rs, *Us, *Cs, *dHseq, *d_at_end, *d_at_len;
@@ -49,6 +51,7 @@
     bool probe = false;
 };
 
+constexpr bool seq_fwd_selects(SeqKind k) { return k == SeqKind::OneWave || k == SeqKind::TwoWave || k == SeqKind::TwoWaveSpec; }
 constexpr bool seq_h_supported(int H) { return H == 16 || H == 32 || H == 64; }
 constexpr bool seq_m_supported(int M) { return M == 1 || M == 2 || M == 3 || M == 4 || M == 5 || M == 7; }
 inline bool seq_desc_reaches(double floats) { return floats * sizeof(float) < 2147483648.0; }
diff --git a/eeg_gnn_ssl_amd/csrc/spec_inst.cpp b/eeg_gnn_ssl_amd/csrc/spec_inst.cpp
--- a/eeg_gnn_ssl_amd/csrc/spec_inst.cpp
+++ b/eeg_gnn_ssl_amd/csrc/spec_inst.cpp
@@ -211,17 +211,23 @@
     return -1;
 }
 
+bool dxf_applies(int Sp, int S, int N, int Fin, long long zero_rows) {
+    if (Fin != 64 || N < 1 || N > kDxfMaxN || Sp < 16 || S < 1 || S > Sp) return false;
+    if ((double)Sp * 192 * 4 >= 2147483648.0 || (double)S * N * 64 * 4 >= 2147483648.0) return false;
+    return zero_rows >= 0 && (double)zero_rows * 64 * 4 < 2147483648.0;
+}
+
 int launch_dxf(const float* dYh, int Sp, int S, int N, int Fin, const float* Wtq, size_t wstride, const float* basis, float* dX,
-               hipStream_t st, const char* tag) {
-    if (Fin != 64 || N < 1 || N > kDxfMaxN || Sp < 16 || S < 1 || S > Sp) return -1;
-    if ((double)Sp * 192 * 4 >= 2147483648.0 || (double)S * N * 64 * 4 >= 2147483648.0) return -1;
+               hipStream_t st, const char* tag, long long zero_rows) {
+    if (!dxf_applies(Sp, S, N, Fin, zero_rows)) return -1;
+    const unsigned zf = (unsigned)(zero_rows * 64);
     const size_t lds = dxf_lds_bytes();
     if (N == 19) {
         EEG_SET_MAX_LDS(gemm_dxf_kernel<19>, lds);
-        EEG_LAUNCH_P(tag, gemm_dxf_kernel<19>, dim3(ceil_div(Sp, kDxfRows)), dim3(256), lds, st, dYh, Sp, S, N, Wtq, (unsigned)wstride, basis, dX);
+        EEG_LAUNCH_P(tag, gemm_dxf_kernel<19>, dim3(ceil_div(Sp, kDxfRows)), dim3(256), lds, st, dYh, Sp, S, N, Wtq, (unsigned)wstride, basis, dX, zf);
     } else {
         EEG_SET_MAX_LDS(gemm_dxf_kernel<0>, lds);
-        EEG_LAUNCH_P(tag, gemm_dxf_kernel<0>, dim3(ceil_div(Sp, kDxfRows)), dim3(256), lds, st, dYh, Sp, S, N, Wtq, (unsigned)wstride, basis, dX);
+        EEG_LAUNCH_P(tag, gemm_dxf_kernel<0>, dim3(ceil_div(Sp, kDxfRows)), dim3(256), lds, st, dYh, Sp, S, N, Wtq, (unsigned)wstride, basis, dX, zf);
     }
     return hipGetLastError() == hipSuccess ? 0 : 2;
 }
diff --git a/eeg_gnn_ssl_amd/csrc/spec_launch.h b/eeg_gnn_ssl_amd/csrc/spec_launch.h
--- a/eeg_gnn_ssl_amd/csrc/spec_launch.h
+++ b/eeg_gnn_ssl_amd/csrc/spec_launch.h
@@ -28,8 +28,9 @@
                     hipStream_t st, const char* tag, size_t ah_gstride = 0);
 int launch_nnf(const float* A, size_t a_gstride, int K, int Sp, int G, const float* Wr, size_t wstride, float* C, int num_cus, hipStream_t st,
                const char* tag, const float* bias, const float* gscale);
+bool dxf_applies(int Sp, int S, int N, int Fin, long long zero_rows);
 int launch_dxf(const float* dYh, int Sp, int S, int N, int Fin, const float* Wtq, size_t wstride, const float* basis, float* dX,
-               hipStream_t st, const char* tag);
+               hipStream_t st, const char* tag, long long zero_rows = 0);
 struct TnfPlan { int ok, fxt, spg, rps; };
 TnfPlan tnf_plan(int Fin, int H, int Sp, int G, int num_cus);
 int launch_tnf(const TnfPlan& p, const float* Xh, size_t x_gstride, int Fin, const float* Hh, size_t h_gstride, const float* RHh,
diff --git a/eeg_gnn_ssl_amd/ops.py b/eeg_gnn_ssl_amd/ops.py
--- a/eeg_gnn_ssl_amd/ops.py
+++ b/eeg_gnn_ssl_amd/ops.py
@@ -506,16 +506,15 @@
     else:
         rs = us = cs = rhs = hpl = rhpl = None
     ws = _new((lib.query("eeg_dcrnn_layer_fwd_ws_floats", ctypes.byref(dims)),), x)
+    if lengths is not None:
+        lengths = lengths.to(device=x.device, dtype=torch.int64).contiguous()
+    if lengths is not None or want_hsel:
+        hsel = _new((b, n * h), x)
+        dims.sel_lengths, dims.hsel = (lengths.data_ptr() if lengths is not None else None), hsel.data_ptr()
+    else:
+        hsel = _new((0,), x)
     lib.call("eeg_dcrnn_layer_fwd", ctypes.byref(dims), _p(xsrc if xsrc is not None else xk), _p(xtm) if (xsrc is not None and bm != 2) else None,
              _p(h0), _p(p), _p(pack), planes_ptr, _p(hext), _p(rs), _p(us), _p(cs), _p(rhs), _p(hpl), _p(rhpl), _p(ws), _stream(x))
-    if lengths is not None:
-        lengths = lengths.to(device=x.device, dtype=torch.int64).contiguous()
-        hsel = _new((b, n * h), x)
-        lib.call("eeg_dcrnn_gather_last", _p(hext[1:]), _p(lengths), t_len, b, n * h, _p(hsel), _stream(x))
-    elif want_hsel:
-        hsel = hext[t_len].clone()
-    else:
-        hsel = _new((0,), x)
     if not save:
         return hext, hsel, []
     return hext, hsel, [xtm if xtm is not None else empty, _new((0,), p) if pack_given else pack, planes, rs, us, cs, rhs, hpl, rhpl,
@@ -582,7 +581,10 @@
     xk_ptr = ctypes.c_void_p(x.data_ptr() + 4 * x_off * b * n * fin)
     dx = _new((t_len + x_off, b, n, fin), hext) if need_dx else _new((0,), hext)
     if need_dx and x_off:
-        lib.call("eeg_dcrnn_zero", _p(dx), 4 * x_off * b * n * fin, _stream(dx))
+        dims.dx_front_rows = x_off * b * n
+        if not lib.query("eeg_dcrnn_layer_bwd_clears_dx_front", ctypes.byref(dims)):
+            dims.dx_front_rows = 0
+            lib.call("eeg_dcrnn_zero", _p(dx), 4 * x_off * b * n * fin, _stream(dx))
     dx_ptr = ctypes.c_void_p(dx.data_ptr() + 4 * x_off * b * n * fin) if need_dx else None
     dh0 = _new((b, n * h), hext) if (need_dh0 and has_h0) else _new((0,), hext)
     ws = _new((lib.query("eeg_dcrnn_layer_bwd_ws_floats", ctypes.byref(dims), 1 if need_dx else 0),), hext)
diff --git a/include/eeg_dcrnn.h b/include/eeg_dcrnn.h
--- a/include/eeg_dcrnn.h
+++ b/include/eeg_dcrnn.h
@@ -17,6 +17,9 @@
     const uint16_t* pack3;
     const float* spectral;
     const float* spack;
+    int64_t dx_front_rows;
+    const int64_t* sel_lengths;
+    float* hsel;
 } eeg_layer_dims;
 
 typedef struct eeg_decoder_dims {
@@ -105,6 +108,7 @@
                         float* Cs, float* RHs, float* Hplanes, float* RHplanes, float* ws, void* stream);
 
 size_t eeg_dcrnn_layer_bwd_ws_floats(const eeg_layer_dims* d, int need_dx);
+int eeg_dcrnn_layer_bwd_clears_dx_front(const eeg_layer_dims* d);
 int eeg_dcrnn_layer_bwd(const eeg_layer_dims* d, const float* X, const float* P, const float* pack,
                         const float* planes, const float* Hext, const float* Rs, const float* Us,
                         const float* Cs, const float* RHs, const float* Hplanes, const float* RHplanes,
```

Result: faster. 138,500 (median of 6 runs) (+1.5%).
